# goodmattg/ndivplanning

Measured on AMD Instinct MI355X. Metric: gan_train_steps_per_sec_traj8_batch64, higher is better.
Workload: dtype f32; 1 GPU; BASELINE configs[1]: train_gan.py step (D update + G update), codes mode, batch=64 trajectories per GPU, traj_len=8, num_sample=6, noise_dim=2; rows_per_gpu=2688, global_batch=64, parallelism=dp1, hip_graph=True, steps_per_graph_launch=16, repeats=1, gradient_exchange=none

## Files before the change

include/ndp.h:

```cpp
#ifndef NDP_H_
#define NDP_H_

#include <stddef.h>
#include <stdint.h>

#ifdef __cplusplus
extern "C" {
#endif

#define NDP_VERSION 135

#define NDP_OK            0
#define NDP_E_ARG         1
#define NDP_E_LAUNCH      2
#define NDP_E_UNSUPPORTED 3

#define NDP_CODE_DIM      256
#define NDP_ACTION_DIM    4
#define NDP_MAX_NOISE_DIM 16
#define NDP_MAX_SAMPLES   256
#define NDP_ROW_PAD       32

int         ndp_version(void);
const char *ndp_last_error(void);

int64_t ndp_g_param_count(int noise_dim);
int64_t ndp_d_param_count(void);

int64_t ndp_pad_rows(int64_t rows);

int64_t ndp_ndiv_partials(int64_t n, int k);
int ndp_ndiv_fwd_bwd(const float *x, int cx, const float *z, int cz, int64_t n, int k,
                     float grad_scale, float *loss_out, float *grad_x, float *partials,
                     void *stream);

int64_t ndp_g_acts_floats(int64_t m);
int ndp_g_forward(const float *g_params, int noise_dim,
                  const float *code, int64_t ld_code, int code_rep,
                  const float *noise, int64_t ld_noise, int64_t m,
                  float *acts, float *action_hat, void *stream);

int64_t ndp_g_bwd_ws_floats(int64_t m, int noise_dim);
int ndp_g_backward(const float *g_params, int noise_dim,
                   const float *code, int64_t ld_code, int code_rep,
                   const float *noise, int64_t ld_noise, int64_t m,
                   const float *acts, const float *d_action,
                   float *grad, float *ws, void *stream);

int ndp_d_forward(const float *d_params,
                  const float *action, int action_rep,
                  const float *code, int64_t ld_code, int code_rep, int64_t m,
                  float *logits, void *stream);

int64_t ndp_d_bwd_ws_floats(int64_t m);
int ndp_d_backward(const float *d_params,
                   const float *action, int action_rep,
                   const float *code, int64_t ld_code, int code_rep, int64_t m,
                   const float *d_logits, float *grad, float *d_action,
                   float *ws, void *stream);

int ndp_adam_step(float *params, const float *grad, float *exp_avg, float *exp_avg_sq,
                  int64_t n, int32_t *step_count, float lr, float beta1, float beta2,
                  float eps, void *stream);

struct ndp_p2p;
typedef struct ndp_step_config {
  int32_t noise_dim;
  int32_t num_sample;
  int64_t flat;
  float   inv_m_global;
  float   pairwise_div_factor;
  float   lr, beta1, beta2, eps;
  int32_t fuse_adam;
  int32_t device_noise;
  uint64_t noise_seed;
  const struct ndp_p2p *p2p;
} ndp_step_config;

typedef struct ndp_step_buffers {
  float   *g_params, *g_grad, *g_exp_avg, *g_exp_avg_sq;
  float   *d_params, *d_grad, *d_exp_avg, *d_exp_avg_sq;
  int32_t *g_step, *d_step;
  float   *losses;
  float   *loss_sums;
  float   *action_hat;
  float   *workspace;
} ndp_step_buffers;

int64_t ndp_step_workspace_floats(const ndp_step_config *cfg);

int ndp_step_d_grads(const ndp_step_config *cfg, const ndp_step_buffers *buf,
                     const float *codes, const float *actions, float *noise,
                     int run_g_forward, void *stream);
int ndp_step_g_grads(const ndp_step_config *cfg, const ndp_step_buffers *buf,
                     const float *codes, const float *actions, const float *noise,
                     void *stream);

int ndp_step_pack_params(const ndp_step_config *cfg, const ndp_step_buffers *buf, void *stream);

int ndp_step_apply_adam(const ndp_step_config *cfg, const ndp_step_buffers *buf, int which,
                        void *stream);

int ndp_uniform_noise(float *out, int64_t n, uint64_t seed, const int32_t *offset_dev,
                      void *stream);

#define NDP_P2P_MAX_RANKS    8
#define NDP_P2P_HANDLE_BYTES 64

typedef struct ndp_p2p {
  int32_t world, rank;
  int32_t timeout_ms;
  int32_t reserved;
  void   *region[NDP_P2P_MAX_RANKS];
} ndp_p2p;

int64_t ndp_p2p_region_bytes(void);
int ndp_p2p_region_alloc(void **region);
int ndp_p2p_region_free(void *region);
int ndp_p2p_region_reset(void *region);
int ndp_p2p_export(void *region, void *handle_out);
int ndp_p2p_open(const void *handle, void **mapped_out);
int ndp_p2p_close(void *mapped);
int ndp_p2p_status(const ndp_p2p *p2p, int32_t *status_out);
#define NDP_P2P_DIAG_WORDS 8
int ndp_p2p_diagnostics(const ndp_p2p *p2p, int32_t *words_out);
int ndp_p2p_status_async(const ndp_p2p *p2p, int32_t *pinned_host_out, void *stream);
int ndp_device_pci_bus_id(char *out, int len);
int ndp_p2p_all_reduce(const ndp_p2p *p2p, int net, const float *in, float *out, int64_t n,
                       const int32_t *step_word, void *stream);

int64_t ndp_encoder_param_floats(void);
int64_t ndp_encoder_workspace_floats(int64_t n_images);
int ndp_encoder_forward(const float *packed_params, const float *images, int64_t n_images,
                        float *codes, float *workspace, void *stream);
int ndp_encoder_forward_u8(const float *packed_params, const uint8_t *frames_hwc, int64_t n_images,
                           float *codes, float *workspace, void *stream);

int64_t ndp_fm_param_floats(void);
int64_t ndp_fm_stat_floats(void);
int64_t ndp_fm_workspace_floats(int64_t n_images);
int64_t ndp_fm_workspace_offset(int64_t n_images, int tensor);
int ndp_fm_layout(int what, int index, int64_t *offset, int64_t *dims );
int ndp_fm_pack_params(const float *params, float *workspace, void *stream);
int ndp_fm_forward(const float *params, float *running_stats, const float *state_cur,
                   const float *actions, int64_t n_images, int training, float *out,
                   float *workspace, void *stream);
int ndp_fm_train_grads(const float *params, float *running_stats, const float *state_cur,
                       const float *state_fut, const float *actions, int64_t n_images,
                       float *grad, float *loss, float *loss_sum, float *resid_out,
                       float *workspace, void *stream);
int ndp_fm_forward_u8(const float *params, float *running_stats, const uint8_t *frames_cur,
                      const float *actions, int64_t n_images, int training, float *out,
                      float *workspace, void *stream);
int ndp_fm_train_grads_u8(const float *params, float *running_stats, const uint8_t *frames_cur,
                          const uint8_t *frames_fut, const float *actions, int64_t n_images,
                          float *grad, float *loss, float *loss_sum, float *resid_out,
                          float *workspace, void *stream);
int ndp_fm_side_stream(int on);
typedef void (*ndp_fm_stat_sync_fn)(void *acc, int64_t words, void *stream, void *ctx);
int ndp_fm_set_stat_sync(ndp_fm_stat_sync_fn fn, void *ctx, int world);

int ndp_fm_grad_buckets(int64_t *offsets, int64_t *counts, int capacity);
int ndp_fm_bucket_wait(int bucket, void *stream);
int ndp_fm_backward(const float *params, const float *d_resid, int64_t n_images, float *grad,
                    float *workspace, void *stream);
int ndp_fm_apply_adam(float *params, const float *grad, float *exp_avg, float *exp_avg_sq,
                      int32_t *step_count, float lr, float beta1, float beta2, float eps,
                      float *workspace, void *stream);

int64_t ndp_ae_param_floats(void);
int64_t ndp_ae_stat_floats(void);
int64_t ndp_ae_workspace_floats(int64_t n_images);
int64_t ndp_ae_workspace_offset(int64_t n_images, int tensor);
int ndp_ae_layout(int what, int index, int64_t *offset, int64_t *dims );
int ndp_ae_pack_params(const float *params, float *workspace, void *stream);
int ndp_ae_train_grads(const float *params, float *running_stats, const float *images, int64_t n_images,
                       float *grad, float *loss, float *loss_sum, float *recon_out, float *workspace,
                       void *stream);
int ndp_ae_apply_adam(float *params, const float *grad, float *exp_avg, float *exp_avg_sq,
                      int32_t *step_count, float lr, float beta1, float beta2, float eps,
                      float *workspace, void *stream);
int ndp_ae_train_grads_dp(const float *params, float *running_stats, const float *images, int64_t n_images,
                          float *grad, float *loss, float *loss_sum, float *recon_out, float *workspace,
                          void *stream, ndp_fm_stat_sync_fn stat_sync, void *stat_ctx, int world);
int ndp_ae_grad_buckets(int64_t *offsets, int64_t *counts, int capacity, int *n_buckets);
int ndp_ae_bucket_wait(int bucket, void *stream);

int ndp_eval_score_select(const float *pred, int64_t n_traj, int rollouts, const float *target, int64_t n_target,
                          const int32_t *target_idx, int64_t values, const float *actions0, const float *pred0,
                          const int32_t *forced, float *err, int32_t *choice, float *action_out, float *pred_out,
                          void *stream);
int64_t ndp_eval_mse_ws_floats(int64_t n_pairs);
int ndp_eval_mse(const float *a, int64_t n_a, const float *b, int64_t n_b, const int32_t *a_idx, const int32_t *b_idx,
                 int64_t n_pairs, int64_t values, int64_t group, float *mse, float *acc, float *ws, void *stream);
int ndp_eval_g_input(const float *state_code, int64_t n_state, int state_rep, const float *goal_code, int64_t n_goal,
                     int goal_rep, int64_t rows, float *out, void *stream);
int ndp_eval_frames_u8(const uint8_t *frames_hwc, int64_t n_images, float *images, void *stream);

#define NDP_JPEG_OK          0
#define NDP_JPEG_UNSUPPORTED 1
#define NDP_JPEG_SIZE        2
#define NDP_JPEG_CORRUPT     3
#define NDP_JPEG_WORKSPACE   4
int64_t ndp_jpeg_workspace_bytes(int64_t n_images, int64_t stream_bytes);
int ndp_jpeg_decode_u8(const uint8_t *streams, const int64_t *offsets , int64_t n_images,
                       uint8_t *frames_hwc , int32_t *status , void *workspace,
                       int64_t workspace_bytes, void *stream);

int ndp_timing_enable(int on);
int ndp_timing_collect(char *names, int names_len, float *total_ms, int32_t *counts,
                       int max_kernels);

#ifdef __cplusplus
}
#endif
#endif
```

ndivplanning_amd/_capi.py:

```python
import ctypes
import os
from ctypes import POINTER, Structure, c_char_p, c_float, c_int, c_int32, c_int64, c_uint64, c_void_p

import torch

from . import _build

CODE_DIM = 256
ACTION_DIM = 4
MAX_NOISE_DIM = 16
MAX_SAMPLES = 256
ROW_PAD = 32
EXPECTED_VERSION = 135

_lib = None


class NdpError(RuntimeError):
    pass


P2P_MAX_RANKS = 8
P2P_HANDLE_BYTES = 64
P2P_DIAG_WORDS = 8


class P2P(Structure):
    _fields_ = [("world", c_int32), ("rank", c_int32), ("timeout_ms", c_int32), ("reserved", c_int32),
                ("region", c_void_p * P2P_MAX_RANKS)]


class StepConfig(Structure):
    _fields_ = [("noise_dim", c_int32), ("num_sample", c_int32), ("flat", c_int64),
                ("inv_m_global", c_float), ("pairwise_div_factor", c_float),
                ("lr", c_float), ("beta1", c_float), ("beta2", c_float), ("eps", c_float),
                ("fuse_adam", c_int32), ("device_noise", c_int32), ("noise_seed", c_uint64),
                ("p2p", POINTER(P2P))]


class StepBuffers(Structure):
    _fields_ = [(n, c_void_p) for n in (
        "g_params", "g_grad", "g_exp_avg", "g_exp_avg_sq",
        "d_params", "d_grad", "d_exp_avg", "d_exp_avg_sq",
        "g_step", "d_step", "losses", "loss_sums", "action_hat", "workspace")]


SIGNATURES = {
    "ndp_version": (c_int, []),
    "ndp_last_error": (c_char_p, []),
    "ndp_g_param_count": (c_int64, [c_int]),
    "ndp_d_param_count": (c_int64, []),
    "ndp_pad_rows": (c_int64, [c_int64]),
    "ndp_ndiv_partials": (c_int64, [c_int64, c_int]),
    "ndp_ndiv_fwd_bwd": (c_int, [c_void_p, c_int, c_void_p, c_int, c_int64, c_int, c_float,
                                 c_void_p, c_void_p, c_void_p, c_void_p]),
    "ndp_g_acts_floats": (c_int64, [c_int64]),
    "ndp_g_forward": (c_int, [c_void_p, c_int, c_void_p, c_int64, c_int, c_void_p, c_int64, c_int64,
                              c_void_p, c_void_p, c_void_p]),
    "ndp_g_bwd_ws_floats": (c_int64, [c_int64, c_int]),
    "ndp_g_backward": (c_int, [c_void_p, c_int, c_void_p, c_int64, c_int, c_void_p, c_int64, c_int64,
                               c_void_p, c_void_p, c_void_p, c_void_p, c_void_p]),
    "ndp_d_forward": (c_int, [c_void_p, c_void_p, c_int, c_void_p, c_int64, c_int, c_int64, c_void_p, c_void_p]),
    "ndp_d_bwd_ws_floats": (c_int64, [c_int64]),
    "ndp_d_backward": (c_int, [c_void_p, c_void_p, c_int, c_void_p, c_int64, c_int, c_int64, c_void_p,
                               c_void_p, c_void_p, c_void_p, c_void_p]),
    "ndp_adam_step": (c_int, [c_void_p, c_void_p, c_void_p, c_void_p, c_int64, c_void_p,
                              c_float, c_float, c_float, c_float, c_void_p]),
    "ndp_step_workspace_floats": (c_int64, [POINTER(StepConfig)]),
    "ndp_step_d_grads": (c_int, [POINTER(StepConfig), POINTER(StepBuffers), c_void_p, c_void_p, c_void_p,
                                 c_int, c_void_p]),
    "ndp_step_g_grads": (c_int, [POINTER(StepConfig), POINTER(StepBuffers), c_void_p, c_void_p, c_void_p,
                                 c_void_p]),
    "ndp_step_pack_params": (c_int, [POINTER(StepConfig), POINTER(StepBuffers), c_void_p]),
    "ndp_step_apply_adam": (c_int, [POINTER(StepConfig), POINTER(StepBuffers), c_int, c_void_p]),
    "ndp_uniform_noise": (c_int, [c_void_p, c_int64, c_uint64, c_void_p, c_void_p]),
    "ndp_p2p_region_bytes": (c_int64, []),
    "ndp_p2p_region_alloc": (c_int, [POINTER(c_void_p)]),
    "ndp_p2p_region_free": (c_int, [c_void_p]),
    "ndp_p2p_region_reset": (c_int, [c_void_p]),
    "ndp_p2p_export": (c_int, [c_void_p, c_void_p]),
    "ndp_p2p_open": (c_int, [c_void_p, POINTER(c_void_p)]),
    "ndp_p2p_close": (c_int, [c_void_p]),
    "ndp_p2p_status": (c_int, [POINTER(P2P), POINTER(c_int32)]),
    "ndp_p2p_diagnostics": (c_int, [POINTER(P2P), POINTER(c_int32)]),
    "ndp_p2p_status_async": (c_int, [POINTER(P2P), c_void_p, c_void_p]),
    "ndp_device_pci_bus_id": (c_int, [ctypes.c_char_p, c_int]),
    "ndp_p2p_all_reduce": (c_int, [POINTER(P2P), c_int, c_void_p, c_void_p, c_int64, c_void_p, c_void_p]),
    "ndp_encoder_param_floats": (c_int64, []),
    "ndp_encoder_workspace_floats": (c_int64, [c_int64]),
    "ndp_encoder_forward": (c_int, [c_void_p, c_void_p, c_int64, c_void_p, c_void_p, c_void_p]),
    "ndp_encoder_forward_u8": (c_int, [c_void_p, c_void_p, c_int64, c_void_p, c_void_p, c_void_p]),
    "ndp_fm_param_floats": (c_int64, []),
    "ndp_fm_stat_floats": (c_int64, []),
    "ndp_fm_workspace_floats": (c_int64, [c_int64]),
    "ndp_fm_workspace_offset": (c_int64, [c_int64, c_int]),
    "ndp_fm_layout": (c_int, [c_int, c_int, POINTER(c_int64), POINTER(c_int64)]),
    "ndp_fm_pack_params": (c_int, [c_void_p, c_void_p, c_void_p]),
    "ndp_fm_forward": (c_int, [c_void_p, c_void_p, c_void_p, c_void_p, c_int64, c_int, c_void_p, c_void_p, c_void_p]),
    "ndp_fm_train_grads": (c_int, [c_void_p, c_void_p, c_void_p, c_void_p, c_void_p, c_int64, c_void_p, c_void_p, c_void_p,
                                   c_void_p, c_void_p, c_void_p]),
    "ndp_fm_forward_u8": (c_int, [c_void_p, c_void_p, c_void_p, c_void_p, c_int64, c_int, c_void_p, c_void_p, c_void_p]),
    "ndp_fm_train_grads_u8": (c_int, [c_void_p, c_void_p, c_void_p, c_void_p, c_void_p, c_int64, c_void_p, c_void_p, c_void_p,
                                      c_void_p, c_void_p, c_void_p]),
    "ndp_fm_side_stream": (c_int, [c_int]),
    "ndp_fm_grad_buckets": (c_int, [POINTER(c_int64), POINTER(c_int64), c_int]),
    "ndp_fm_set_stat_sync": (c_int, [c_void_p, c_void_p, c_int]),
    "ndp_fm_bucket_wait": (c_int, [c_int, c_void_p]),
    "ndp_fm_backward": (c_int, [c_void_p, c_void_p, c_int64, c_void_p, c_void_p, c_void_p]),
    "ndp_fm_apply_adam": (c_int, [c_void_p, c_void_p, c_void_p, c_void_p, c_void_p, c_float, c_float, c_float, c_float,
                                  c_void_p, c_void_p]),
    "ndp_ae_param_floats": (c_int64, []),
    "ndp_ae_stat_floats": (c_int64, []),
    "ndp_ae_workspace_floats": (c_int64, [c_int64]),
    "ndp_ae_workspace_offset": (c_int64, [c_int64, c_int]),
    "ndp_ae_layout": (c_int, [c_int, c_int, POINTER(c_int64), POINTER(c_int64)]),
    "ndp_ae_pack_params": (c_int, [c_void_p, c_void_p, c_void_p]),
    "ndp_ae_train_grads": (c_int, [c_void_p, c_void_p, c_void_p, c_int64, c_void_p, c_void_p, c_void_p, c_void_p, c_void_p,
                                   c_void_p]),
    "ndp_ae_apply_adam": (c_int, [c_void_p, c_void_p, c_void_p, c_void_p, c_void_p, c_float, c_float, c_float, c_float,
                                  c_void_p, c_void_p]),
    "ndp_ae_train_grads_dp": (c_int, [c_void_p, c_void_p, c_void_p, c_int64, c_void_p, c_void_p, c_void_p, c_void_p,
                                      c_void_p, c_void_p, c_void_p, c_void_p, c_int]),
    "ndp_ae_grad_buckets": (c_int, [POINTER(c_int64), POINTER(c_int64), c_int, POINTER(c_int)]),
    "ndp_ae_bucket_wait": (c_int, [c_int, c_void_p]),
    "ndp_eval_score_select": (c_int, [c_void_p, c_int64, c_int, c_void_p, c_int64, c_void_p, c_int64, c_void_p, c_void_p,
                                      c_void_p, c_void_p, c_void_p, c_void_p, c_void_p, c_void_p]),
    "ndp_eval_mse_ws_floats": (c_int64, [c_int64]),
    "ndp_eval_mse": (c_int, [c_void_p, c_int64, c_void_p, c_int64, c_void_p, c_void_p, c_int64, c_int64, c_int64, c_void_p,
                             c_void_p, c_void_p, c_void_p]),
    "ndp_eval_g_input": (c_int, [c_void_p, c_int64, c_int, c_void_p, c_int64, c_int, c_int64, c_void_p, c_void_p]),
    "ndp_eval_frames_u8": (c_int, [c_void_p, c_int64, c_void_p, c_void_p]),
    "ndp_jpeg_workspace_bytes": (c_int64, [c_int64, c_int64]),
    "ndp_jpeg_decode_u8": (c_int, [c_void_p, c_void_p, c_int64, c_void_p, c_void_p, c_void_p, c_int64, c_void_p]),
    "ndp_timing_enable": (c_int, [c_int]),
    "ndp_timing_collect": (c_int, [ctypes.c_char_p, c_int, POINTER(c_float), POINTER(c_int32), c_int]),
}


def lib_path():
    return _build.LIB_PATH


def load():
    global _lib
    if _lib is not None:
        return _lib
    path = lib_path()
    if not os.path.exists(path):
        raise NdpError(
            "ndivplanning_amd: %s is missing -- build it with `python -m ndivplanning_amd._build` "
            "(or __graft_entry__.build()); there is no fallback path." % path)
    lib = ctypes.CDLL(path)
    for name, (res, args) in SIGNATURES.items():
        fn = getattr(lib, name)
        fn.restype = res
        fn.argtypes = args
    if lib.ndp_version() != EXPECTED_VERSION:
        raise NdpError("%s is version %d, this package needs %d: rebuild with `python -m ndivplanning_amd._build`"
                       % (path, lib.ndp_version(), EXPECTED_VERSION))
    _lib = lib
    return lib


def check(rc, what):
    if rc != 0:
        msg = load().ndp_last_error()
        raise NdpError("%s failed (code %d): %s" % (what, rc, msg.decode() if msg else "?"))


def stream_ptr(device=None):
    return c_void_p(torch.cuda.current_stream(device).cuda_stream)


def on_device(t):
    dev = t.device if isinstance(t, torch.Tensor) else torch.device(t)
    return torch.cuda.device(dev)


def ptr(t):
    return c_void_p(t.data_ptr()) if t is not None else c_void_p(0)


def require_gpu_f32(t, name):
    if not isinstance(t, torch.Tensor):
        raise TypeError("%s must be a torch.Tensor" % name)
    if not t.is_cuda:
        raise NdpError("%s is on %s: ndivplanning_amd computes only on a ROCm GPU (no CPU fallback)"
                       % (name, t.device))
    if t.dtype != torch.float32:
        raise NdpError("%s must be float32, got %s" % (name, t.dtype))
    return t


def empty(n, like):
    return torch.empty(int(n), dtype=torch.float32, device=like.device)


def timing_enable(on):
    load().ndp_timing_enable(1 if on else 0)


def timing_collect():
    lib = load()
    names = ctypes.create_string_buffer(4096)
    ms = (c_float * 64)()
    counts = (c_int32 * 64)()
    n = lib.ndp_timing_collect(names, 4096, ms, counts, 64)
    keys = [k for k in names.value.decode().split(";") if k]
    return {keys[i]: (float(ms[i]), int(counts[i])) for i in range(min(n, len(keys)))}


def g_param_count(noise_dim):
    return int(load().ndp_g_param_count(int(noise_dim)))


def d_param_count():
    return int(load().ndp_d_param_count())


def pad_rows(m):
    return (int(m) + ROW_PAD - 1) // ROW_PAD * ROW_PAD


def fm_grad_buckets():
    lib = load()
    off = (ctypes.c_int64 * 16)()
    cnt = (ctypes.c_int64 * 16)()
    n = lib.ndp_fm_grad_buckets(off, cnt, 16)
    if n <= 0:
        msg = lib.ndp_last_error()
        raise NdpError("ndp_fm_grad_buckets failed: %s" % (msg.decode() if msg else "?"))
    return [(int(off[i]), int(cnt[i])) for i in range(n)]


def ae_grad_buckets():
    lib = load()
    off = (ctypes.c_int64 * 16)()
    cnt = (ctypes.c_int64 * 16)()
    n = ctypes.c_int(0)
    check(lib.ndp_ae_grad_buckets(off, cnt, 16, ctypes.byref(n)), "ndp_ae_grad_buckets")
    return [(int(off[i]), int(cnt[i])) for i in range(n.value)]


STAT_SYNC_FN = ctypes.CFUNCTYPE(None, c_void_p, c_int64, c_void_p, c_void_p)
```

ndivplanning_amd/csrc/ndp_capi.inc:

```
#include <stdarg.h>
#include <stdio.h>
#include <stdlib.h>
#include <string.h>

#include <dlfcn.h>
#include <mutex>

#include "../../include/ndp.h"

namespace ndp {

static thread_local char g_err[512] = "";

static int fail(int code, const char* fmt, ...) {
  va_list ap;
  va_start(ap, fmt);
  vsnprintf(g_err, sizeof(g_err), fmt, ap);
  va_end(ap);
  return code;
}

#define NDP_CHECK_ARG(cond, ...) \
  do { if (!(cond)) return ndp::fail(NDP_E_ARG, __VA_ARGS__); } while (0)

static int check_launch(const char* what) {
  hipError_t e = hipGetLastError();
  if (e != hipSuccess) return fail(NDP_E_LAUNCH, "%s: %s", what, hipGetErrorString(e));
  return NDP_OK;
}

struct TimedLaunch { const char* name; hipEvent_t t0, t1; };
struct TimingState {
  bool on = false;
  TimedLaunch ev[4096];
  int n = 0;
};
static thread_local TimingState g_timing;

struct Roctx { int (*push)(const char*); int (*pop)(); bool on; };
static Roctx& roctx() {
  static Roctx r = [] {
    Roctx x = {nullptr, nullptr, false};
    const char* e = getenv("NDP_ROCTX");
    if (e && e[0] == '1') {
      void* h = dlopen("libroctx64.so", RTLD_NOW | RTLD_GLOBAL);
      if (!h) h = dlopen("libroctx64.so.4", RTLD_NOW | RTLD_GLOBAL);
      if (h) {
        x.push = reinterpret_cast<int (*)(const char*)>(dlsym(h, "roctxRangePushA"));
        x.pop = reinterpret_cast<int (*)()>(dlsym(h, "roctxRangePop"));
        x.on = x.push && x.pop;
      }
    }
    return x;
  }();
  return r;
}

struct KTimer {
  hipStream_t st; int idx; bool range;
  KTimer(const char* name, hipStream_t s) : st(s), idx(-1), range(false) {
    if (roctx().on) { roctx().push(name); range = true; }
    TimingState& t = g_timing;
    if (!t.on || t.n >= 4096) return;
    idx = t.n++;
    t.ev[idx].name = name;
    hipEventCreate(&t.ev[idx].t0);
    hipEventCreate(&t.ev[idx].t1);
    hipEventRecord(t.ev[idx].t0, st);
  }
  ~KTimer() {
    if (idx >= 0) hipEventRecord(g_timing.ev[idx].t1, st);
    if (range) roctx().pop();
  }
};

static inline bool aligned16(const void* p) { return (reinterpret_cast<uintptr_t>(p) & 15) == 0; }
static inline int64_t pad_rows(int64_t rows) { return (rows + NDP_ROW_PAD - 1) / NDP_ROW_PAD * NDP_ROW_PAD; }

template <typename K>
static void allow_lds(K kernel, int bytes) {
  hipFuncSetAttribute(reinterpret_cast<const void*>(kernel), hipFuncAttributeMaxDynamicSharedMemorySize, bytes);
}

constexpr int kMaxDevices = 64;
static std::once_flag g_attr_once[kMaxDevices];
static std::once_flag& device_once(std::once_flag (&flags)[kMaxDevices]) {
  int dev = 0;
  if (hipGetDevice(&dev) != hipSuccess || dev < 0 || dev >= kMaxDevices) dev = 0;
  return flags[dev];
}
static_assert(phase_a_lds_floats() * 4 * 3 <= 160 * 1024, "phase A: three workgroups per CU at large M");

static void set_attrs() {
  std::call_once(device_once(g_attr_once), [] {
#define NDP_ATTR_GFWD(WA) \
    allow_lds(k_g_fwd<WA, false>, g_fwd_lds_floats() * 4); \
    allow_lds(k_g_fwd<WA, true>, g_fwd_lds_floats() * 4);
    NDP_ATTR_GFWD(1) NDP_ATTR_GFWD(2) NDP_ATTR_GFWD(4)
#undef NDP_ATTR_GFWD
#define NDP_ATTR_D(NP) \
    allow_lds(k_d<NP, false>, (d_lds_floats<NP>() * 4)); \
    allow_lds(k_d<NP, true>, (d_lds_floats<NP>() * 4));
    NDP_ATTR_D(1) NDP_ATTR_D(2)
#undef NDP_ATTR_D
    allow_lds(k_g_bwd<false>, g_bwd_lds_floats() * 4);
    allow_lds(k_g_bwd<true>, g_bwd_lds_floats() * 4);
    allow_lds(k_wgrad, wgrad_lds_floats() * 4);
    allow_lds(k_wgrad_wide, wgrad_wide_launch_lds_floats() * 4);
#define NDP_ALLOW_A(RG, NR) allow_lds((k_phase_a<true, RG, NR>), phase_a_lds_floats() * 4)
#define NDP_ALLOW_B(RG, PRE, NR) allow_lds((k_phase_b<true, RG, PRE, NR>), phase_b_lds_floats(PRE) * 4)
    NDP_ALLOW_A(96, 0);
    NDP_ALLOW_A(kPhaseASmallRing, 0); NDP_ALLOW_A(kPhaseASmallRing, 1); NDP_ALLOW_A(kPhaseASmallRing, 4);
    NDP_ALLOW_B(96, true, 0);
    NDP_ALLOW_B(32, false, 0); NDP_ALLOW_B(32, false, 1); NDP_ALLOW_B(32, false, 4);
#undef NDP_ALLOW_A
#undef NDP_ALLOW_B
    allow_lds(k_ndiv<4, 2>, 64 * 1024);
    allow_lds(k_ndiv<16, 16>, 64 * 1024);
  });
}

struct GLayout { int64_t w1, b1, w2, b2, w3, b3, w4, b4, w5, b5, total; int in1; };
static GLayout g_layout(int nz) {
  GLayout L;
  L.in1 = CODE + nz;
  int64_t o = 0;
  L.w1 = o; o += 128 * (int64_t)L.in1;
  L.b1 = o; o += 128;
  L.w2 = o; o += 64 * 128;
  L.b2 = o; o += 64;
  L.w3 = o; o += 128 * 64;
  L.b3 = o; o += 128;
  L.w4 = o; o += 256 * 128;
  L.b4 = o; o += 256;
  L.w5 = o; o += 4 * 256;
  L.b5 = o; o += 4;
  L.total = o;
  return L;
}
struct DLayout { int64_t w1, b1, w2, b2, w3, b3, w4, b4, total; };
static DLayout d_layout() {
  DLayout L;
  int64_t o = 0;
  L.w1 = o; o += 64 * 260;
  L.b1 = o; o += 64;
  L.w2 = o; o += 128 * 64;
  L.b2 = o; o += 128;
  L.w3 = o; o += 256 * 128;
  L.b3 = o; o += 256;
  L.w4 = o; o += 256;
  L.b4 = o; o += 1;
  L.total = o;
  return L;
}
constexpr int kGPackF1 = 0, kGPackF2 = 32768, kGPackF3 = 40960, kGPackF4 = 49152,
              kGPackG2 = 81920, kGPackG3 = 90112, kGPackG4 = 98304, kGPackFloats = 131072;
constexpr int kDPackF1 = 0, kDPackF2 = 16384, kDPackF3 = 24576, kDPackG2 = 57344, kDPackG3 = 65536,
              kDPackFloats = 98304;

static GNet g_net(const float* p, int nz, const float* packed = nullptr) {
  const GLayout L = g_layout(nz);
  GNet n;
  n.w1 = p + L.w1; n.b1 = p + L.b1; n.w2 = p + L.w2; n.b2 = p + L.b2; n.w3 = p + L.w3; n.b3 = p + L.b3;
  n.w4 = p + L.w4; n.b4 = p + L.b4; n.w5 = p + L.w5; n.b5 = p + L.b5;
  n.ld1 = L.in1; n.nz = nz;
  n.pf1 = n.pf2 = n.pf3 = n.pf4 = n.pg2 = n.pg3 = n.pg4 = nullptr;
  if (packed) {
    n.pf1 = packed + kGPackF1; n.pf2 = packed + kGPackF2; n.pf3 = packed + kGPackF3; n.pf4 = packed + kGPackF4;
    n.pg2 = packed + kGPackG2; n.pg3 = packed + kGPackG3; n.pg4 = packed + kGPackG4;
  }
  return n;
}
static DNet d_net(const float* p, const float* packed = nullptr) {
  const DLayout L = d_layout();
  DNet n;
  n.w1 = p + L.w1; n.b1 = p + L.b1; n.w2 = p + L.w2; n.b2 = p + L.b2; n.w3 = p + L.w3; n.b3 = p + L.b3;
  n.w4 = p + L.w4; n.b4 = p + L.b4;
  n.pf1 = n.pf2 = n.pf3 = n.pg2 = n.pg3 = nullptr;
  if (packed) {
    n.pf1 = packed + kDPackF1; n.pf2 = packed + kDPackF2; n.pf3 = packed + kDPackF3;
    n.pg2 = packed + kDPackG2; n.pg3 = packed + kDPackG3;
  }
  return n;
}
static PackLayer pack_layer(int64_t w_off, int ld, int out, int main0, int main_in, int fwd_off, int dg_off) {
  PackLayer l;
  l.w_off = (int)w_off; l.ld = ld; l.out = out; l.main0 = main0; l.main_in = main_in; l.fwd_off = fwd_off; l.dg_off = dg_off;
  return l;
}
static PackSpec g_pack_spec(int nz, float* packed) {
  const GLayout L = g_layout(nz);
  PackSpec ps;
  memset(&ps, 0, sizeof(ps));
  ps.L[0] = pack_layer(L.w1, L.in1, 128, 0, CODE, kGPackF1, -1);
  ps.L[1] = pack_layer(L.w2, 128, 64, 0, 128, kGPackF2, kGPackG2);
  ps.L[2] = pack_layer(L.w3, 64, 128, 0, 64, kGPackF3, kGPackG3);
  ps.L[3] = pack_layer(L.w4, 128, 256, 0, 128, kGPackF4, kGPackG4);
  ps.nl = 4; ps.packed = packed;
  return ps;
}
static PackSpec d_pack_spec(float* packed) {
  const DLayout L = d_layout();
  PackSpec ps;
  memset(&ps, 0, sizeof(ps));
  ps.L[0] = pack_layer(L.w1, 260, 64, ADIM, CODE, kDPackF1, -1);
  ps.L[1] = pack_layer(L.w2, 64, 128, 0, 64, kDPackF2, kDPackG2);
  ps.L[2] = pack_layer(L.w3, 128, 256, 0, 128, kDPackF3, kDPackG3);
  ps.nl = 3; ps.packed = packed;
  return ps;
}
static int launch_pack(const float* params, int64_t n, const PackSpec& ps, hipStream_t st) {
  KTimer kt("k_pack", st);
  PackArgs a;
  a.params = params; a.n = (int)n; a.ps = ps;
  hipLaunchKernelGGL(k_pack, dim3((unsigned)((n + kThreads - 1) / kThreads)), dim3(kThreads), 0, st, a);
  return check_launch("k_pack");
}
static inline int64_t pad4(int64_t n) { return (n + 3) / 4 * 4; }

struct GActs { float *h1, *h2, *h3, *h4; };
static int64_t g_acts_floats(int64_t mpad) { return mpad * (128 + 64 + 128 + 256); }
static GActs g_acts(float* base, int64_t mpad) {
  GActs a;
  a.h1 = base; a.h2 = a.h1 + mpad * 128; a.h3 = a.h2 + mpad * 64; a.h4 = a.h3 + mpad * 128;
  return a;
}
static int wgrad_chunks(int njobs, int64_t rows) {
  int64_t want = 512 / njobs;
  if (want >= 8) want = want / 8 * 8;
  if (rows >= 16384 && want < 32) want = 32;
  int64_t maxc = rows / 64;
  if (maxc < 1) maxc = 1;
  if (want > maxc) want = maxc;
  if (want > 64) want = 64;
  return (int)want;
}
constexpr int kGJobs = 26, kDJobs = 19;
static void wgrad_plan(bool is_g, int64_t rows, int* heavy, int* light) {
  const int h = is_g ? 24 : (rows <= 4096 ? 8 : 32), l = is_g ? 12 : 8;
  if (rows >= 16384 || rows / 64 < h) { *heavy = *light = wgrad_chunks(is_g ? kGJobs : kDJobs, rows); return; }
  *heavy = h; *light = l;
}
static int wgrad_wide_chunks(int64_t rows) {
  if (rows < 28000) return 0;
  const int64_t want = (rows / 480 + 16) / 32 * 32;
  return (int)(want < 64 ? 64 : want);
}
static int wgrad_slabs(bool is_g, int64_t rows) {
  int h, l;
  wgrad_plan(is_g, rows, &h, &l);
  const int w = wgrad_wide_chunks(rows);
  return h > w ? h : w;
}
struct GBwdWs { float *dy1, *dy2, *dy3, *dy4, *dy5, *slabs; int nchunks, light; int64_t slab_stride; };
static int64_t g_bwd_floats(int64_t mpad, int nz) {
  return mpad * (128 + 64 + 128 + 256 + 4) + (int64_t)wgrad_slabs(true, mpad) * pad4(g_layout(nz).total);
}
static GBwdWs g_bwd_ws(float* base, int64_t mpad, int nz) {
  GBwdWs w;
  w.dy1 = base; w.dy2 = w.dy1 + mpad * 128; w.dy3 = w.dy2 + mpad * 64; w.dy4 = w.dy3 + mpad * 128;
  w.dy5 = w.dy4 + mpad * 256; w.slabs = w.dy5 + mpad * 4;
  wgrad_plan(true, mpad, &w.nchunks, &w.light);
  w.slab_stride = pad4(g_layout(nz).total);
  return w;
}
struct DBwdWs { float *xa, *h1, *h2, *h3, *dy1, *dy2, *dy3, *dl, *slabs, *lossp; int nchunks, light; int64_t slab_stride; };
static int64_t d_bwd_floats_rows(int64_t rows) {
  return rows * (4 + 2 * (64 + 128 + 256) + 1) + (int64_t)wgrad_slabs(false, rows) * pad4(d_layout().total) +
         pad4(rows / 16);
}
static int64_t d_bwd_floats(int64_t mpad, int npass) { return d_bwd_floats_rows(mpad * npass); }
static DBwdWs d_bwd_ws_rows(float* base, int64_t rows) {
  DBwdWs w;
  w.xa = base; w.h1 = w.xa + rows * 4; w.h2 = w.h1 + rows * 64; w.h3 = w.h2 + rows * 128;
  w.dy1 = w.h3 + rows * 256; w.dy2 = w.dy1 + rows * 64; w.dy3 = w.dy2 + rows * 128; w.dl = w.dy3 + rows * 256;
  w.slabs = w.dl + rows;
  wgrad_plan(false, rows, &w.nchunks, &w.light);
  w.slab_stride = pad4(d_layout().total);
  w.lossp = w.slabs + (int64_t)wgrad_slabs(false, rows) * w.slab_stride;
  return w;
}
static DBwdWs d_bwd_ws(float* base, int64_t mpad, int npass) { return d_bwd_ws_rows(base, mpad * npass); }
static int64_t step_real_pad(const ndp_step_config* c) { return pad_rows(c->flat); }
static int64_t step_d_rows(const ndp_step_config* c) { return step_real_pad(c) + pad_rows(c->flat * c->num_sample); }

struct NoiseGen { float* out; uint64_t seed; const int32_t* step; };

static int launch_g_fwd(const GNet& net, const float* code, int64_t ld_code, int code_rep,
                        const float* noise, int64_t ld_noise, int64_t m, const GActs* acts,
                        float* action_hat, const NoiseGen* gen, hipStream_t st) {
  set_attrs();
  GFwdArgs a;
  a.net = net;
  a.code = code; a.ld_code = ld_code; a.code_rep = code_rep;
  a.code_vec4 = (ld_code % 4 == 0) && aligned16(code);
  a.noise = noise; a.ld_noise = ld_noise; a.m = m;
  a.h1 = acts ? acts->h1 : nullptr; a.h2 = acts ? acts->h2 : nullptr;
  a.h3 = acts ? acts->h3 : nullptr; a.h4 = acts ? acts->h4 : nullptr;
  a.action_hat = action_hat;
  a.noise_out = gen ? gen->out : nullptr; a.noise_seed = gen ? gen->seed : 0; a.noise_step = gen ? gen->step : nullptr;
  const int walign = (net.ld1 % 4 == 0) ? 4 : (net.ld1 % 2 == 0 ? 2 : 1);
  const dim3 grid((unsigned)(pad_rows(m) / 16));
  const bool pk = net.pf1 != nullptr;
#define NDP_LAUNCH_GFWD(WA) \
  do { \
    if (pk) hipLaunchKernelGGL((k_g_fwd<WA, true>), grid, dim3(kThreads), g_fwd_lds_floats() * 4, st, a); \
    else hipLaunchKernelGGL((k_g_fwd<WA, false>), grid, dim3(kThreads), g_fwd_lds_floats() * 4, st, a); \
  } while (0)
  KTimer kt("k_g_fwd", st);
  if (walign == 4) NDP_LAUNCH_GFWD(4); else if (walign == 2) NDP_LAUNCH_GFWD(2); else NDP_LAUNCH_GFWD(1);
#undef NDP_LAUNCH_GFWD
  return check_launch("k_g_fwd");
}

static int launch_d(DArgs& a, int npass, int nd_blocks, hipStream_t st) {
  set_attrs();
  a.ntiles = (int)(a.mpad / 16);
  if (nd_blocks == 0) a.nd.n = 0;
  const dim3 grid((unsigned)(a.ntiles + nd_blocks));
  KTimer kt(a.do_backward ? (npass == 2 ? "k_d[2 pass fwd+bwd]" : "k_d[fwd+bwd]") : "k_d[fwd]", st);
  const bool pk = a.net.pf1 != nullptr;
#define NDP_LAUNCH_D(NP) \
  do { \
    if (pk) hipLaunchKernelGGL((k_d<NP, true>), grid, dim3(kThreads), (d_lds_floats<NP>() * 4), st, a); \
    else hipLaunchKernelGGL((k_d<NP, false>), grid, dim3(kThreads), (d_lds_floats<NP>() * 4), st, a); \
  } while (0)
  if (npass == 2) NDP_LAUNCH_D(2);
  else NDP_LAUNCH_D(1);
#undef NDP_LAUNCH_D
  return check_launch("k_d");
}

static int launch_g_bwd(GBwdArgs& a, hipStream_t st) {
  set_attrs();
  const dim3 grid((unsigned)(pad_rows(a.m) / 16));
  KTimer kt("k_g_bwd", st);
  if (a.net.pg2 != nullptr) hipLaunchKernelGGL((k_g_bwd<true>), grid, dim3(kThreads), g_bwd_lds_floats() * 4, st, a);
  else hipLaunchKernelGGL((k_g_bwd<false>), grid, dim3(kThreads), g_bwd_lds_floats() * 4, st, a);
  return check_launch("k_g_bwd");
}

static WgradJob make_job(const float* A, int lda, int a_cols, const float* B, int ldb, int b_cols,
                         int64_t dst_off, int dst_ld, int64_t bias_off, int kind) {
  WgradJob j;
  j.A = A; j.lda = lda; j.a_cols = a_cols;
  j.B = B; j.ldb = ldb; j.b_cols = b_cols;
  j.b_rowmod = 0x7fffffff; j.b_rowdiv = 1; j.b_rowmax = 0x7fffffff;
  j.b_vec = (ldb % 4 == 0) && aligned16(B);
  j.dst_off = (int)dst_off; j.dst_ld = dst_ld; j.bias_off = (int)bias_off; j.kind = kind;
  j.rows = 0; j.seg = 0; j.seg_s = 1; j.seg_k = 1; j.seg_wrap = 0;
  j.nchunks = kind == WG_FULL ? 1 : 0;
  return j;
}

static int seg_per_tile(int K) { int s = 15 / K + 2; return s < 16 ? s : 16; }
static int64_t seg_entries(int64_t mpad, int K) { return (mpad / 16 * seg_per_tile(K) + 15) / 16 * 16; }

static void build_g_jobs(WgradArgs& w, int nz, const GBwdWs& ws, const GActs& acts,
                         const float* code, int64_t ld_code, int code_rep,
                         const float* noise, int64_t ld_noise, int64_t m, const float* dy1seg = nullptr) {
  const GLayout L = g_layout(nz);
  int n = 0;
  const int code_rowmax = (int)((m - 1) / code_rep);
  for (int jb = 0; jb < 2; ++jb) {
    for (int kb = 0; kb < 4; ++kb) {
      WgradJob j = make_job((dy1seg ? dy1seg : ws.dy1) + jb * 64, 128, 64, code + kb * 64, (int)ld_code, 64,
                            L.w1 + (int64_t)jb * 64 * L.in1 + kb * 64, L.in1,
                            kb == 0 ? L.b1 + jb * 64 : -1, WG_FULL);
      j.b_rowdiv = code_rep; j.b_rowmax = code_rowmax;
      if (dy1seg) { j.rows = (int)seg_entries(pad_rows(m), code_rep); j.seg = 1; j.seg_s = seg_per_tile(code_rep); j.seg_k = code_rep; }
      j.nchunks = 0;
      w.job[n++] = j;
    }
    WgradJob t = make_job(ws.dy1 + jb * 64, 128, 64, noise, (int)ld_noise, nz,
                          L.w1 + (int64_t)jb * 64 * L.in1 + CODE, L.in1, -1, WG_SKINNY_B);
    t.b_rowmax = (int)(m - 1);
    w.job[n++] = t;
  }
  for (int kb = 0; kb < 2; ++kb)
    w.job[n++] = make_job(ws.dy2, 64, 64, acts.h1 + kb * 64, 128, 64, L.w2 + kb * 64, 128,
                          kb == 0 ? L.b2 : -1, WG_FULL);
  for (int jb = 0; jb < 2; ++jb)
    w.job[n++] = make_job(ws.dy3 + jb * 64, 128, 64, acts.h2, 64, 64, L.w3 + (int64_t)jb * 64 * 64, 64,
                          L.b3 + jb * 64, WG_FULL);
  const int wide = wgrad_wide_chunks(pad_rows(m));
  if (!wide)
    for (int jb = 0; jb < 4; ++jb)
      for (int kb = 0; kb < 2; ++kb)
        w.job[n++] = make_job(ws.dy4 + jb * 64, 256, 64, acts.h3 + kb * 64, 128, 64,
                              L.w4 + (int64_t)jb * 64 * 128 + kb * 64, 128, kb == 0 ? L.b4 + jb * 64 : -1, WG_FULL);
  for (int kb = 0; kb < 4; ++kb)
    w.job[n++] = make_job(ws.dy5, 4, 4, acts.h4 + kb * 64, 256, 64, L.w5 + kb * 64, 256,
                          kb == 0 ? L.b5 : -1, WG_SKINNY_A);
  w.njobs = n; w.net_is_g = 1;
  w.nwide = 0; w.wide_chunks = 0;
  w.wide_begin = w.wide_end = 0;
  if (wide) {
    w.nwide = 2;
    for (int h = 0; h < 2; ++h)
      w.job[n + h] = make_job(ws.dy4 + h * 128, 256, 128, acts.h3, 128, 128, L.w4 + (int64_t)h * 128 * 128, 128, L.b4 + h * 128, WG_WIDE);
    w.wide_chunks = wide;
    w.wide_begin = (int)L.w4; w.wide_end = (int)L.b4 + 256;
  }
  w.nreg = 2;
  w.reg_begin[0] = (int)L.w1; w.reg_end[0] = (int)L.b1 + 128;
  w.reg_begin[1] = (int)L.w5; w.reg_end[1] = (int)L.b5 + 4;
}

static void build_d_jobs(WgradArgs& w, const DBwdWs& ws, const float* code, int64_t ld_code, int code_rep,
                         int64_t m, int64_t mpad, const float* dy1seg = nullptr, int64_t rpad = 0, int64_t wide_rows = 0) {
  const DLayout L = d_layout();
  int n = 0;
  for (int kb = 0; kb < 4; ++kb) {
    WgradJob j = make_job(dy1seg ? dy1seg : ws.dy1, 64, 64, code + kb * 64, (int)ld_code, 64, L.w1 + ADIM + kb * 64, 260,
                          kb == 0 ? L.b1 : -1, WG_FULL);
    j.b_rowmod = (int)mpad; j.b_rowdiv = code_rep; j.b_rowmax = (int)((m - 1) / code_rep);
    if (dy1seg) {
      const int e = (int)seg_entries(mpad, code_rep);
      j.rows = e + (int)rpad; j.seg = 1; j.seg_wrap = e;
      j.seg_s = seg_per_tile(code_rep); j.seg_k = code_rep;
    }
    j.nchunks = 0;
    w.job[n++] = j;
  }
  w.job[n++] = make_job(ws.dy1, 64, 64, ws.xa, 4, ADIM, L.w1, 260, -1, WG_SKINNY_B);
  for (int jb = 0; jb < 2; ++jb)
    w.job[n++] = make_job(ws.dy2 + jb * 64, 128, 64, ws.h1, 64, 64, L.w2 + (int64_t)jb * 64 * 64, 64,
                          L.b2 + jb * 64, WG_FULL);
  const int wide = wgrad_wide_chunks(wide_rows);
  if (!wide)
    for (int jb = 0; jb < 4; ++jb)
      for (int kb = 0; kb < 2; ++kb)
        w.job[n++] = make_job(ws.dy3 + jb * 64, 256, 64, ws.h2 + kb * 64, 128, 64,
                              L.w3 + (int64_t)jb * 64 * 128 + kb * 64, 128, kb == 0 ? L.b3 + jb * 64 : -1, WG_FULL);
  for (int kb = 0; kb < 4; ++kb)
    w.job[n++] = make_job(ws.dl, 1, 1, ws.h3 + kb * 64, 256, 64, L.w4 + kb * 64, 256,
                          kb == 0 ? L.b4 : -1, WG_SKINNY_A);
  w.njobs = n; w.net_is_g = 0;
  w.nwide = 0; w.wide_chunks = 0;
  w.wide_begin = w.wide_end = 0;
  if (wide) {
    w.nwide = 2;
    for (int h = 0; h < 2; ++h)
      w.job[n + h] = make_job(ws.dy3 + h * 128, 256, 128, ws.h2, 128, 128, L.w3 + (int64_t)h * 128 * 128, 128, L.b3 + h * 128, WG_WIDE);
    w.wide_chunks = wide;
    w.wide_begin = (int)L.w3; w.wide_end = (int)L.b3 + 256;
  }
  w.nreg = 2;
  w.reg_begin[0] = (int)L.w1; w.reg_end[0] = (int)L.b1 + 64;
  w.reg_begin[1] = (int)L.w4; w.reg_end[1] = (int)L.b4 + 1;
}

struct AdamHyper { float lr, beta1, beta2; };

static int launch_wgrad(WgradArgs& w, int64_t rows, int nchunks, int light, float* slabs, int64_t slab_stride,
                        int32_t* bump, const AdamHyper& hp, const NdivArgs* nd, int nd_blocks, hipStream_t st) {
  set_attrs();
  w.rows = (int)rows;
  for (int i = 0; i < w.njobs; ++i) w.job[i].nchunks = w.job[i].nchunks ? nchunks : light;
  for (int i = 0; i < w.nwide; ++i) w.job[w.njobs + i].nchunks = w.wide_chunks;
  w.slabs = slabs; w.slab_stride = slab_stride; w.bump = bump;
  w.lr = hp.lr; w.beta1 = hp.beta1; w.beta2 = hp.beta2;
  w.nchunks = nchunks;
  if (nd != nullptr && nd_blocks > 0) w.nd = *nd; else { memset(&w.nd, 0, sizeof(w.nd)); nd_blocks = 0; }
  const dim3 grid((unsigned)(w.nwide * w.wide_chunks + 8 * ((nchunks + 7) / 8) * w.njobs + nd_blocks));
  KTimer kt(w.net_is_g ? "k_wgrad[G]" : "k_wgrad[D]", st);
  if (w.nwide) hipLaunchKernelGGL(k_wgrad_wide, grid, dim3(kThreads), wgrad_wide_launch_lds_floats() * 4, st, w);
  else hipLaunchKernelGGL(k_wgrad, grid, dim3(kThreads), wgrad_lds_floats() * 4, st, w);
  return check_launch("k_wgrad");
}

static void set_red_regions(ReduceArgs& r, const WgradArgs& w, int light) {
  r.nregions = light != r.nchunks ? w.nreg : 0;
  for (int i = 0; i < r.nregions; ++i) { r.reg_begin[i] = w.reg_begin[i]; r.reg_end[i] = w.reg_end[i]; r.reg_slabs[i] = light; }
  if (w.nwide) {
    const int i = r.nregions++;
    r.reg_begin[i] = w.wide_begin; r.reg_end[i] = w.wide_end; r.reg_slabs[i] = w.wide_chunks;
  }
}

static int launch_reduce(ReduceArgs& r, hipStream_t st) {
  const dim3 grid((unsigned)((r.n + kThreads - 1) / kThreads + 1));
  KTimer kt("k_reduce_adam", st);
  if (r.p2p.world > 1)
    hipLaunchKernelGGL(k_reduce_adam<true>, grid, dim3(kThreads), 0, st, r);
  else
    hipLaunchKernelGGL(k_reduce_adam<false>, grid, dim3(kThreads), 0, st, r);
  return check_launch("k_reduce_adam");
}

static int ndiv_block_threads(int k) { return k <= 64 ? 64 : kThreads; }
static int ndiv_rows_per_block(int k, int threads) { return threads / k; }
static size_t ndiv_lds_bytes(int G, int k, int cx, int cz) { return ((size_t)G * k * (cx + cz + 2) + 8) * 4; }

static NdivArgs ndiv_args(const float* x, int cx, const float* z, int cz, int64_t n, int k, float grad_scale,
                          float* grad, float* partials, int threads) {
  NdivArgs a;
  a.x = x; a.cx = cx; a.z = z; a.cz = cz; a.n = n; a.k = k;
  a.rows_per_block = ndiv_rows_per_block(k, threads);
  a.grad_scale = grad_scale; a.grad = grad; a.partials = partials;
  return a;
}

static int launch_ndiv(const float* x, int cx, const float* z, int cz, int64_t n, int k, float grad_scale,
                       float* grad, float* partials, hipStream_t st) {
  set_attrs();
  const int threads = ndiv_block_threads(k);
  NdivArgs a = ndiv_args(x, cx, z, cz, n, k, grad_scale, grad, partials, threads);
  const int G = a.rows_per_block;
  const size_t lds = ndiv_lds_bytes(G, k, cx, cz);
  const dim3 grid((unsigned)((n + G - 1) / G));
  KTimer kt("k_ndiv", st);
  if (cx <= 4 && cz <= 2) hipLaunchKernelGGL((k_ndiv<4, 2>), grid, dim3(threads), lds, st, a);
  else hipLaunchKernelGGL((k_ndiv<16, 16>), grid, dim3(threads), lds, st, a);
  return check_launch("k_ndiv");
}

}

using namespace ndp;

extern "C" {

int ndp_version(void) { return NDP_VERSION; }
const char* ndp_last_error(void) { return g_err; }
int64_t ndp_g_param_count(int noise_dim) { return g_layout(noise_dim).total; }
int64_t ndp_d_param_count(void) { return d_layout().total; }
int64_t ndp_pad_rows(int64_t rows) { return pad_rows(rows); }

int64_t ndp_ndiv_partials(int64_t n, int k) {
  if (k < 1 || k > NDP_MAX_SAMPLES || n < 0) return 0;
  const int G = ndiv_rows_per_block(k, ndiv_block_threads(k));
  return (n + G - 1) / G + 1;
}

int ndp_ndiv_fwd_bwd(const float* x, int cx, const float* z, int cz, int64_t n, int k, float grad_scale,
                     float* loss_out, float* grad_x, float* partials, void* stream) {
  NDP_CHECK_ARG(x && z && loss_out && partials, "ndp_ndiv_fwd_bwd: null pointer");
  NDP_CHECK_ARG(k >= 1 && k <= NDP_MAX_SAMPLES, "ndp_ndiv_fwd_bwd: k=%d outside 1..%d", k, NDP_MAX_SAMPLES);
  NDP_CHECK_ARG(cx >= 1 && cx <= kNdivMaxC && cz >= 1 && cz <= kNdivMaxC, "ndp_ndiv_fwd_bwd: channel count outside 1..16");
  NDP_CHECK_ARG(n >= 1 && n * k < (1ll << 31), "ndp_ndiv_fwd_bwd: bad row count %lld", (long long)n);
  hipStream_t st = (hipStream_t)stream;
  int rc = launch_ndiv(x, cx, z, cz, n, k, grad_scale, grad_x, partials, st);
  if (rc) return rc;
  const int G = ndiv_rows_per_block(k, ndiv_block_threads(k));
  hipLaunchKernelGGL(k_sum_partials, dim3(1), dim3(kThreads), 0, st, (const float*)partials,
                     (int)((n + G - 1) / G), 1.0f, loss_out);
  return check_launch("k_sum_partials");
}

int64_t ndp_g_acts_floats(int64_t m) { return g_acts_floats(pad_rows(m)); }

static int check_g_common(const char* fn, const float* g_params, int noise_dim, const float* code,
                          int64_t ld_code, int code_rep, const float* noise, int64_t ld_noise, int64_t m) {
  NDP_CHECK_ARG(g_params && code && noise, "%s: null pointer", fn);
  NDP_CHECK_ARG(aligned16(g_params), "%s: g_params must be 16-byte aligned", fn);
  NDP_CHECK_ARG(noise_dim >= 1 && noise_dim <= NDP_MAX_NOISE_DIM, "%s: noise_dim=%d outside 1..%d", fn, noise_dim, NDP_MAX_NOISE_DIM);
  NDP_CHECK_ARG(m >= 1 && m < (1ll << 30), "%s: bad row count %lld", fn, (long long)m);
  NDP_CHECK_ARG(code_rep >= 1 && ld_code >= NDP_CODE_DIM && ld_noise >= noise_dim, "%s: bad strides", fn);
  return NDP_OK;
}

int ndp_g_forward(const float* g_params, int noise_dim, const float* code, int64_t ld_code, int code_rep,
                  const float* noise, int64_t ld_noise, int64_t m, float* acts, float* action_hat, void* stream) {
  int rc = check_g_common("ndp_g_forward", g_params, noise_dim, code, ld_code, code_rep, noise, ld_noise, m);
  if (rc) return rc;
  NDP_CHECK_ARG(action_hat && aligned16(action_hat), "ndp_g_forward: action_hat null or not 16-byte aligned");
  NDP_CHECK_ARG(!acts || aligned16(acts), "ndp_g_forward: acts not 16-byte aligned");
  const int64_t mpad = pad_rows(m);
  GActs a;
  if (acts) a = g_acts(acts, mpad);
  return launch_g_fwd(g_net(g_params, noise_dim), code, ld_code, code_rep, noise, ld_noise, m,
                      acts ? &a : nullptr, action_hat, nullptr, (hipStream_t)stream);
}

int64_t ndp_g_bwd_ws_floats(int64_t m, int noise_dim) { return g_bwd_floats(pad_rows(m), noise_dim); }

static int g_backward_impl(const GNet& gnet, int nz, const float* code, int64_t ld_code, int code_rep,
                           const float* noise, int64_t ld_noise, int64_t m, const GActs& acts,
                           const float* d_action, const float* d_action2, float* ws_base,
                           ReduceArgs& red, int32_t* bump, const AdamHyper& hp, hipStream_t st,
                           const float* dy1seg = nullptr) {
  const int64_t mpad = pad_rows(m);
  GBwdWs ws = g_bwd_ws(ws_base, mpad, nz);
  GBwdArgs b;
  b.net = gnet;
  b.m = m;
  b.h1 = acts.h1; b.h2 = acts.h2; b.h3 = acts.h3; b.h4 = acts.h4;
  b.d_action = d_action; b.d_action2 = d_action2;
  b.dy1 = ws.dy1; b.dy2 = ws.dy2; b.dy3 = ws.dy3; b.dy4 = ws.dy4; b.dy5 = ws.dy5;
  int rc = NDP_OK;
  if (d_action != nullptr) {
    rc = launch_g_bwd(b, st);
    if (rc) return rc;
  }
  WgradArgs w;
  build_g_jobs(w, nz, ws, acts, code, ld_code, code_rep, noise, ld_noise, m, dy1seg);
  rc = launch_wgrad(w, mpad, ws.nchunks, ws.light, ws.slabs, ws.slab_stride, bump, hp, nullptr, 0, st);
  if (rc) return rc;
  red.slabs = ws.slabs; red.nchunks = ws.nchunks; red.slab_stride = ws.slab_stride;
  set_red_regions(red, w, ws.light);
  red.n = g_layout(nz).total;
  return launch_reduce(red, st);
}

int ndp_g_backward(const float* g_params, int noise_dim, const float* code, int64_t ld_code, int code_rep,
                   const float* noise, int64_t ld_noise, int64_t m, const float* acts, const float* d_action,
                   float* grad, float* ws, void* stream) {
  int rc = check_g_common("ndp_g_backward", g_params, noise_dim, code, ld_code, code_rep, noise, ld_noise, m);
  if (rc) return rc;
  NDP_CHECK_ARG(acts && d_action && grad && ws, "ndp_g_backward: null pointer");
  NDP_CHECK_ARG(aligned16(acts) && aligned16(d_action) && aligned16(ws), "ndp_g_backward: buffers must be 16-byte aligned");
  ReduceArgs red;
  memset(&red, 0, sizeof(red));
  red.grad = grad;
  GActs a = g_acts(const_cast<float*>(acts), pad_rows(m));
  return g_backward_impl(g_net(g_params, noise_dim), noise_dim, code, ld_code, code_rep, noise, ld_noise, m, a, d_action,
                         nullptr, ws, red, nullptr, AdamHyper{0.f, 0.f, 0.f}, (hipStream_t)stream);
}

static int check_d_common(const char* fn, const float* d_params, const float* action, int action_rep,
                          const float* code, int64_t ld_code, int code_rep, int64_t m) {
  NDP_CHECK_ARG(d_params && action && code, "%s: null pointer", fn);
  NDP_CHECK_ARG(aligned16(d_params), "%s: d_params must be 16-byte aligned", fn);
  NDP_CHECK_ARG(m >= 1 && m < (1ll << 29), "%s: bad row count %lld", fn, (long long)m);
  NDP_CHECK_ARG(action_rep >= 1 && code_rep >= 1 && ld_code >= NDP_CODE_DIM, "%s: bad strides", fn);
  return NDP_OK;
}

static void d_args_init(DArgs& a, const float* d_params, const float* code, int64_t ld_code, int code_rep, int64_t m) {
  memset(&a, 0, sizeof(a));
  a.net = d_net(d_params);
  a.code = code; a.ld_code = ld_code; a.code_rep = code_rep;
  a.code_vec4 = (ld_code % 4 == 0) && aligned16(code);
  a.m = m; a.mpad = pad_rows(m);
  a.inv_m = 1.f / (float)m;
}

int ndp_d_forward(const float* d_params, const float* action, int action_rep, const float* code, int64_t ld_code,
                  int code_rep, int64_t m, float* logits, void* stream) {
  int rc = check_d_common("ndp_d_forward", d_params, action, action_rep, code, ld_code, code_rep, m);
  if (rc) return rc;
  NDP_CHECK_ARG(logits, "ndp_d_forward: null logits");
  DArgs a;
  d_args_init(a, d_params, code, ld_code, code_rep, m);
  a.pass[0].action = action; a.pass[0].action_rep = action_rep; a.pass[0].target = 0.f;
  a.logits = logits;
  return launch_d(a, 1, 0, (hipStream_t)stream);
}

int64_t ndp_d_bwd_ws_floats(int64_t m) { return d_bwd_floats(pad_rows(m), 1); }

int ndp_d_backward(const float* d_params, const float* action, int action_rep, const float* code, int64_t ld_code,
                   int code_rep, int64_t m, const float* d_logits, float* grad, float* d_action, float* ws,
                   void* stream) {
  int rc = check_d_common("ndp_d_backward", d_params, action, action_rep, code, ld_code, code_rep, m);
  if (rc) return rc;
  NDP_CHECK_ARG(d_logits, "ndp_d_backward: null d_logits");
  NDP_CHECK_ARG(!grad || (ws && aligned16(ws)), "ndp_d_backward: grad needs a 16-byte aligned workspace");
  NDP_CHECK_ARG(!d_action || action_rep == 1, "ndp_d_backward: d_action needs action_rep == 1");
  hipStream_t st = (hipStream_t)stream;
  DArgs a;
  d_args_init(a, d_params, code, ld_code, code_rep, m);
  a.pass[0].action = action; a.pass[0].action_rep = action_rep; a.pass[0].target = 0.f;
  a.ext_dlogit = d_logits;
  a.do_backward = 1;
  a.d_action = d_action;
  DBwdWs w;
  if (grad) {
    w = d_bwd_ws(ws, a.mpad, 1);
    a.h1 = w.h1; a.h2 = w.h2; a.h3 = w.h3; a.dy1 = w.dy1; a.dy2 = w.dy2; a.dy3 = w.dy3; a.dl = w.dl; a.xa = w.xa;
  }
  rc = launch_d(a, 1, 0, st);
  if (rc || !grad) return rc;
  WgradArgs wa;
  build_d_jobs(wa, w, code, ld_code, code_rep, m, a.mpad, nullptr, 0, a.mpad);
  rc = launch_wgrad(wa, a.mpad, w.nchunks, w.light, w.slabs, w.slab_stride, nullptr, AdamHyper{0.f, 0.f, 0.f}, nullptr, 0, st);
  if (rc) return rc;
  ReduceArgs red;
  memset(&red, 0, sizeof(red));
  red.slabs = w.slabs; red.nchunks = w.nchunks; red.slab_stride = w.slab_stride; red.n = d_layout().total;
  set_red_regions(red, wa, w.light);
  red.grad = grad;
  return launch_reduce(red, st);
}

int ndp_adam_step(float* params, const float* grad, float* exp_avg, float* exp_avg_sq, int64_t n,
                  int32_t* step_count, float lr, float beta1, float beta2, float eps, void* stream) {
  NDP_CHECK_ARG(params && grad && exp_avg && exp_avg_sq && step_count, "ndp_adam_step: null pointer");
  NDP_CHECK_ARG(n >= 1, "ndp_adam_step: n < 1");
  hipStream_t st = (hipStream_t)stream;
  hipLaunchKernelGGL(k_adam_advance, dim3(1), dim3(1), 0, st, step_count, lr, beta1, beta2);
  AdamArgs a;
  a.params = params; a.exp_avg = exp_avg; a.exp_avg_sq = exp_avg_sq; a.grad = grad; a.n = n;
  a.step = step_count; a.lr = lr; a.beta1 = beta1; a.beta2 = beta2; a.eps = eps;
  memset(&a.pack, 0, sizeof(a.pack));
  KTimer kt("k_adam", st);
  hipLaunchKernelGGL(k_adam, dim3((unsigned)((n + kThreads - 1) / kThreads)), dim3(kThreads), 0, st, a);
  return check_launch("k_adam");
}

struct StepWs {
  GActs acts; float* gb; float* db; float* d_action; float* nd_grad; float* nd_part; int64_t nd_count;
  float* g_packed; float* d_packed;
  float* d_seg; float* g_seg;
};
static bool several_per_cu(int64_t workgroups) { return workgroups > 256; }

static int step_code_rows(int K, bool several_per_cu) {
  if (!several_per_cu) return 0;
  return K % 16 == 0 ? 1 : (K >= 6 ? 4 : 0);
}

static bool step_ndiv_fused(const ndp_step_config* c) { return c->noise_dim <= 2; }
static int step_ndiv_threads(const ndp_step_config* c) {
  return step_ndiv_fused(c) ? kThreads : ndiv_block_threads(c->num_sample);
}

static int64_t step_floats(const ndp_step_config* c, StepWs* out, float* base) {
  const int64_t m = c->flat * c->num_sample, mpad = pad_rows(m);
  int64_t o = 0;
  const int64_t o_acts = o; o += g_acts_floats(mpad);
  const int64_t o_gb = o; o += g_bwd_floats(mpad, c->noise_dim);
  const int64_t o_db = o;
  { const int64_t a_ = d_bwd_floats(mpad, 2), b_ = d_bwd_floats_rows(step_d_rows(c)); o += a_ > b_ ? a_ : b_; }
  const int64_t o_da = o; o += mpad * 4;
  const int64_t o_ng = o; o += mpad * 4;
  const int64_t o_np = o;
  const int G = ndiv_rows_per_block(c->num_sample, step_ndiv_threads(c));
  const int64_t npart = (c->flat + G - 1) / G;
  o += pad4(npart);
  const int64_t o_gp = o; o += kGPackFloats;
  const int64_t o_dp = o; o += kDPackFloats;
  const int64_t o_ds = o;
  o += (seg_entries(mpad, c->num_sample) + step_real_pad(c)) * 64;
  const int64_t o_gs = o; o += seg_entries(mpad, c->num_sample) * 128;
  if (out) {
    out->g_packed = base + o_gp; out->d_packed = base + o_dp;
    out->d_seg = base + o_ds; out->g_seg = base + o_gs;
    out->acts = g_acts(base + o_acts, mpad);
    out->gb = base + o_gb; out->db = base + o_db; out->d_action = base + o_da; out->nd_grad = base + o_ng;
    out->nd_part = base + o_np; out->nd_count = npart;
  }
  return o;
}

static int check_step(const char* fn, const ndp_step_config* c, const ndp_step_buffers* b, const float* codes,
                      const float* actions, const float* noise) {
  NDP_CHECK_ARG(c && b && codes && actions && noise, "%s: null pointer", fn);
  NDP_CHECK_ARG(c->noise_dim >= 1 && c->noise_dim <= NDP_MAX_NOISE_DIM, "%s: noise_dim=%d outside 1..%d", fn, c->noise_dim, NDP_MAX_NOISE_DIM);
  NDP_CHECK_ARG(c->num_sample >= 1 && c->num_sample <= NDP_MAX_SAMPLES, "%s: num_sample=%d outside 1..%d", fn, c->num_sample, NDP_MAX_SAMPLES);
  NDP_CHECK_ARG(c->flat >= 1 && c->flat * c->num_sample < (1ll << 28), "%s: bad flat=%lld", fn, (long long)c->flat);
  NDP_CHECK_ARG(b->g_params && b->d_params && b->losses && b->action_hat && b->workspace && b->g_step && b->d_step,
                "%s: null buffer", fn);
  NDP_CHECK_ARG(c->fuse_adam ? (b->g_exp_avg && b->g_exp_avg_sq && b->d_exp_avg && b->d_exp_avg_sq)
                             : (b->g_grad && b->d_grad), "%s: missing Adam state / gradient buffers", fn);
  NDP_CHECK_ARG(aligned16(b->g_params) && aligned16(b->d_params) && aligned16(b->workspace) && aligned16(b->action_hat) &&
                aligned16(codes) && aligned16(actions), "%s: buffers must be 16-byte aligned", fn);
  return NDP_OK;
}

static int fill_p2p(const char* fn, P2PArgs& x, const ndp_p2p* c, int net, int64_t n) {
  memset(&x, 0, sizeof(x));
  if (c == nullptr || c->world <= 1) return NDP_OK;
  NDP_CHECK_ARG(c->world <= NDP_P2P_MAX_RANKS && c->rank >= 0 && c->rank < c->world, "%s: p2p world=%d rank=%d", fn, c->world, c->rank);
  NDP_CHECK_ARG(n <= (net == 0 ? kP2PCapD : kP2PCapG), "%s: %lld values exceed the p2p inbox of net %d", fn, (long long)n, net);
  for (int r = 0; r < c->world; ++r) NDP_CHECK_ARG(c->region[r] != nullptr, "%s: p2p region of rank %d is null", fn, r);
  x.world = c->world; x.rank = c->rank; x.net = net;
  x.timeout_ticks = 100000ll * (c->timeout_ms > 0 ? c->timeout_ms : 10000);
  for (int r = 0; r < c->world; ++r) x.region[r] = static_cast<uint32_t*>(c->region[r]);
  return NDP_OK;
}

#define NDP_HIP(call, what) do { hipError_t e_ = (call); if (e_ != hipSuccess) \
  return ndp::fail(NDP_E_LAUNCH, "%s: %s", what, hipGetErrorString(e_)); } while (0)

int64_t ndp_p2p_region_bytes(void) { return kP2PWords * 4; }

int ndp_p2p_region_alloc(void** region) {
  NDP_CHECK_ARG(region != nullptr, "ndp_p2p_region_alloc: null pointer");
  static_assert(sizeof(hipIpcMemHandle_t) == NDP_P2P_HANDLE_BYTES, "handle size");
  void* p = nullptr;
  NDP_HIP(hipExtMallocWithFlags(&p, (size_t)kP2PWords * 4, hipDeviceMallocUncached), "ndp_p2p_region_alloc");
  hipError_t e = hipMemset(p, 0, (size_t)kP2PWords * 4);
  if (e == hipSuccess) e = hipDeviceSynchronize();
  if (e != hipSuccess) { hipFree(p); return ndp::fail(NDP_E_LAUNCH, "ndp_p2p_region_alloc: %s", hipGetErrorString(e)); }
  *region = p;
  return NDP_OK;
}

int ndp_p2p_region_free(void* region) {
  if (region == nullptr) return NDP_OK;
  NDP_HIP(hipFree(region), "ndp_p2p_region_free");
  return NDP_OK;
}

int ndp_p2p_region_reset(void* region) {
  NDP_CHECK_ARG(region != nullptr, "ndp_p2p_region_reset: null pointer");
  NDP_HIP(hipDeviceSynchronize(), "ndp_p2p_region_reset");
  NDP_HIP(hipMemset(region, 0, (size_t)kP2PInboxD * 4), "ndp_p2p_region_reset");
  NDP_HIP(hipDeviceSynchronize(), "ndp_p2p_region_reset");
  return NDP_OK;
}

int ndp_p2p_export(void* region, void* handle_out) {
  NDP_CHECK_ARG(region && handle_out, "ndp_p2p_export: null pointer");
  hipIpcMemHandle_t h;
  NDP_HIP(hipIpcGetMemHandle(&h, region), "ndp_p2p_export");
  memcpy(handle_out, &h, sizeof(h));
  return NDP_OK;
}

int ndp_p2p_open(const void* handle, void** mapped_out) {
  NDP_CHECK_ARG(handle && mapped_out, "ndp_p2p_open: null pointer");
  hipIpcMemHandle_t h;
  memcpy(&h, handle, sizeof(h));
  void* p = nullptr;
  NDP_HIP(hipIpcOpenMemHandle(&p, h, hipIpcMemLazyEnablePeerAccess), "ndp_p2p_open");
  *mapped_out = p;
  return NDP_OK;
}

int ndp_p2p_close(void* mapped) {
  if (mapped == nullptr) return NDP_OK;
  NDP_HIP(hipIpcCloseMemHandle(mapped), "ndp_p2p_close");
  return NDP_OK;
}

int ndp_p2p_status(const ndp_p2p* c, int32_t* status_out) {
  NDP_CHECK_ARG(c && status_out && c->rank >= 0 && c->rank < NDP_P2P_MAX_RANKS && c->region[c->rank], "ndp_p2p_status: bad arguments");
  NDP_HIP(hipMemcpy(status_out, c->region[c->rank], 4, hipMemcpyDeviceToHost), "ndp_p2p_status");
  return NDP_OK;
}

int ndp_p2p_diagnostics(const ndp_p2p* c, int32_t* words_out) {
  NDP_CHECK_ARG(c && words_out && c->rank >= 0 && c->rank < NDP_P2P_MAX_RANKS && c->region[c->rank], "ndp_p2p_diagnostics: bad arguments");
  NDP_HIP(hipMemcpy(words_out, c->region[c->rank], 4 * NDP_P2P_DIAG_WORDS, hipMemcpyDeviceToHost), "ndp_p2p_diagnostics");
  return NDP_OK;
}

int ndp_p2p_status_async(const ndp_p2p* c, int32_t* pinned_host_out, void* stream) {
  NDP_CHECK_ARG(c && pinned_host_out && c->rank >= 0 && c->rank < NDP_P2P_MAX_RANKS && c->region[c->rank], "ndp_p2p_status_async: bad arguments");
  NDP_HIP(hipMemcpyAsync(pinned_host_out, c->region[c->rank], 4, hipMemcpyDeviceToHost, (hipStream_t)stream), "ndp_p2p_status_async");
  return NDP_OK;
}

int ndp_device_pci_bus_id(char* out, int len) {
  NDP_CHECK_ARG(out && len >= 16, "ndp_device_pci_bus_id: need a buffer of >= 16 bytes");
  int dev = 0;
  NDP_HIP(hipGetDevice(&dev), "ndp_device_pci_bus_id");
  NDP_HIP(hipDeviceGetPCIBusId(out, len, dev), "ndp_device_pci_bus_id");
  return NDP_OK;
}

int ndp_p2p_all_reduce(const ndp_p2p* c, int net, const float* in, float* out, int64_t n, const int32_t* step_word,
                       void* stream) {
  NDP_CHECK_ARG(c && in && out && step_word && n >= 1 && (net == 0 || net == 1), "ndp_p2p_all_reduce: bad arguments");
  ReduceArgs red;
  memset(&red, 0, sizeof(red));
  int rc = fill_p2p("ndp_p2p_all_reduce", red.p2p, c, net, n);
  if (rc) return rc;
  red.slabs = in; red.nchunks = 1; red.slab_stride = 0; red.n = n;
  red.grad = out; red.step = step_word;
  return launch_reduce(red, (hipStream_t)stream);
}

int64_t ndp_step_workspace_floats(const ndp_step_config* cfg) {
  if (!cfg || cfg->flat < 1 || cfg->num_sample < 1 || cfg->num_sample > NDP_MAX_SAMPLES) return 0;
  return step_floats(cfg, nullptr, nullptr);
}

int ndp_step_d_grads(const ndp_step_config* c, const ndp_step_buffers* b, const float* codes, const float* actions,
                     float* noise, int run_g_forward, void* stream) {
  int rc = check_step("ndp_step_d_grads", c, b, codes, actions, noise);
  if (rc) return rc;
  hipStream_t st = (hipStream_t)stream;
  const int K = c->num_sample, nz = c->noise_dim;
  const int64_t m = c->flat * K, mpad = pad_rows(m);
  StepWs ws;
  step_floats(c, &ws, b->workspace);
  const int64_t rpad = step_real_pad(c);
  DBwdWs dw = run_g_forward ? d_bwd_ws_rows(ws.db, step_d_rows(c)) : d_bwd_ws(ws.db, mpad, 2);
  const bool fused_ndiv = step_ndiv_fused(c);
  NdivArgs nd;
  if (fused_ndiv)
    nd = ndiv_args(b->action_hat, ADIM, noise, nz, c->flat, K, c->pairwise_div_factor, ws.nd_grad, ws.nd_part, kThreads);
  int loss_count = (int)(mpad / 16);
  if (run_g_forward) {
    set_attrs();
    PhaseAArgs pa;
    memset(&pa, 0, sizeof(pa));
    pa.g = g_net(b->g_params, nz, ws.g_packed);
    pa.d = d_net(b->d_params, ws.d_packed);
    pa.code = codes; pa.code_rep = K;
    pa.noise = c->device_noise ? nullptr : noise;
    pa.noise_out = c->device_noise ? noise : nullptr; pa.noise_seed = c->noise_seed; pa.noise_step = b->g_step;
    pa.actions = actions;
    pa.m = m; pa.mpad = mpad; pa.flat = c->flat; pa.rpad = rpad;
    pa.inv_m = c->inv_m_global; pa.real_scale = (float)K;
    pa.gh1 = ws.acts.h1; pa.gh2 = ws.acts.h2; pa.gh3 = ws.acts.h3; pa.gh4 = ws.acts.h4;
    pa.action_hat = b->action_hat;
    pa.h1 = dw.h1; pa.h2 = dw.h2; pa.h3 = dw.h3; pa.dy1 = dw.dy1; pa.dy2 = dw.dy2; pa.dy3 = dw.dy3; pa.dl = dw.dl; pa.xa = dw.xa;
    pa.loss_partials = dw.lossp;
    pa.dy1seg = ws.d_seg; pa.seg_s = seg_per_tile(K); pa.seg_entries = (int)seg_entries(mpad, K);
    KTimer kt("k_phase_a", st);
    loss_count = (int)(mpad / 16 + rpad / 16);
    const bool small = several_per_cu(loss_count);
    const int nr = step_code_rows(K, small);
#define NDP_LAUNCH_A(RG, NR) hipLaunchKernelGGL((k_phase_a<true, RG, NR>), dim3((unsigned)loss_count), dim3(kThreads), phase_a_lds_floats() * 4, st, pa)
    if (small) {
      if (nr == 1) NDP_LAUNCH_A(kPhaseASmallRing, 1);
      else if (nr == 4) NDP_LAUNCH_A(kPhaseASmallRing, 4);
      else NDP_LAUNCH_A(kPhaseASmallRing, 0);
    } else {
      NDP_LAUNCH_A(96, 0);
    }
#undef NDP_LAUNCH_A
    rc = check_launch("k_phase_a");
    if (rc) return rc;
  } else {
    DArgs a;
    d_args_init(a, b->d_params, codes, CODE, K, m);
    a.net = d_net(b->d_params, ws.d_packed);
    a.inv_m = c->inv_m_global;
    a.pass[0].action = actions; a.pass[0].action_rep = K; a.pass[0].target = 1.f;
    a.pass[1].action = b->action_hat; a.pass[1].action_rep = 1; a.pass[1].target = 0.f;
    a.do_backward = 1;
    a.h1 = dw.h1; a.h2 = dw.h2; a.h3 = dw.h3; a.dy1 = dw.dy1; a.dy2 = dw.dy2; a.dy3 = dw.dy3; a.dl = dw.dl; a.xa = dw.xa;
    a.loss_partials = dw.lossp;
    rc = launch_d(a, 2, 0, st);
    if (rc) return rc;
  }
  WgradArgs wa;
  build_d_jobs(wa, dw, codes, CODE, K, m, mpad, run_g_forward ? ws.d_seg : nullptr, rpad, run_g_forward ? step_d_rows(c) : 2 * mpad);
  rc = launch_wgrad(wa, run_g_forward ? step_d_rows(c) : 2 * mpad, dw.nchunks, dw.light, dw.slabs, dw.slab_stride, b->d_step,
                    AdamHyper{c->lr, c->beta1, c->beta2}, fused_ndiv ? &nd : nullptr, (int)ws.nd_count, st);
  if (rc) return rc;
  ReduceArgs red;
  memset(&red, 0, sizeof(red));
  red.slabs = dw.slabs; red.nchunks = dw.nchunks; red.slab_stride = dw.slab_stride; red.n = d_layout().total;
  set_red_regions(red, wa, dw.light);
  red.grad = b->d_grad;
  if (c->fuse_adam) {
    red.params = b->d_params; red.exp_avg = b->d_exp_avg; red.exp_avg_sq = b->d_exp_avg_sq; red.step = b->d_step;
    red.lr = c->lr; red.beta1 = c->beta1; red.beta2 = c->beta2; red.eps = c->eps;
    red.pack = d_pack_spec(ws.d_packed);
  }
  red.step = b->d_step;
  rc = fill_p2p("ndp_step_d_grads", red.p2p, c->p2p, 0, red.n);
  if (rc) return rc;
  red.loss[0].partials = dw.lossp; red.loss[0].count = loss_count; red.loss[0].scale = c->inv_m_global;
  red.loss[0].slot = 0;
  red.nloss = 1; red.losses = b->losses; red.loss_sums = b->loss_sums;
  return launch_reduce(red, st);
}

int ndp_step_g_grads(const ndp_step_config* c, const ndp_step_buffers* b, const float* codes, const float* actions,
                     const float* noise, void* stream) {
  int rc = check_step("ndp_step_g_grads", c, b, codes, actions, noise);
  if (rc) return rc;
  hipStream_t st = (hipStream_t)stream;
  const int K = c->num_sample, nz = c->noise_dim;
  const int64_t m = c->flat * K, mpad = pad_rows(m);
  StepWs ws;
  step_floats(c, &ws, b->workspace);
  DBwdWs dw = d_bwd_ws_rows(ws.db, step_d_rows(c));
  if (!step_ndiv_fused(c)) {
    rc = launch_ndiv(b->action_hat, ADIM, noise, nz, c->flat, K, c->pairwise_div_factor, ws.nd_grad, ws.nd_part, st);
    if (rc) return rc;
  }
  set_attrs();
  GBwdWs gw = g_bwd_ws(ws.gb, mpad, nz);
  PhaseBArgs pb;
  memset(&pb, 0, sizeof(pb));
  pb.g = g_net(b->g_params, nz, ws.g_packed);
  pb.d = d_net(b->d_params, ws.d_packed);
  pb.code = codes; pb.code_rep = K;
  pb.action_hat = b->action_hat; pb.nd_grad = ws.nd_grad;
  pb.m = m; pb.inv_m = c->inv_m_global;
  pb.gh1 = ws.acts.h1; pb.gh2 = ws.acts.h2; pb.gh3 = ws.acts.h3; pb.gh4 = ws.acts.h4;
  pb.dy1 = gw.dy1; pb.dy2 = gw.dy2; pb.dy3 = gw.dy3; pb.dy4 = gw.dy4; pb.dy5 = gw.dy5;
  pb.loss_partials = dw.lossp;
  pb.dy1seg = ws.g_seg; pb.seg_s = seg_per_tile(K); pb.seg_entries = (int)seg_entries(mpad, K);
  {
    KTimer kt("k_phase_b", st);
    const int nt = (int)(mpad / 16);
    const bool small = several_per_cu(nt);
    const int nr = step_code_rows(K, small);
#define NDP_LAUNCH_B(RG, PRE, NR) hipLaunchKernelGGL((k_phase_b<true, RG, PRE, NR>), dim3((unsigned)nt), dim3(kThreads), phase_b_lds_floats(PRE) * 4, st, pb)
    if (small) {
      if (nr == 1) NDP_LAUNCH_B(32, false, 1);
      else if (nr == 4) NDP_LAUNCH_B(32, false, 4);
      else NDP_LAUNCH_B(32, false, 0);
    } else {
      NDP_LAUNCH_B(96, true, 0);
    }
#undef NDP_LAUNCH_B
  }
  rc = check_launch("k_phase_b");
  if (rc) return rc;
  ReduceArgs red;
  memset(&red, 0, sizeof(red));
  red.grad = b->g_grad;
  if (c->fuse_adam) {
    red.params = b->g_params; red.exp_avg = b->g_exp_avg; red.exp_avg_sq = b->g_exp_avg_sq; red.step = b->g_step;
    red.lr = c->lr; red.beta1 = c->beta1; red.beta2 = c->beta2; red.eps = c->eps;
    red.pack = g_pack_spec(nz, ws.g_packed);
  }
  red.step = b->g_step;
  rc = fill_p2p("ndp_step_g_grads", red.p2p, c->p2p, 1, g_layout(nz).total);
  if (rc) return rc;
  red.loss[0].partials = dw.lossp; red.loss[0].count = (int)(mpad / 16); red.loss[0].scale = c->inv_m_global;
  red.loss[0].slot = 1;
  red.loss[1].partials = ws.nd_part; red.loss[1].count = (int)ws.nd_count; red.loss[1].scale = 1.f;
  red.loss[1].slot = 2;
  red.nloss = 2; red.losses = b->losses; red.loss_sums = b->loss_sums;
  return g_backward_impl(g_net(b->g_params, nz, ws.g_packed), nz, codes, CODE, K, noise, nz, m, ws.acts, nullptr,
                         nullptr, ws.gb, red, b->g_step, AdamHyper{c->lr, c->beta1, c->beta2}, st, ws.g_seg);
}

#ifdef NDP_STAMPS
int ndp_debug_set_stamps(void* dev_buffer, int kernel_id) {
  unsigned long long* p = (unsigned long long*)dev_buffer;
  if (hipMemcpyToSymbol(HIP_SYMBOL(g_stamp_kernel), &kernel_id, sizeof(int)) != hipSuccess) return NDP_E_LAUNCH;
  return hipMemcpyToSymbol(HIP_SYMBOL(g_stamps), &p, sizeof(p)) == hipSuccess ? 0 : NDP_E_LAUNCH;
}
#endif

int ndp_timing_enable(int on) {
  TimingState& t = g_timing;
  for (int i = 0; i < t.n; ++i) { hipEventDestroy(t.ev[i].t0); hipEventDestroy(t.ev[i].t1); }
  t.n = 0;
  t.on = on != 0;
  return NDP_OK;
}

int ndp_timing_collect(char* names, int names_len, float* total_ms, int32_t* counts, int max_kernels) {
  if (!(names && total_ms && counts && names_len > 0 && max_kernels > 0)) {
    fail(NDP_E_ARG, "ndp_timing_collect: bad arguments");
    return 0;
  }
  TimingState& t = g_timing;
  const char* seen[64];
  int nk = 0;
  names[0] = 0;
  for (int i = 0; i < t.n; ++i) {
    if (hipEventSynchronize(t.ev[i].t1) != hipSuccess) {
      fail(NDP_E_LAUNCH, "ndp_timing_collect: event sync failed");
      return 0;
    }
    float ms = 0.f;
    hipEventElapsedTime(&ms, t.ev[i].t0, t.ev[i].t1);
    int k = 0;
    while (k < nk && strcmp(seen[k], t.ev[i].name) != 0) ++k;
    if (k == nk) {
      if (nk >= max_kernels || nk >= 64) continue;
      seen[nk] = t.ev[i].name; total_ms[nk] = 0.f; counts[nk] = 0; ++nk;
      strncat(names, t.ev[i].name, names_len - strlen(names) - 2);
      strncat(names, ";", names_len - strlen(names) - 1);
    }
    total_ms[k] += ms;
    counts[k] += 1;
    hipEventDestroy(t.ev[i].t0);
    hipEventDestroy(t.ev[i].t1);
  }
  t.n = 0;
  return nk;
}

int ndp_step_pack_params(const ndp_step_config* c, const ndp_step_buffers* b, void* stream) {
  NDP_CHECK_ARG(c && b && b->g_params && b->d_params && b->workspace, "ndp_step_pack_params: null pointer");
  NDP_CHECK_ARG(c->noise_dim >= 1 && c->noise_dim <= NDP_MAX_NOISE_DIM && c->flat >= 1 && c->num_sample >= 1 &&
                c->num_sample <= NDP_MAX_SAMPLES, "ndp_step_pack_params: bad configuration");
  StepWs ws;
  step_floats(c, &ws, b->workspace);
  hipStream_t st = (hipStream_t)stream;
  int rc = launch_pack(b->g_params, g_layout(c->noise_dim).total, g_pack_spec(c->noise_dim, ws.g_packed), st);
  if (rc) return rc;
  return launch_pack(b->d_params, d_layout().total, d_pack_spec(ws.d_packed), st);
}

int ndp_step_apply_adam(const ndp_step_config* c, const ndp_step_buffers* b, int which, void* stream) {
  NDP_CHECK_ARG(c && b && b->workspace, "ndp_step_apply_adam: null pointer");
  NDP_CHECK_ARG(which == 0 || which == 1, "ndp_step_apply_adam: which must be 0 (D) or 1 (G)");
  StepWs ws;
  step_floats(c, &ws, b->workspace);
  hipStream_t st = (hipStream_t)stream;
  AdamArgs a;
  if (which == 1) {
    NDP_CHECK_ARG(b->g_params && b->g_grad && b->g_exp_avg && b->g_exp_avg_sq && b->g_step, "ndp_step_apply_adam: null G buffer");
    a.params = b->g_params; a.grad = b->g_grad; a.exp_avg = b->g_exp_avg; a.exp_avg_sq = b->g_exp_avg_sq;
    a.n = g_layout(c->noise_dim).total; a.step = b->g_step; a.pack = g_pack_spec(c->noise_dim, ws.g_packed);
  } else {
    NDP_CHECK_ARG(b->d_params && b->d_grad && b->d_exp_avg && b->d_exp_avg_sq && b->d_step, "ndp_step_apply_adam: null D buffer");
    a.params = b->d_params; a.grad = b->d_grad; a.exp_avg = b->d_exp_avg; a.exp_avg_sq = b->d_exp_avg_sq;
    a.n = d_layout().total; a.step = b->d_step; a.pack = d_pack_spec(ws.d_packed);
  }
  a.lr = c->lr; a.beta1 = c->beta1; a.beta2 = c->beta2; a.eps = c->eps;
  KTimer kt("k_adam", st);
  hipLaunchKernelGGL(k_adam, dim3((unsigned)((a.n + kThreads - 1) / kThreads)), dim3(kThreads), 0, st, a);
  return check_launch("k_adam");
}

int ndp_uniform_noise(float* out, int64_t n, uint64_t seed, const int32_t* offset_dev, void* stream) {
  NDP_CHECK_ARG(out && n >= 1, "ndp_uniform_noise: bad arguments");
  const int64_t nthreads = n;
  hipLaunchKernelGGL(k_philox, dim3((unsigned)((nthreads + kThreads - 1) / kThreads)), dim3(kThreads), 0,
                     (hipStream_t)stream, out, n, seed, offset_dev);
  return check_launch("k_philox");
}

}
```

ndivplanning_amd/csrc/ndp_device.h:

```cpp
#pragma once
#include <hip/hip_runtime.h>
#include <stdint.h>

namespace ndp {

typedef float f32x4 __attribute__((ext_vector_type(4)));
typedef float f32x2 __attribute__((ext_vector_type(2)));
typedef uint32_t u32x4 __attribute__((ext_vector_type(4)));

constexpr int kThreads = 256;
constexpr int kWaves = 4;
constexpr float kLreluSlope = 0.01f;

enum Act { ACT_NONE = 0, ACT_RELU = 1, ACT_LRELU = 2 };

__device__ __forceinline__ int lds_ld(int width) { return width + 4; }

template <int ACT>
__device__ __forceinline__ float act_fwd(float v) {
  if (ACT == ACT_RELU) return v > 0.f ? v : 0.f;
  if (ACT == ACT_LRELU) return v > 0.f ? v : v * kLreluSlope;
  return v;
}

// ... 116 lines not shown
            if (4 * q + j < tail_n_) wtail[n][j] = wt_p[(size_t)(n * 16) * ldw + j];
        }
      }
    }
#pragma unroll
    for (int p = 0; p < PF; ++p)
#pragma unroll
      for (int n = 0; n < NT; ++n)
        if ((p * NT + n) * nslices / kItems == i) ring[p][n] = frag(n, p);
  }
  __device__ __forceinline__ void preload(const float* __restrict__ Wm, int ldw_,
                                          const float* __restrict__ bias,
                                          const float* __restrict__ Wt, int tail_n) {
    bind(Wm, ldw_, bias, Wt, tail_n);
    preload_slice(0, 1);
    pin_vmem();
  }
};

struct NoPrefetch {
  __device__ __forceinline__ void preload_slice(int, int) {}
};

template <int RT, int IN, int OUT, int ACT, int WALIGN, bool PACKED, int RING, class NEXT>
__device__ __forceinline__ void layer_fwd_run(FwdW<IN, OUT, WALIGN, PACKED, RING>& w,
                                              const float* X, int ldx, float* Y, int ldy,
                                              const float* Xt, int ldt, NEXT& next) {
  constexpr int NT = OUT / 64, NIT = IN / 16;
  constexpr int PF = FwdW<IN, OUT, WALIGN, PACKED, RING>::PF;
  const int lane = threadIdx.x & 63, wave = threadIdx.x >> 6;
  const int c = lane & 15, q = lane >> 4;
  const int col0 = wave * (OUT / 4);
  const float* xp = X + c * ldx + 4 * q;

  constexpr int NA = (RT * NT == 1) ? 2 : 1;
  f32x4 acc[NA][RT][NT];
#pragma unroll
  for (int a = 0; a < NA; ++a)
#pragma unroll
    for (int r = 0; r < RT; ++r)
#pragma unroll
      for (int n = 0; n < NT; ++n) acc[a][r][n] = f32x4{0.f, 0.f, 0.f, 0.f};

  f32x4 av[2][RT];
#pragma unroll
  for (int r = 0; r < RT; ++r) av[0][r] = *reinterpret_cast<const f32x4*>(xp + r * 16 * ldx);
#pragma unroll
  for (int t = 0; t < NIT; ++t) {
    f32x4 bv[NT];
#pragma unroll
    for (int n = 0; n < NT; ++n) bv[n] = w.ring[t % PF][n];
    if (t + PF < NIT) {
#pragma unroll
      for (int n = 0; n < NT; ++n) w.ring[t % PF][n] = w.frag(n, t + PF);
    }
    next.preload_slice(t, NIT);
    if (t + 1 < NIT) {
#pragma unroll
      for (int r = 0; r < RT; ++r) av[(t + 1) & 1][r] = *reinterpret_cast<const f32x4*>(xp + r * 16 * ldx + 16 * (t + 1));
    } else if (Xt != nullptr) {
#pragma unroll
      for (int r = 0; r < RT; ++r) av[(t + 1) & 1][r] = *reinterpret_cast<const f32x4*>(Xt + (r * 16 + c) * ldt + 4 * q);
    }
    pin_vmem_lds();
#pragma unroll
    for (int s = 0; s < 4; ++s)
#pragma unroll
      for (int r = 0; r < RT; ++r)
#pragma unroll
        for (int n = 0; n < NT; ++n)
          acc[s % NA][r][n] = mfma16(av[t & 1][r][s], bv[n][s], acc[s % NA][r][n]);
  }
  if (Xt != nullptr) {
#pragma unroll
    for (int s = 0; s < 4; ++s)
#pragma unroll
      for (int r = 0; r < RT; ++r)
#pragma unroll
        for (int n = 0; n < NT; ++n)
          acc[s % NA][r][n] = mfma16(av[NIT & 1][r][s], w.wtail[n][s], acc[s % NA][r][n]);
  }
  if (NA == 2) {
#pragma unroll
    for (int r = 0; r < RT; ++r)
#pragma unroll
      for (int n = 0; n < NT; ++n) acc[0][r][n] += acc[NA - 1][r][n];
  }

#pragma unroll
  for (int n = 0; n < NT; ++n) {
    const int col = col0 + n * 16 + c;
#pragma unroll
    for (int r = 0; r < RT; ++r)
#pragma unroll
      for (int i = 0; i < 4; ++i) {
        const int row = r * 16 + 4 * q + i;
        Y[row * ldy + col] = act_fwd<ACT>(acc[0][r][n][i] + w.bias_r[n]);
      }
  }
}
template <int RT, int IN, int OUT, int ACT, int WALIGN, bool PACKED, int RING>
__device__ __forceinline__ void layer_fwd_run(FwdW<IN, OUT, WALIGN, PACKED, RING>& w,
                                              const float* X, int ldx, float* Y, int ldy,
                                              const float* Xt, int ldt) {
  NoPrefetch none;
  layer_fwd_run<RT, IN, OUT, ACT, WALIGN, PACKED, RING>(w, X, ldx, Y, ldy, Xt, ldt, none);
}

template <int IN, int OUT, bool PACKED, int RING = 96>
struct DgW {
  static constexpr int V = IN / 64;
  static constexpr int NIT = OUT / 16;
  static constexpr int PF0 = RING / (4 * V);
  static constexpr int PF = PF0 < NIT ? PF0 : NIT;
  float ring[PF][4][V];
  const float* wbase;
  int ldw;

  __device__ __forceinline__ void load_step(int t, float (&dst)[4][V]) const {
    if (PACKED) {
      const float* p = wbase + (size_t)t * 64 * (4 * V);
#pragma unroll
      for (int h = 0; h < V; ++h) {
        const f32x4 x = *reinterpret_cast<const f32x4*>(p + 4 * h);
#pragma unroll
        for (int e = 0; e < 4; ++e) dst[(4 * h + e) / V][(4 * h + e) % V] = x[e];
      }
      return;
    }
#pragma unroll
    for (int s = 0; s < 4; ++s) {
      const float* p = wbase + (size_t)(16 * t + s) * ldw;
      if (V == 2) {
        f32x2 v2 = *reinterpret_cast<const f32x2*>(p);
        dst[s][0] = v2[0];
        dst[s][V - 1] = v2[1];
      } else {
        dst[s][0] = *p;
      }
    }
  }

  __device__ __forceinline__ void bind(const float* __restrict__ W, int ldw_) {
    static_assert((IN == 64 || IN == 128) && OUT % 16 == 0, "layer_dgrad shape");
    const int lane = threadIdx.x & 63, wave = threadIdx.x >> 6;
    const int c = lane & 15, q = lane >> 4;
    ldw = ldw_;
    wbase = PACKED ? W + ((size_t)wave * NIT * 64 + lane) * (4 * V)
                   : W + (size_t)(4 * q) * ldw_ + wave * 16 * V + V * c;
  }
  __device__ __forceinline__ void preload_slice(int i, int nslices) {
#pragma unroll
    for (int p = 0; p < PF; ++p)
      if (p * nslices / PF == i) load_step(p, ring[p]);
  }
  __device__ __forceinline__ void preload(const float* __restrict__ W, int ldw_) {
    bind(W, ldw_);
    preload_slice(0, 1);
    pin_vmem();
  }
};

template <int RT, int IN, int OUT, int ACT, bool PACKED, int RING, class NEXT>
__device__ __forceinline__ void layer_dgrad_run(DgW<IN, OUT, PACKED, RING>& w, const float* dY, int ldd,
                                                float* H, int ldh, NEXT& next) {
  constexpr int V = IN / 64, NIT = OUT / 16;
  constexpr int PF = DgW<IN, OUT, PACKED, RING>::PF;
  const int lane = threadIdx.x & 63, wave = threadIdx.x >> 6;
  const int c = lane & 15, q = lane >> 4;
  const int colbase = wave * 16 * V + V * c;
  const float* dp = dY + c * ldd + 4 * q;

  constexpr int NA = (RT * V == 1) ? 2 : 1;
  f32x4 acc[NA][RT][V];
#pragma unroll
  for (int a = 0; a < NA; ++a)
#pragma unroll
    for (int r = 0; r < RT; ++r)
#pragma unroll
      for (int v = 0; v < V; ++v) acc[a][r][v] = f32x4{0.f, 0.f, 0.f, 0.f};

  f32x4 av[2][RT];
#pragma unroll
  for (int r = 0; r < RT; ++r) av[0][r] = *reinterpret_cast<const f32x4*>(dp + r * 16 * ldd);
#pragma unroll
  for (int t = 0; t < NIT; ++t) {
    float bv[4][V];
#pragma unroll
    for (int s = 0; s < 4; ++s)
#pragma unroll
      for (int v = 0; v < V; ++v) bv[s][v] = w.ring[t % PF][s][v];
    if (t + PF < NIT) w.load_step(t + PF, w.ring[t % PF]);
    next.preload_slice(t, NIT);
    if (t + 1 < NIT) {
#pragma unroll
      for (int r = 0; r < RT; ++r) av[(t + 1) & 1][r] = *reinterpret_cast<const f32x4*>(dp + r * 16 * ldd + 16 * (t + 1));
    }
    pin_vmem_lds();
#pragma unroll
    for (int s = 0; s < 4; ++s)
#pragma unroll
      for (int r = 0; r < RT; ++r)
#pragma unroll
        for (int v = 0; v < V; ++v) acc[s % NA][r][v] = mfma16(av[t & 1][r][s], bv[s][v], acc[s % NA][r][v]);
  }
  if (NA == 2) {
#pragma unroll
    for (int r = 0; r < RT; ++r)
#pragma unroll
      for (int v = 0; v < V; ++v) acc[0][r][v] += acc[NA - 1][r][v];
  }

#pragma unroll
  for (int r = 0; r < RT; ++r)
#pragma unroll
    for (int i = 0; i < 4; ++i) {
      float* hp = H + (r * 16 + 4 * q + i) * ldh + colbase;
#pragma unroll
      for (int v = 0; v < V; ++v) hp[v] = act_bwd<ACT>(hp[v], acc[0][r][v][i]);
    }
}
template <int RT, int IN, int OUT, int ACT, bool PACKED, int RING>
__device__ __forceinline__ void layer_dgrad_run(DgW<IN, OUT, PACKED, RING>& w, const float* dY, int ldd,
                                                float* H, int ldh) {
  NoPrefetch none;
  layer_dgrad_run<RT, IN, OUT, ACT, PACKED, RING>(w, dY, ldd, H, ldh, none);
}

template <int RT, int IN, int OUT>
__device__ __forceinline__ void layer_fwd_narrow(const float* X, int ldx,
                                                 const float* __restrict__ W,
                                                 const float* __restrict__ bias,
                                                 float* Y, int ldy) {
  constexpr int R = 16 * RT;
  constexpr int PARTS = kThreads / R;
  constexpr int NV = IN / 4 / PARTS;
  static_assert(IN % (4 * PARTS) == 0, "layer_fwd_narrow shape");
  const int row = threadIdx.x / PARTS, part = threadIdx.x % PARTS;
  float sum[OUT];
#pragma unroll
  for (int o = 0; o < OUT; ++o) sum[o] = 0.f;
#pragma unroll
  for (int m = 0; m < NV; ++m) {
    const int k = 4 * (part + PARTS * m);
    const f32x4 x = *reinterpret_cast<const f32x4*>(X + row * ldx + k);
#pragma unroll
    for (int o = 0; o < OUT; ++o) {
      const f32x4 w = *reinterpret_cast<const f32x4*>(W + (size_t)o * IN + k);
      sum[o] = fmaf(x[0], w[0], sum[o]);
      sum[o] = fmaf(x[1], w[1], sum[o]);
      sum[o] = fmaf(x[2], w[2], sum[o]);
      sum[o] = fmaf(x[3], w[3], sum[o]);
    }
  }
#pragma unroll
  for (int o = 0; o < OUT; ++o) {
#pragma unroll
    for (int d = PARTS / 2; d >= 1; d >>= 1) sum[o] += __shfl_xor(sum[o], d, 64);
  }
  if (part == 0) {
#pragma unroll
    for (int o = 0; o < OUT; ++o) Y[row * ldy + o] = sum[o] + bias[o];
  }
}

template <int RT, int IN, int OUT, int ACT>
__device__ __forceinline__ void layer_dgrad_narrow(const float* dY, int ldd,
                                                   const float* __restrict__ W,
                                                   float* H, int ldh) {
  constexpr int R = 16 * RT;
  constexpr int NV = R * IN / 4;
  for (int idx = threadIdx.x; idx < NV; idx += kThreads) {
    const int row = idx / (IN / 4), k = 4 * (idx % (IN / 4));
    f32x4 g = {0.f, 0.f, 0.f, 0.f};
#pragma unroll
    for (int o = 0; o < OUT; ++o) {
      const float d = dY[row * ldd + o];
      const f32x4 w = *reinterpret_cast<const f32x4*>(W + (size_t)o * IN + k);
      g[0] = fmaf(d, w[0], g[0]);
      g[1] = fmaf(d, w[1], g[1]);
      g[2] = fmaf(d, w[2], g[2]);
      g[3] = fmaf(d, w[3], g[3]);
    }
    f32x4* hp = reinterpret_cast<f32x4*>(H + row * ldh + k);
    f32x4 h = *hp;
    h[0] = act_bwd<ACT>(h[0], g[0]);
    h[1] = act_bwd<ACT>(h[1], g[1]);
    h[2] = act_bwd<ACT>(h[2], g[2]);
    h[3] = act_bwd<ACT>(h[3], g[3]);
    *hp = h;
  }
}

__device__ __forceinline__ void stg4_wt(float* base, uint32_t off, f32x4 v) {
  const uint64_t ub = reinterpret_cast<uint64_t>(base);
  const uint32_t hi = (uint32_t)__builtin_amdgcn_readfirstlane((int)(ub >> 32));
  const uint32_t lo = (uint32_t)__builtin_amdgcn_readfirstlane((int)(uint32_t)ub);
  const uint64_t sb = ((uint64_t)hi << 32) | (uint64_t)lo;
  const __amdgpu_buffer_rsrc_t rsrc =
      __builtin_amdgcn_make_buffer_rsrc(reinterpret_cast<float*>(sb), 0, 0x7fffffff, 0x00020000);
  __builtin_amdgcn_raw_buffer_store_b128(__builtin_bit_cast(u32x4, v), rsrc, (int)(off * 4u), 0, 16 );
}

template <int RT, int W, bool WT = false>
__device__ __forceinline__ void store_tile(float* __restrict__ dst, size_t gld,
                                           const float* src, int ld) {
  constexpr int R = 16 * RT;
  constexpr int NV = R * W / 4;
#ifdef NDP_EXP_NOSTORE
  if (gld == 0x7fffffff)
#endif
  for (int idx = threadIdx.x; idx < NV; idx += kThreads) {
    const int row = idx / (W / 4), k = 4 * (idx % (W / 4));
    const f32x4 v = *reinterpret_cast<const f32x4*>(src + row * ld + k);
    if constexpr (WT) stg4_wt(dst, (uint32_t)(row * (int)gld + k), v);
    else *reinterpret_cast<f32x4*>(dst + (size_t)row * gld + k) = v;
  }
}

template <int RT, int W>
struct TileRegs {
  static constexpr int NV = 16 * RT * W / 4;
  static constexpr int N = (NV + kThreads - 1) / kThreads;
  f32x4 v[N];
  __device__ __forceinline__ void load(const float* __restrict__ src, size_t gld) {
#pragma unroll
    for (int u = 0; u < N; ++u) {
      int idx = threadIdx.x + u * kThreads;
      idx = idx < NV ? idx : NV - 1;
      const int row = idx / (W / 4), k = 4 * (idx % (W / 4));
      v[u] = ldg4<4>(src + (size_t)row * gld + k);
    }
  }
  __device__ __forceinline__ void store(float* dst, int ld) const {
#pragma unroll
    for (int u = 0; u < N; ++u) {
      const int idx = threadIdx.x + u * kThreads;
      if (idx < NV) {
        const int row = idx / (W / 4), k = 4 * (idx % (W / 4));
        *reinterpret_cast<f32x4*>(dst + row * ld + k) = v[u];
      }
    }
  }
};

template <int RT, int W>
__device__ __forceinline__ void load_tile(float* dst, int ld,
                                          const float* __restrict__ src, size_t gld) {
  constexpr int R = 16 * RT;
  constexpr int NV = R * W / 4;
  for (int idx = threadIdx.x; idx < NV; idx += kThreads) {
    const int row = idx / (W / 4), k = 4 * (idx % (W / 4));
    *reinterpret_cast<f32x4*>(dst + row * ld + k) =
        *reinterpret_cast<const f32x4*>(src + (size_t)row * gld + k);
  }
}

template <int RT>
__device__ __forceinline__ void load_code_tile(float* dst, int ld,
                                               const float* __restrict__ code, int64_t ld_code,
                                               int rep, int64_t row0, int64_t m, bool vec4) {
  constexpr int R = 16 * RT;
  constexpr int NV = R * 64;
  for (int idx = threadIdx.x; idx < NV; idx += kThreads) {
    const int i = idx >> 6, k = 4 * (idx & 63);
    const int64_t row = row0 + i;
    f32x4 v = {0.f, 0.f, 0.f, 0.f};
    if (row < m) {
      const float* p = code + (row / rep) * ld_code + k;
      if (vec4) {
        v = *reinterpret_cast<const f32x4*>(p);
      } else {
        v[0] = p[0]; v[1] = p[1]; v[2] = p[2]; v[3] = p[3];
      }
    }
    *reinterpret_cast<f32x4*>(dst + i * ld + k) = v;
  }
}

__device__ __forceinline__ float wave_sum(float v) {
#pragma unroll
  for (int d = 32; d >= 1; d >>= 1) v += __shfl_xor(v, d, 64);
  return v;
}

__device__ __forceinline__ float block_sum(float v, float* red) {
  v = wave_sum(v);
  if ((threadIdx.x & 63) == 0) red[threadIdx.x >> 6] = v;
  __syncthreads();
  float r = 0.f;
  if (threadIdx.x == 0) {
    const int nw = blockDim.x >> 6;
    for (int w = 0; w < nw; ++w) r += red[w];
  }
  __syncthreads();
  return r;
}

}
```

ndivplanning_amd/csrc/ndp_kernels.hip:

```cpp
#include <hip/hip_runtime.h>
#include <math.h>
#include <stddef.h>
#include <stdint.h>

#include "ndp_device.h"

namespace ndp {

#ifdef NDP_STAMPS
__device__ unsigned long long* g_stamps = nullptr;
__device__ int g_stamp_kernel = 0;
#define NDP_STAMP_ON(id) (g_stamps != nullptr && (g_stamp_kernel == 0 || g_stamp_kernel == (id)))
#define NDP_STAMP_DECL __shared__ unsigned long long stamp_store_[64]; unsigned long long* stamp_lds_ = stamp_store_
#define NDP_STAMP_PTR stamp_lds_
#define NDP_STAMP(i)                                             \
  do {                                                           \
    if (threadIdx.x == 0) {                                      \
      stamp_lds_[2 * (i)] = clock64();                           \
      stamp_lds_[2 * (i) + 1] = wall_clock64();                  \
    }                                                            \
  } while (0)
#define NDP_STAMP_FLUSH(n, id)                                                              \
  do {                                                                                      \
    if (threadIdx.x == 0 && NDP_STAMP_ON(id))                                               \
// ... 755 lines not shown
        const int idx = threadIdx.x + u * kThreads;
        *reinterpret_cast<f32x4*>(XC + (idx >> 6) * 260 + 4 * (idx & 63)) = ct[u];
      }
    }
    NDP_STAMP(25);
    XT[threadIdx.x] = nv;
    *reinterpret_cast<f32x4*>(W5S + 4 * threadIdx.x) = w5r;
    if (threadIdx.x < 4) W5S[1024 + threadIdx.x] = b5r;
    W4S[threadIdx.x] = w4r;
    if (threadIdx.x == 0) W4S[256] = b4r;
    NDP_STAMP(26);
    __syncthreads();
    NDP_STAMP(1);
    float* CPG = XC + NRR * 260;
    float* CPD = CPG + NRR * 256;
    if (DD) {
      code_rows_dot<128, NRR>(g.pf1, XC, CPG);
      code_rows_dot<64, NRR>(d.pf1, XC, CPD);
      __syncthreads();
      fc1_from_code_rows<128, ACT_RELU, NRR>(CPG, g.b1, g.w1 + CODE, g.ld1, g.nz, XT, B1, 132,
                                             (int)(row0 % a.code_rep), a.code_rep);
    } else {
      gw2.bind(PK ? g.pf2 : g.w2, 128, g.b2, nullptr, 0);
      layer_fwd_run<1, 256, 128, ACT_RELU, 2, PK>(gw1, XC, 260, B1, 132, XT, TAILLD, gw2);
    }
    __syncthreads();
    NDP_STAMP(12);
    FwdW<64, 128, 4, PK, RG> gw3;
    gw3.bind(PK ? g.pf3 : g.w3, 64, g.b3, nullptr, 0);
    store_tile<1, 128, WT>(a.gh1 + row0 * 128, 128, B1, 132);
    layer_fwd_run<1, 128, 64, ACT_RELU, 4, PK>(gw2, B1, 132, B2, 68, nullptr, 0, gw3);
    __syncthreads();
    NDP_STAMP(13);
    FwdW<128, 256, 4, PK, RG> gw4;
    gw4.bind(PK ? g.pf4 : g.w4, 128, g.b4, nullptr, 0);
    NDP_STAMP(16);
    store_tile<1, 64, WT>(a.gh2 + row0 * 64, 64, B2, 68);
    NDP_STAMP(17);
    layer_fwd_run<1, 64, 128, ACT_RELU, 4, PK>(gw3, B2, 68, B1, 132, nullptr, 0, gw4);
    NDP_STAMP(18);
    __syncthreads();
    NDP_STAMP(14);
    if (DD) dw2.bind(PK ? d.pf2 : d.w2, 64, d.b2, nullptr, 0);
    else dw1.bind(PK ? d.pf1 : d.w1 + ADIM, 260, d.b1, d.w1, ADIM);
    NDP_STAMP(19);
    store_tile<1, 128, WT>(a.gh3 + row0 * 128, 128, B1, 132);
    NDP_STAMP(20);
    if (DD) layer_fwd_run<1, 128, 256, ACT_RELU, 4, PK>(gw4, B1, 132, B3, 260, nullptr, 0, dw2);
    else layer_fwd_run<1, 128, 256, ACT_RELU, 4, PK>(gw4, B1, 132, B3, 260, nullptr, 0, dw1);
    NDP_STAMP(21);
    __syncthreads();
    NDP_STAMP(15);
    store_tile<1, 256, WT>(a.gh4 + row0 * 256, 256, B3, 260);
    NDP_STAMP(22);
    layer_fwd_narrow<1, 256, 4>(B3, 260, W5S, W5S + 1024, A, 4);
    NDP_STAMP(23);
    __syncthreads();
    NDP_STAMP(2);
    for (int idx = threadIdx.x; idx < R * TAILLD; idx += kThreads) {
      const int i = idx / TAILLD, t = idx % TAILLD;
      const int64_t row = row0 + i;
      XT[idx] = (row < a.m && t < ADIM) ? A[i * 4 + t] : 0.f;
    }
    if (threadIdx.x < R) {
      const int64_t row = row0 + threadIdx.x;
      if (row < a.m)
        if constexpr (WT) stg4_wt(a.action_hat + row0 * 4, 4 * threadIdx.x, *reinterpret_cast<const f32x4*>(A + threadIdx.x * 4));
        else *reinterpret_cast<f32x4*>(a.action_hat + row * 4) = *reinterpret_cast<const f32x4*>(A + threadIdx.x * 4);
    }
    __syncthreads();
    NDP_STAMP(9);
    phase_a_d_part<PK, RG, NR>(a, false, tile, ntiles, dw1, dw2, CPD, XC, XT, B1, B2, L, DL, W4S, NDP_STAMP_PTR);
  } else {
    const int tile = (int)blockIdx.x - ntiles;
    const int64_t row0 = (int64_t)tile * R;
    dw1.preload(PK ? d.pf1 : d.w1 + ADIM, 260, d.b1, d.w1, ADIM);
    W4S[threadIdx.x] = d.w4[threadIdx.x];
    if (threadIdx.x == 0) W4S[256] = d.b4[0];
    for (int idx = threadIdx.x; idx < R * 64; idx += kThreads) {
      const int i = idx >> 6, k = 4 * (idx & 63);
      const int64_t row = row0 + i;
      f32x4 v = {0.f, 0.f, 0.f, 0.f};
      if (row < a.flat) v = *reinterpret_cast<const f32x4*>(a.code + row * CODE + k);
      *reinterpret_cast<f32x4*>(XC + i * 260 + k) = v;
    }
    for (int idx = threadIdx.x; idx < R * TAILLD; idx += kThreads) {
      const int i = idx / TAILLD, t = idx % TAILLD;
      const int64_t row = row0 + i;
      XT[idx] = (row < a.flat && t < ADIM) ? a.actions[row * ADIM + t] : 0.f;
    }
    __syncthreads();
    phase_a_d_part<PK, RG, 0>(a, true, tile, ntiles, dw1, dw2, nullptr, XC, XT, B1, B2, L, DL, W4S, NDP_STAMP_PTR);
  }
  (void)red;
  NDP_STAMP(8);
  NDP_STAMP_FLUSH(32, 5);
}

struct PhaseBArgs {
  GNet g; DNet d;
  const float* code; int code_rep;
  const float* action_hat;
  const float* nd_grad;
  int64_t m;
  float inv_m;
  const float *gh1, *gh2, *gh3, *gh4;
  float *dy1, *dy2, *dy3, *dy4, *dy5;
  float* loss_partials;
  float* dy1seg; int seg_s, seg_entries;
};

constexpr int phase_b_lds_floats(bool pre) {
  return 16 * (260 + TAILLD + 132 + 68 + 132 + 4 + 2) + 8 + 256 + kSW4 + kSW5 + (pre ? 16 * (260 + 132 + 68) : 0);
}

template <bool PK, int RG, bool PRE, int NR>
__global__ __launch_bounds__(kThreads, (RG >= 96 ? 2 : 3)) void k_phase_b(PhaseBArgs a_segment) {
  constexpr bool DD = NR > 0;
  constexpr int NRR = NR > 0 ? NR : 1;
  constexpr bool WT = wt_tiles(RG);
  const PhaseBArgs a = RG >= 96 ? load_kernargs<PhaseBArgs>() : a_segment;
  constexpr int R = 16;
  extern __shared__ __attribute__((aligned(16))) float smem[];
  float* XC = smem;
  float* XT = XC + R * 260;
  float* B1 = XT + R * TAILLD;
  float* B2 = B1 + R * 132;
  float* H1 = B2 + R * 68;
  float* DA = H1 + R * 132;
  float* L = DA + R * 4;
  float* DL = L + R;
  float* red = DL + R;
  float* W1A = red + 8;
  float* W4S = W1A + 256;
  float* W5S = W4S + kSW4;
  float* G4 = PRE ? W5S + kSW5 : XC;
  float* G3 = PRE ? G4 + R * 260 : B1;
  float* G2 = PRE ? G3 + R * 132 : B2;
  const int64_t row0 = (int64_t)blockIdx.x * R;
  const GNet& g = a.g;
  const DNet& d = a.d;
  NDP_STAMP_DECL;
  NDP_STAMP(0);

  FwdW<256, 64, 4, PK, RG> dw1;
  FwdW<64, 128, 4, PK, RG> dw2;
  f32x4 ct[R * 64 / kThreads];
  float av = 0.f;
  {
    if (DD) {
      load_code_rows<NRR>(XC, a.code, row0 / a.code_rep, (a.m + a.code_rep - 1) / a.code_rep);
    } else {
#pragma unroll
      for (int u = 0; u < R * 64 / kThreads; ++u) {
        const int idx = threadIdx.x + u * kThreads;
        const int i = idx >> 6, k = 4 * (idx & 63);
        const int64_t row = row0 + i;
        const bool ok = row < a.m;
        const f32x4 v = *reinterpret_cast<const f32x4*>(a.code + ((ok ? row : 0) / a.code_rep) * CODE + k);
        ct[u] = ok ? v : f32x4{0.f, 0.f, 0.f, 0.f};
      }
    }
    const int i = threadIdx.x / TAILLD, t = threadIdx.x % TAILLD;
    const int64_t row = row0 + i;
    if (row < a.m && t < ADIM) av = a.action_hat[row * ADIM + t];
  }
  const float w1a = d.w1[(threadIdx.x >> 2) * 260 + (threadIdx.x & 3)], w4r = d.w4[threadIdx.x], b4r = d.b4[0];
  const f32x4 w5r = *reinterpret_cast<const f32x4*>(g.w5 + 4 * threadIdx.x);
  pin_vmem();
  if (DD) dw2.preload(PK ? d.pf2 : d.w2, 64, d.b2, nullptr, 0);
  else dw1.preload(PK ? d.pf1 : d.w1 + ADIM, 260, d.b1, d.w1, ADIM);
  if (!DD) {
#pragma unroll
    for (int u = 0; u < R * 64 / kThreads; ++u) {
      const int idx = threadIdx.x + u * kThreads;
      *reinterpret_cast<f32x4*>(XC + (idx >> 6) * 260 + 4 * (idx & 63)) = ct[u];
    }
  }
  XT[threadIdx.x] = av;
  TileRegs<1, 128> t1;
  TileRegs<1, 256> t4;
  TileRegs<1, 128> t3;
  TileRegs<1, 64> t2;
  W1A[threadIdx.x] = w1a;
  W4S[threadIdx.x] = w4r;
  if (threadIdx.x == 0) W4S[256] = b4r;
  *reinterpret_cast<f32x4*>(W5S + 4 * threadIdx.x) = w5r;
  if (PRE) {
    t1.load(a.gh1 + row0 * 128, 128);
    t4.load(a.gh4 + row0 * 256, 256);
    t3.load(a.gh3 + row0 * 128, 128);
    t2.load(a.gh2 + row0 * 64, 64);
    pin_vmem();
  } else {
    load_tile<1, 128>(H1, 132, a.gh1 + row0 * 128, 128);
  }
  __syncthreads();
  NDP_STAMP(1);
  if (DD) {
    code_rows_dot<64, NRR>(d.pf1, XC, XC + NRR * 260);
    __syncthreads();
    fc1_from_code_rows<64, ACT_LRELU, NRR>(XC + NRR * 260, d.b1, d.w1, 260, ADIM, XT, B2, 68,
                                           (int)(row0 % a.code_rep), a.code_rep);
  } else {
    dw2.bind(PK ? d.pf2 : d.w2, 64, d.b2, nullptr, 0);
    layer_fwd_run<1, 256, 64, ACT_LRELU, 4, PK>(dw1, XC, 260, B2, 68, XT, TAILLD, dw2);
  }
  if (PRE) {
    t1.store(H1, 132);
    t4.store(G4, 260);
    t3.store(G3, 132);
    t2.store(G2, 68);
  }
  __syncthreads();
  FwdW<128, 256, 4, PK, RG> dw3;
  dw3.bind(PK ? d.pf3 : d.w3, 128, d.b3, nullptr, 0);
  layer_fwd_run<1, 64, 128, ACT_LRELU, 4, PK>(dw2, B2, 68, B1, 132, nullptr, 0, dw3);
  __syncthreads();
  DgW<128, 256, PK, RG> dg3;
  dg3.bind(PK ? d.pg3 : d.w3, 128);
  layer_fwd_run<1, 128, 256, ACT_LRELU, 4, PK>(dw3, B1, 132, XC, 260, nullptr, 0, dg3);
  __syncthreads();
  NDP_STAMP(2);
  layer_fwd_narrow<1, 256, 1>(XC, 260, W4S, W4S + 256, L, 1);
  __syncthreads();
  float lsum = 0.f;
  if (threadIdx.x < R) {
    const int64_t row = row0 + threadIdx.x;
    const float x = L[threadIdx.x];
    float dl = 0.f;
    if (row < a.m) {
      lsum = fmaxf(x, 0.f) - x + log1pf(expf(-fabsf(x)));
      dl = (1.f / (1.f + expf(-x)) - 1.f) * a.inv_m;
    }
    DL[threadIdx.x] = dl;
  }
  if (threadIdx.x < 64) {
    const float tot = wave_sum(lsum);
    if (threadIdx.x == 0) a.loss_partials[blockIdx.x] = tot;
  }
  __syncthreads();
  NDP_STAMP(3);
  layer_dgrad_narrow<1, 256, 1, ACT_LRELU>(DL, 1, W4S, XC, 260);
  __syncthreads();
  DgW<64, 128, PK, RG> dg2;
  dg2.bind(PK ? d.pg2 : d.w2, 64);
  layer_dgrad_run<1, 128, 256, ACT_LRELU, PK>(dg3, XC, 260, B1, 132, dg2);
  __syncthreads();
  DgW<128, 256, PK, RG> gg4;
  gg4.bind(PK ? g.pg4 : g.w4, 128);
  layer_dgrad_run<1, 64, 128, ACT_LRELU, PK>(dg2, B1, 132, B2, 68, gg4);
  __syncthreads();
  NDP_STAMP(4);
  {
    const int i = threadIdx.x >> 4, j = (threadIdx.x >> 2) & 3, part = threadIdx.x & 3;
    const int64_t row = row0 + i;
    const float ng = (part == 0 && row < a.m && a.nd_grad != nullptr) ? a.nd_grad[row * ADIM + j] : 0.f;
    float s = 0.f;
#pragma unroll
    for (int o = 16 * part; o < 16 * part + 16; ++o) s = fmaf(B2[i * 68 + o], W1A[o * 4 + j], s);
    s += __shfl_xor(s, 1, 64);
    s += __shfl_xor(s, 2, 64);
    if (part == 0) {
      s = row < a.m ? s + ng : 0.f;
      DA[i * ADIM + j] = s;
      a.dy5[row * ADIM + j] = s;
    }
  }
  __syncthreads();
  NDP_STAMP(5);

  if (!PRE) {
    load_tile<1, 256>(G4, 260, a.gh4 + row0 * 256, 256);
    load_tile<1, 128>(G3, 132, a.gh3 + row0 * 128, 128);
    load_tile<1, 64>(G2, 68, a.gh2 + row0 * 64, 64);
    __syncthreads();
  }
  NDP_STAMP(6);
  layer_dgrad_narrow<1, 256, 4, ACT_RELU>(DA, 4, W5S, G4, 260);
  __syncthreads();
  NDP_STAMP(7);
  DgW<64, 128, PK, RG> gg3;
  gg3.bind(PK ? g.pg3 : g.w3, 64);
  layer_dgrad_run<1, 128, 256, ACT_RELU, PK>(gg4, G4, 260, G3, 132, gg3);
  __syncthreads();
  NDP_STAMP(8);
  DgW<128, 64, PK, RG> gg2;
  gg2.bind(PK ? g.pg2 : g.w2, 128);
  store_tile<1, 256, WT>(a.dy4 + row0 * 256, 256, G4, 260);
  layer_dgrad_run<1, 64, 128, ACT_RELU, PK>(gg3, G3, 132, G2, 68, gg2);
  __syncthreads();
  NDP_STAMP(9);
  store_tile<1, 128, WT>(a.dy3 + row0 * 128, 128, G3, 132);
  layer_dgrad_run<1, 128, 64, ACT_RELU, PK>(gg2, G2, 68, H1, 132);
  __syncthreads();
  NDP_STAMP(10);
  store_tile<1, 64, WT>(a.dy2 + row0 * 64, 64, G2, 68);
  store_tile<1, 128, WT>(a.dy1 + row0 * 128, 128, H1, 132);
  store_segment_sums<128, 1>(H1, 132, a.dy1seg, row0, a.code_rep, a.seg_s, a.seg_entries, (int)blockIdx.x, (int)gridDim.x);
  NDP_STAMP(11);
  NDP_STAMP_FLUSH(12, 6);
}

__device__ __forceinline__ void adam_advance(int32_t* state, float lr, float b1, float b2) {
  const int32_t t = state[0] + 1;
  state[0] = t;
  const double bc1 = 1.0 - pow((double)b1, (double)t);
  const double bc2 = 1.0 - pow((double)b2, (double)t);
  reinterpret_cast<float*>(state)[1] = (float)((double)lr / bc1);
  reinterpret_cast<float*>(state)[2] = (float)sqrt(bc2);
}

enum { WG_FULL = 0, WG_SKINNY_B = 1, WG_SKINNY_A = 2, WG_WIDE = 3 };
constexpr int kWgradPrefetch = 8;

struct WgradJob {
  const float* A;
  const float* B;
  int lda, ldb;
  int a_cols, b_cols;
  int b_rowmod, b_rowdiv, b_rowmax;
  int b_vec;
  int dst_off, dst_ld;
  int bias_off;
  int kind;
  int rows, seg, seg_s, seg_k;
  int seg_wrap;
  int nchunks;
};
constexpr int kMaxJobs = 28;
struct WgradHead {
  int njobs;
  int nwide;
  int wide_chunks;
  int rows;
  float* slabs;
  int64_t slab_stride;
  int32_t* bump;
  float lr, beta1, beta2;
  int nchunks;
  NdivArgs nd;
};
struct WgradArgs : WgradHead {
  WgradJob job[kMaxJobs];
  int net_is_g;
  int nreg, reg_begin[4], reg_end[4];
  int wide_begin, wide_end;
};

#ifdef NDP_STAMPS
#define NDP_WSTAMP(i) do { if (threadIdx.x == 0) { wst[2 * (i)] = clock64(); wst[2 * (i) + 1] = wall_clock64(); } } while (0)
#else
#define NDP_WSTAMP(i) do { } while (0)
#endif

template <int MT, int NT, int KIND, bool WT>
__device__ __forceinline__ void wgrad_block(const WgradJob& jb, int rbeg, int rend, int row_last,
                                            float* slab, float* smem, unsigned long long* wst) {
  const int lane = threadIdx.x & 63, wave = threadIdx.x >> 6;
  const int c = lane & 15, q = lane >> 4;
  f32x4 acc[MT][NT];
  float bs[MT];
#pragma unroll
  for (int u = 0; u < MT; ++u) {
    bs[u] = 0.f;
#pragma unroll
    for (int v = 0; v < NT; ++v) acc[u][v] = f32x4{0.f, 0.f, 0.f, 0.f};
  }
  constexpr int PF = kWgradPrefetch;
  const bool seg_b = jb.seg != 0;
  const bool plain_b = !seg_b && jb.b_rowdiv == 1 && jb.b_rowmod == 0x7fffffff;
  const float b_inv = 1.0f / (float)(seg_b ? jb.seg_k : jb.b_rowdiv);
  const float s_inv = 1.0f / (float)(seg_b ? jb.seg_s : 1);
  const int nsteps = rend > rbeg ? (rend - rbeg) >> 4 : 0;
  const int row_first = rbeg + 4 * wave + q;
  const int ca = KIND == WG_SKINNY_A ? (c < jb.a_cols ? c : jb.a_cols - 1) : 4 * c;
  const int cb = KIND == WG_SKINNY_B ? (c < jb.b_cols ? c : jb.b_cols - 1) : 4 * c;
  const bool a_on = KIND != WG_SKINNY_A || c < jb.a_cols;
  const bool b_on = KIND != WG_SKINNY_B || c < jb.b_cols;
  f32x4 ra[PF], rb[PF];
  auto load_a = [&](int t) -> f32x4 {
    int row = row_first + 16 * t;
    row = row < row_last ? row : row_last;
    const float* p = jb.A + (size_t)row * jb.lda + ca;
    if (KIND == WG_SKINNY_A) {
      const float v = *p;
      return f32x4{a_on ? v : 0.f, 0.f, 0.f, 0.f};
    }
    return *reinterpret_cast<const f32x4*>(p);
  };
  auto load_b = [&](int t) -> f32x4 {
    int row = row_first + 16 * t;
    row = row < row_last ? row : row_last;
    int brow = row;
    if (seg_b) {
      const bool ident = jb.seg_wrap != 0 && row >= jb.seg_wrap;
      const int e = ident ? 0 : row;
      int tile = (int)((float)e * s_inv);
      tile = tile * jb.seg_s > e ? tile - 1 : tile;
      tile = (tile + 1) * jb.seg_s <= e ? tile + 1 : tile;
      const int x = 16 * tile;
      int f0 = (int)((float)x * b_inv);
      f0 = f0 * jb.seg_k > x ? f0 - 1 : f0;
      f0 = (f0 + 1) * jb.seg_k <= x ? f0 + 1 : f0;
      brow = ident ? row - jb.seg_wrap : f0 + (e - tile * jb.seg_s);
    } else if (!plain_b) {
      const int x = row >= jb.b_rowmod ? row - jb.b_rowmod : row;
      int qd = (int)((float)x * b_inv);
      qd = qd * jb.b_rowdiv > x ? qd - 1 : qd;
      qd = (qd + 1) * jb.b_rowdiv <= x ? qd + 1 : qd;
      brow = qd;
    }
    brow = brow < jb.b_rowmax ? brow : jb.b_rowmax;
    const float* p = jb.B + (size_t)brow * jb.ldb + cb;
    if (KIND == WG_SKINNY_B) {
      const float v = *p;
      return f32x4{b_on ? v : 0.f, 0.f, 0.f, 0.f};
    }
    if (jb.b_vec) return *reinterpret_cast<const f32x4*>(p);
    return f32x4{p[0], p[1], p[2], p[3]};
  };
  auto mma_step = [&](const f32x4& va, const f32x4& vb) {
#pragma unroll
    for (int u = 0; u < MT; ++u) {
      bs[u] += va[u];
#pragma unroll
      for (int v = 0; v < NT; ++v) acc[u][v] = mfma16(va[u], vb[v], acc[u][v]);
    }
  };
  NDP_WSTAMP(1);
#pragma unroll
  for (int p = 0; p < PF; ++p) {
    ra[p] = load_a(p);
    rb[p] = load_b(p);
  }
  pin_vmem();
  int t = 0;
  for (; t + PF <= nsteps; t += PF) {
#pragma unroll
    for (int p = 0; p < PF; ++p) {
      const f32x4 va = ra[p], vb = rb[p];
      ra[p] = load_a(t + p + PF);
      rb[p] = load_b(t + p + PF);
      pin_vmem();
      mma_step(va, vb);
    }
  }
  const int rem = nsteps - t;
#pragma unroll
  for (int p = 0; p < PF; ++p)
    if (p < rem) mma_step(ra[p], rb[p]);
  NDP_WSTAMP(2);
  constexpr int JR = KIND == WG_SKINNY_A ? 16 : 64;
  constexpr int KC = KIND == WG_SKINNY_B ? 16 : 64;
  float* mine = smem + wave * (JR * KC);
  float* bsh = smem + kWaves * (JR * KC);
#pragma unroll
  for (int u = 0; u < MT; ++u)
#pragma unroll
    for (int i = 0; i < 4; ++i) {
      const int j = KIND == WG_SKINNY_A ? (4 * q + i) : (4 * (4 * q + i) + u);
      if (KIND == WG_SKINNY_B) {
        mine[j * KC + c] = acc[u][0][i];
      } else {
        f32x4 t;
#pragma unroll
        for (int v = 0; v < NT; ++v) t[v] = acc[u][v][i];
        *reinterpret_cast<f32x4*>(mine + j * KC + 4 * c) = t;
      }
    }
#pragma unroll
  for (int u = 0; u < MT; ++u) {
    float s = bs[u];
    s += __shfl_xor(s, 16, 64);
    s += __shfl_xor(s, 32, 64);
    if (q == 0) bsh[wave * 64 + (KIND == WG_SKINNY_A ? c : 4 * c + u)] = s;
  }
  __syncthreads();
  NDP_WSTAMP(3);
  const int jn = jb.a_cols, kn = jb.b_cols;
  for (int e = threadIdx.x; e < JR * KC / 4; e += kThreads) {
    const int j = e / (KC / 4), k = 4 * (e % (KC / 4));
    f32x4 s = *reinterpret_cast<const f32x4*>(smem + j * KC + k);
#pragma unroll
    for (int w = 1; w < kWaves; ++w) s += *reinterpret_cast<const f32x4*>(smem + w * (JR * KC) + j * KC + k);
    if (j < jn) {
      float* d = slab + jb.dst_off + (size_t)j * jb.dst_ld + k;
      if (KIND != WG_SKINNY_B && ((jb.dst_ld | jb.dst_off) & 3) == 0) {
        if constexpr (WT) stg4_wt(slab + jb.dst_off, (uint32_t)(j * jb.dst_ld + k), s);
        else *reinterpret_cast<f32x4*>(d) = s;
      } else {
#pragma unroll
        for (int t = 0; t < 4; ++t)
          if (k + t < kn) d[t] = s[t];
      }
    }
  }
  if (jb.bias_off >= 0 && threadIdx.x < 64 && (int)threadIdx.x < jn) {
    const int j = threadIdx.x;
    slab[jb.bias_off + j] = bsh[j] + bsh[64 + j] + bsh[128 + j] + bsh[192 + j];
  }
}

constexpr int kWideR = 16;
constexpr int wide_slab_floats() { return kWideR * (128 + 128); }
constexpr int wgrad_wide_lds_floats() { return 3 * wide_slab_floats(); }
template <bool WT>
__device__ __forceinline__ void wgrad_wide(const WgradJob& jb, int rbeg, int rend, float* slab, float* smem) {
  typedef __attribute__((address_space(3))) void* lds_ptr_t;
  typedef const __attribute__((address_space(1))) void* glb_ptr_t;
  constexpr int AW = 128;
  constexpr int SLAB = wide_slab_floats();
  const int t = threadIdx.x, lane = t & 63, wave = t >> 6;
  const int c = lane & 15, q = lane >> 4;
  const int jt = wave >> 1, kt0 = wave & 1;
  f32x4 acc[4][4];
  float bs[4];
#pragma unroll
  for (int u = 0; u < 4; ++u) {
    bs[u] = 0.f;
#pragma unroll
    for (int v = 0; v < 4; ++v) acc[u][v] = f32x4{0.f, 0.f, 0.f, 0.f};
  }
  const int nslabs = rend > rbeg ? (rend - rbeg) / kWideR : 0;
  auto fetch = [&](int s) {
    float* buf = smem + (s % 3) * SLAB;
    const size_t r0 = (size_t)rbeg + (size_t)s * kWideR;
#pragma unroll
    for (int i = 0; i < 2; ++i) {
      const int pair = wave + 4 * i;
      __builtin_amdgcn_global_load_lds((glb_ptr_t)(jb.A + (r0 + 2 * pair + (lane >> 5)) * jb.lda + 4 * (lane & 31)),
                                       (lds_ptr_t)(buf + pair * 256), 16, 0, 0);
    }
#pragma unroll
    for (int i = 0; i < 2; ++i) {
      const int pair = wave + 4 * i;
      __builtin_amdgcn_global_load_lds((glb_ptr_t)(jb.B + (r0 + 2 * pair + (lane >> 5)) * jb.ldb + 4 * (lane & 31)),
                                       (lds_ptr_t)(buf + kWideR * AW + pair * 256), 16, 0, 0);
    }
  };
  if (nslabs > 0) fetch(0);
  if (nslabs > 1) fetch(1);
  for (int s = 0; s < nslabs; ++s) {
    if (s + 1 < nslabs) asm volatile("s_waitcnt vmcnt(4)" ::: "memory");
    else asm volatile("s_waitcnt vmcnt(0)" ::: "memory");
    __builtin_amdgcn_s_barrier();
    if (s + 2 < nslabs) fetch(s + 2);
    const float* As = smem + (s % 3) * SLAB + 64 * jt + 4 * c;
    const float* Bs = smem + (s % 3) * SLAB + kWideR * AW + 64 * kt0 + 4 * c;
#pragma unroll
    for (int st = 0; st < kWideR / 4; ++st) {
      const f32x4 va = *reinterpret_cast<const f32x4*>(As + (4 * st + q) * AW);
      const f32x4 vb = *reinterpret_cast<const f32x4*>(Bs + (4 * st + q) * 128);
#pragma unroll
      for (int u = 0; u < 4; ++u) {
        if (kt0 == 0) bs[u] += va[u];
#pragma unroll
        for (int v = 0; v < 4; ++v) acc[u][v] = mfma16(va[u], vb[v], acc[u][v]);
      }
    }
  }
#pragma unroll
  for (int u = 0; u < 4; ++u)
#pragma unroll
    for (int i = 0; i < 4; ++i) {
      const f32x4 o = {acc[u][0][i], acc[u][1][i], acc[u][2][i], acc[u][3][i]};
      if constexpr (WT) {
        stg4_wt(slab + jb.dst_off, (uint32_t)((64 * jt + 4 * (4 * q + i) + u) * jb.dst_ld + 64 * kt0 + 4 * c), o);
      } else {
        float* d = slab + jb.dst_off + (size_t)(64 * jt + 4 * (4 * q + i) + u) * jb.dst_ld + 64 * kt0 + 4 * c;
        *reinterpret_cast<f32x4*>(d) = o;
      }
    }
  if (jb.bias_off >= 0 && kt0 == 0) {
#pragma unroll
    for (int u = 0; u < 4; ++u) {
      float sum = bs[u];
      sum += __shfl_xor(sum, 16, 64);
      sum += __shfl_xor(sum, 32, 64);
      if (q == 0) slab[jb.bias_off + 64 * jt + 4 * c + u] = sum;
    }
  }
}

constexpr int wgrad_lds_floats() { return kWaves * 64 * 64 + kWaves * 64; }
constexpr int wgrad_wide_launch_lds_floats() { return wgrad_wide_lds_floats() > wgrad_lds_floats() ? wgrad_wide_lds_floats() : wgrad_lds_floats(); }

__device__ __forceinline__ void wgrad_fetch_args(WgradHead& a, WgradJob& jb, int& job_id, int& chunk) {
  typedef const __attribute__((address_space(4))) char* kbytes_t;
  static_assert(sizeof(WgradHead) <= 192 && offsetof(WgradArgs, job) % 8 == 0, "k_wgrad argument prefetch");
    kbytes_t kp = (kbytes_t)__builtin_amdgcn_kernarg_segment_ptr();
    uint32_t h0, h1, h2, hw0, hw1;
    asm volatile("s_load_dword %0, %5, 0x0\n\ts_load_dword %1, %5, 0x40\n\ts_load_dword %2, %5, 0x80\n\t"
                 "s_load_dword %3, %5, 0x4\n\ts_load_dword %4, %5, 0x8\n\ts_waitcnt lgkmcnt(0)"
                 : "=&s"(h0), "=&s"(h1), "=&s"(h2), "=&s"(hw0), "=&s"(hw1) : "s"(kp) : "memory");
    const int njobs = (int)h0;
    const int wide_blocks = (int)hw0 * (int)hw1;
    if ((int)blockIdx.x < wide_blocks) {
      job_id = njobs + (int)blockIdx.x / (int)hw1;
      chunk = (int)blockIdx.x % (int)hw1;
    } else {
      const int b = (int)blockIdx.x - wide_blocks;
      const int idx = b >> 3;
      job_id = idx % njobs;
      chunk = (b & 7) + 8 * (idx / njobs);
    }
    const uint32_t joff = (uint32_t)(offsetof(WgradArgs, job) + (size_t)job_id * sizeof(WgradJob));
    uint32_t j0, j1;
    asm volatile("s_load_dword %0, %2, %3\n\ts_load_dword %1, %2, %4\n\ts_waitcnt lgkmcnt(0)"
                 : "=&s"(j0), "=&s"(j1) : "s"(kp), "s"(joff), "s"(joff + (uint32_t)sizeof(WgradJob) - 4u) : "memory");
    uint64_t v = (uint64_t)kp;
    asm volatile("" : "+s"(v) : "s"(h0 | h1 | h2 | j0 | j1));
    __builtin_memcpy(&a, (kbytes_t)v, sizeof(WgradHead));
    __builtin_memcpy(&jb, (kbytes_t)v + joff, sizeof(WgradJob));
}

template <bool WIDE>
__device__ __forceinline__ void wgrad_body(float* smem) {
  WgradHead a;
  WgradJob jb;
  int job_id, chunk;
  wgrad_fetch_args(a, jb, job_id, chunk);
  const int slots = a.nwide * a.wide_chunks + 8 * ((a.nchunks + 7) / 8) * a.njobs;
  if ((int)blockIdx.x >= slots) {
    ndiv_block<4, 2>(a.nd, (int)blockIdx.x - slots, smem);
    return;
  }
  if (chunk >= jb.nchunks) return;
  const int jrows = jb.rows != 0 ? jb.rows : a.rows;
  const int jrpc = ((jrows + jb.nchunks - 1) / jb.nchunks + 15) & ~15;
  const int rbeg = chunk * jrpc;
  int rend = rbeg + jrpc;
  rend = rend < jrows ? rend : jrows;
  float* slab = a.slabs + (size_t)chunk * a.slab_stride;
  if (a.bump != nullptr && blockIdx.x == 0 && threadIdx.x == 0)
    adam_advance(a.bump, a.lr, a.beta1, a.beta2);
  const int kind = jb.kind;
#ifdef NDP_STAMPS
  __shared__ unsigned long long wst[32];
  NDP_WSTAMP(0);
#else
  unsigned long long* wst = nullptr;
#endif
  constexpr bool WT = WIDE ? kWtSlabsWide : kWtSlabs;
  if (WIDE && kind == WG_WIDE) wgrad_wide<WT>(jb, rbeg, rend, slab, smem);
  else if (kind == WG_FULL) wgrad_block<4, 4, WG_FULL, WT>(jb, rbeg, rend, jrows - 1, slab, smem, wst);
  else if (kind == WG_SKINNY_B) wgrad_block<4, 1, WG_SKINNY_B, WT>(jb, rbeg, rend, jrows - 1, slab, smem, wst);
  else wgrad_block<1, 4, WG_SKINNY_A, WT>(jb, rbeg, rend, jrows - 1, slab, smem, wst);
#ifdef NDP_STAMPS
  NDP_WSTAMP(4);
  if (threadIdx.x == 0 && NDP_STAMP_ON(4))
    for (int i_ = 0; i_ < 10; ++i_) g_stamps[(size_t)blockIdx.x * 64 + i_] = wst[i_];
#endif
}

__global__ __launch_bounds__(kThreads) void k_wgrad(WgradArgs a_segment) {
  extern __shared__ __attribute__((aligned(16))) float smem[];
  (void)a_segment;
  wgrad_body<false>(smem);
}
__global__ __launch_bounds__(kThreads, 2) void k_wgrad_wide(WgradArgs a_segment) {
  extern __shared__ __attribute__((aligned(16))) float smem[];
  (void)a_segment;
  wgrad_body<true>(smem);
}

struct LossTerm {
  const float* partials; int count; float scale; int slot;
};
constexpr int kP2PRanks = 8;
constexpr int kP2PCapD = 58368;
constexpr int kP2PCapG = 86016;
constexpr int kP2PBlocks = kP2PCapG / kThreads;
constexpr int64_t kP2PFlagOff = 64;
constexpr int64_t kP2PInboxD = kP2PFlagOff + 2ll * kP2PRanks * kP2PBlocks;
constexpr int64_t kP2PInboxG = kP2PInboxD + (int64_t)kP2PRanks * 2 * kP2PCapD;
constexpr int64_t kP2PWords = kP2PInboxG + (int64_t)kP2PRanks * 2 * kP2PCapG;

struct P2PArgs {
  int world, rank, net;
  long long timeout_ticks;
  uint32_t* region[kP2PRanks];
};

__device__ __forceinline__ float p2p_sum(const P2PArgs& x, float g, int64_t p, bool valid, uint32_t step) {
  const int W = x.world, me = x.rank;
  const int64_t cap = x.net == 0 ? kP2PCapD : kP2PCapG;
  const int64_t inbox = x.net == 0 ? kP2PInboxD : kP2PInboxG;
  const int64_t par = (int64_t)(step & 1u) * cap;
  if (valid) {
    const int64_t at = inbox + (int64_t)me * 2 * cap + par + p;
#pragma unroll
    for (int r = 0; r < kP2PRanks; ++r)
      if (r < W && r != me)
        __hip_atomic_store(reinterpret_cast<float*>(x.region[r]) + at, g, __ATOMIC_RELAXED, __HIP_MEMORY_SCOPE_SYSTEM);
  }
  __builtin_amdgcn_fence(__ATOMIC_RELEASE, "workgroup");
  asm volatile("s_waitcnt vmcnt(0)" ::: "memory");
  __syncthreads();
  const int t = threadIdx.x;
  if (t < W && t != me) {
    const int64_t fbase = kP2PFlagOff + (int64_t)x.net * kP2PRanks * kP2PBlocks + blockIdx.x;
    __hip_atomic_store(x.region[t] + fbase + (int64_t)me * kP2PBlocks, step, __ATOMIC_RELAXED, __HIP_MEMORY_SCOPE_SYSTEM);
    uint32_t* status = x.region[me];
    const uint32_t* flag = x.region[me] + fbase + (int64_t)t * kP2PBlocks;
    if (__hip_atomic_load(status, __ATOMIC_RELAXED, __HIP_MEMORY_SCOPE_SYSTEM) == 0u) {
      const long long t0 = wall_clock64();
      while ((int32_t)(__hip_atomic_load(flag, __ATOMIC_RELAXED, __HIP_MEMORY_SCOPE_SYSTEM) - step) < 0) {
        if (wall_clock64() - t0 > x.timeout_ticks) {
          const uint32_t seen = __hip_atomic_load(flag, __ATOMIC_RELAXED, __HIP_MEMORY_SCOPE_SYSTEM);
          uint32_t expected = 0u;
          if (__hip_atomic_compare_exchange_strong(status, &expected, (uint32_t)(1 + t), __ATOMIC_RELAXED,
                                                   __ATOMIC_RELAXED, __HIP_MEMORY_SCOPE_SYSTEM)) {
            __hip_atomic_store(status + 1, (uint32_t)blockIdx.x, __ATOMIC_RELAXED, __HIP_MEMORY_SCOPE_SYSTEM);
            __hip_atomic_store(status + 2, (uint32_t)x.net, __ATOMIC_RELAXED, __HIP_MEMORY_SCOPE_SYSTEM);
            __hip_atomic_store(status + 3, step, __ATOMIC_RELAXED, __HIP_MEMORY_SCOPE_SYSTEM);
            __hip_atomic_store(status + 4, seen, __ATOMIC_RELAXED, __HIP_MEMORY_SCOPE_SYSTEM);
            __hip_atomic_store(status + 5, (uint32_t)t, __ATOMIC_RELAXED, __HIP_MEMORY_SCOPE_SYSTEM);
            __hip_atomic_store(status + 6, (uint32_t)(wall_clock64() - t0), __ATOMIC_RELAXED, __HIP_MEMORY_SCOPE_SYSTEM);
          }
          break;
        }
        __builtin_amdgcn_s_sleep(2);
      }
    }
  }
  __syncthreads();
  float v[kP2PRanks];
  const float* own = reinterpret_cast<const float*>(x.region[me]) + inbox + par + p;
#pragma unroll
  for (int r = 0; r < kP2PRanks; ++r)
    v[r] = __hip_atomic_load(own + (int64_t)(r < W ? r : me) * 2 * cap, __ATOMIC_RELAXED, __HIP_MEMORY_SCOPE_SYSTEM);
  float s = 0.f;
#pragma unroll
  for (int r = 0; r < kP2PRanks; ++r)
    if (r < W) s += (r == me) ? g : v[r];
  (void)valid;
  return s;
}

struct ReduceArgs {
  const float* slabs; int nchunks; int64_t slab_stride; int64_t n;
  int nregions; int reg_begin[4], reg_end[4], reg_slabs[4];
  P2PArgs p2p;
  float* grad;
  float *params, *exp_avg, *exp_avg_sq;
  const int32_t* step;
  float lr, beta1, beta2, eps;
  LossTerm loss[3]; int nloss;
  float* losses; float* loss_sums;
  PackSpec pack;
};

__device__ __forceinline__ void adam_update(float& p, float g, float& m, float& v,
                                            float step_size, float bc2_sqrt, float b1, float b2, float eps) {
  m = m + (g - m) * (1.f - b1);
  v = v * b2 + (1.f - b2) * g * g;
  const float denom = sqrtf(v) / bc2_sqrt + eps;
  p = p - step_size * (m / denom);
}

template <bool P2P>
__global__ __launch_bounds__(kThreads) void k_reduce_adam(ReduceArgs a) {
  __shared__ float sh[8];
  const int64_t p = (int64_t)blockIdx.x * kThreads + threadIdx.x;
  const bool live = p < a.n;
  const bool upd = live && a.params != nullptr;
  float g = 0.f;
  float pv = 0.f, m = 0.f, v = 0.f, step_size = 0.f, bc2_sqrt = 1.f;
  if (upd) {
    pv = a.params[p]; m = a.exp_avg[p]; v = a.exp_avg_sq[p];
    step_size = reinterpret_cast<const float*>(a.step)[1];
    bc2_sqrt = reinterpret_cast<const float*>(a.step)[2];
  }
  if (live) {
    const float* sp = a.slabs + p;
    int nch = a.nchunks;
#pragma unroll
    for (int r = 0; r < 4; ++r)
      if (r < a.nregions && p >= a.reg_begin[r] && p < a.reg_end[r]) nch = a.reg_slabs[r];
    constexpr int NB = P2P ? 16 : 32;
    for (int ch = 0; ch < nch; ch += NB) {
      float t[NB];
#pragma unroll
      for (int u = 0; u < NB; ++u) t[u] = (ch + u < nch) ? sp[(size_t)(ch + u) * a.slab_stride] : 0.f;
#pragma unroll
      for (int u = 0; u < NB; ++u) g += t[u];
    }
  }
  if constexpr (P2P) g = p2p_sum(a.p2p, g, p, live, (uint32_t)a.step[0]);
  if (live && a.grad != nullptr) a.grad[p] = g;
  if (upd) {
    adam_update(pv, g, m, v, step_size, bc2_sqrt, a.beta1, a.beta2, a.eps);
    a.params[p] = pv;
    a.exp_avg[p] = m;
    a.exp_avg_sq[p] = v;
    if (a.pack.packed != nullptr) pack_store(a.pack, (int)p, pv);
  }
  if (blockIdx.x == gridDim.x - 1) {
#pragma unroll
    for (int t = 0; t < 3; ++t) {
      if (t >= a.nloss) break;
      const LossTerm lt = a.loss[t];
      float s = 0.f;
      for (int i = threadIdx.x; i < lt.count; i += kThreads) s += lt.partials[i];
      s = block_sum(s, sh + 4);
      if (threadIdx.x == 0) {
        s *= lt.scale;
        a.losses[lt.slot] = s;
        if (a.loss_sums != nullptr) a.loss_sums[lt.slot] += s;
      }
    }
  }
}

__global__ void k_adam_advance(int32_t* state, float lr, float b1, float b2) { adam_advance(state, lr, b1, b2); }

struct AdamArgs {
  float *params, *exp_avg, *exp_avg_sq; const float* grad; int64_t n;
  const int32_t* step; float lr, beta1, beta2, eps;
  PackSpec pack;
};
__global__ __launch_bounds__(kThreads) void k_adam(AdamArgs a) {
  const float step_size = reinterpret_cast<const float*>(a.step)[1];
  const float bc2_sqrt = reinterpret_cast<const float*>(a.step)[2];
  const int64_t p = (int64_t)blockIdx.x * kThreads + threadIdx.x;
  if (p < a.n) {
    float pv = a.params[p], m = a.exp_avg[p], v = a.exp_avg_sq[p];
    adam_update(pv, a.grad[p], m, v, step_size, bc2_sqrt, a.beta1, a.beta2, a.eps);
    a.params[p] = pv;
    a.exp_avg[p] = m;
    a.exp_avg_sq[p] = v;
    if (a.pack.packed != nullptr) pack_store(a.pack, (int)p, pv);
  }
}

__global__ __launch_bounds__(kThreads) void k_sum_partials(const float* partials, int count,
                                                           float scale, float* out) {
  __shared__ float red[4];
  float s = 0.f;
  for (int i = threadIdx.x; i < count; i += kThreads) s += partials[i];
  s = block_sum(s, red);
  if (threadIdx.x == 0) *out = s * scale;
}

__global__ __launch_bounds__(kThreads) void k_philox(float* out, int64_t n, uint64_t seed,
                                                     const int32_t* offset_dev) {
  const int64_t idx = (int64_t)blockIdx.x * kThreads + threadIdx.x;
  if (idx >= n) return;
  const uint32_t off = offset_dev != nullptr ? (uint32_t)*offset_dev : 0u;
  out[idx] = philox_uniform((uint64_t)idx, seed, off);
}

}

#include "ndp_capi.inc"
#include "ndp_encoder.inc"
#include "ndp_forward_model.inc"
#include "ndp_autoencoder.inc"
#include "ndp_eval.inc"
#include "ndp_jpeg.inc"
```

ndivplanning_amd/trainer.py:

```python
import ctypes

import torch

from . import _capi, dp
from .models.gan import ACTION_DIM, CODE_DIM, Decoder, Discriminator


def _on_own_device(fn):
    import functools

    @functools.wraps(fn)
    def wrapper(self, *args, **kw):
        with torch.cuda.device(self.device):
            return fn(self, *args, **kw)
    return wrapper


class GanTrainer:
    def __init__(self, decoder: Decoder, discriminator: Discriminator, *, flat: int, num_sample: int,
                 lr: float = 2e-4, betas=(0.5, 0.999), eps: float = 1e-8, pairwise_div_factor: float = 0.1,
                 discrim_steps: int = 1, flat_global: int = None, reduce_fn=None, use_graph: bool = True,
                 noise_seed: int = 0, steps_per_launch: int = 1, p2p=None, copy_stream=None):
        self.lib = _capi.load()
        self.decoder, self.discriminator = decoder, discriminator
        self.noise_dim = decoder.noise_dim
        self.flat, self.k = int(flat), int(num_sample)
        self.flat_global = int(flat_global) if flat_global is not None else self.flat
        self.m = self.flat * self.k
        self.discrim_steps = int(discrim_steps)
        if p2p is not None and reduce_fn is not None:
            raise ValueError("give either p2p (in-kernel exchange) or reduce_fn (collective between the phases)")
        self.reduce_fn = reduce_fn
        self.p2p = p2p
        self.use_graph = bool(use_graph) and reduce_fn is None
        self.noise_seed = int(noise_seed)
        self.nslots = max(1, int(steps_per_launch))
        self.g_flat = decoder.flat_parameters()
        self.d_flat = discriminator.flat_parameters()
        dev = self.g_flat.device
        if dev.type != "cuda":
            raise _capi.NdpError("GanTrainer needs the networks on a ROCm GPU (got %s); there is no CPU path" % dev)
        self.device = dev
        f32 = dict(dtype=torch.float32, device=dev)
        self.g_grad, self.d_grad = torch.zeros_like(self.g_flat), torch.zeros_like(self.d_flat)
        self.g_m, self.g_v = torch.zeros_like(self.g_flat), torch.zeros_like(self.g_flat)
        self.d_m, self.d_v = torch.zeros_like(self.d_flat), torch.zeros_like(self.d_flat)
        self.g_step = torch.zeros(4, dtype=torch.int32, device=dev)
        self.d_step = torch.zeros(4, dtype=torch.int32, device=dev)
        self.losses_dev = torch.zeros(4, **f32)
        self.loss_sums = torch.zeros(4, **f32)
        mpad = _capi.pad_rows(self.m)
        self.action_hat = torch.zeros(mpad, ACTION_DIM, **f32)
        self.codes_slots = torch.zeros(self.nslots, self.flat, CODE_DIM, **f32)
        self.actions_slots = torch.zeros(self.nslots, self.flat, ACTION_DIM, **f32)
        self.noise_slots = torch.zeros(self.nslots, self.flat, self.k, self.noise_dim, **f32)
        self.codes, self.actions, self.noise = self.codes_slots[0], self.actions_slots[0], self.noise_slots[0]
        self.cfg = _capi.StepConfig(
            noise_dim=self.noise_dim, num_sample=self.k, flat=self.flat,
            inv_m_global=1.0 / float(self.flat_global * self.k), pairwise_div_factor=float(pairwise_div_factor),
            lr=float(lr), beta1=float(betas[0]), beta2=float(betas[1]), eps=float(eps),
            fuse_adam=0 if reduce_fn is not None else 1, device_noise=0, noise_seed=self.noise_seed,
            p2p=p2p.pointer() if p2p is not None else None)
        nws = self.lib.ndp_step_workspace_floats(ctypes.byref(self.cfg))
        if nws <= 0:
            raise _capi.NdpError("bad step configuration (flat=%d, num_sample=%d)" % (self.flat, self.k))
        self.workspace = torch.empty(nws, **f32)
        self._graphs = None
        self._copy_stream = copy_stream
        self._stage = None
        self._alt_slots = None
        self._device_noise_now = False
        self._d_calls = 0
        with torch.cuda.device(self.device):
            self._bind()

    def _versions(self):
        return (self.g_flat._version, self.d_flat._version,
                tuple(p._version for p in self.decoder._param_list()),
                tuple(p._version for p in self.discriminator._param_list()))

    def _repack(self):
        _capi.check(self.lib.ndp_step_pack_params(ctypes.byref(self.cfg), ctypes.byref(self.buf), _capi.stream_ptr(self.device)),
                    "ndp_step_pack_params")
        self._seen_versions = self._versions()

    def _bind(self):
        self.g_flat = self.decoder.flat_parameters()
        self.d_flat = self.discriminator.flat_parameters()
        p = _capi.ptr
        self.buf = _capi.StepBuffers(
            g_params=p(self.g_flat), g_grad=p(self.g_grad), g_exp_avg=p(self.g_m), g_exp_avg_sq=p(self.g_v),
            d_params=p(self.d_flat), d_grad=p(self.d_grad), d_exp_avg=p(self.d_m), d_exp_avg_sq=p(self.d_v),
            g_step=p(self.g_step), d_step=p(self.d_step), losses=p(self.losses_dev), loss_sums=p(self.loss_sums),
            action_hat=p(self.action_hat), workspace=p(self.workspace))
        self.buf_nosum = _capi.StepBuffers()
        ctypes.memmove(ctypes.byref(self.buf_nosum), ctypes.byref(self.buf), ctypes.sizeof(_capi.StepBuffers))
        self.buf_nosum.loss_sums = None
        self._repack()

    def _inputs(self, slot, sset=0):
        if sset == 0:
            return self.codes_slots[slot], self.actions_slots[slot], self.noise_slots[slot]
        if self._alt_slots is None:
            self._alt_slots = (torch.zeros_like(self.codes_slots), torch.zeros_like(self.actions_slots),
                               torch.zeros_like(self.noise_slots))
        return tuple(t[slot] for t in self._alt_slots)

    def _phase_a(self, first, device_noise=False, last=True, slot=0, sset=0):
        self.cfg.device_noise = 1 if device_noise else 0
        buf = self.buf if last else self.buf_nosum
        codes, actions, noise = self._inputs(slot, sset)
        _capi.check(self.lib.ndp_step_d_grads(ctypes.byref(self.cfg), ctypes.byref(buf), _capi.ptr(codes),
                                              _capi.ptr(actions), _capi.ptr(noise), 1 if first else 0,
                                              _capi.stream_ptr(self.device)), "ndp_step_d_grads")

    def _phase_b(self, slot=0, sset=0):
        codes, actions, noise = self._inputs(slot, sset)
        _capi.check(self.lib.ndp_step_g_grads(ctypes.byref(self.cfg), ctypes.byref(self.buf), _capi.ptr(codes),
                                              _capi.ptr(actions), _capi.ptr(noise), _capi.stream_ptr(self.device)),
                    "ndp_step_g_grads")

    def _segments(self, device_noise, slot=0, sset=0):
        segs = []

        def seg_d(first, last):
            def run():
                self._phase_a(first, device_noise, last, slot, sset)
            return run

        def seg_g():
            self._phase_b(slot, sset)

        def d_update():
            _capi.check(self.lib.ndp_step_apply_adam(ctypes.byref(self.cfg), ctypes.byref(self.buf), 0,
                                                     _capi.stream_ptr(self.device)), "ndp_step_apply_adam")

        def g_update():
            _capi.check(self.lib.ndp_step_apply_adam(ctypes.byref(self.cfg), ctypes.byref(self.buf), 1,
                                                     _capi.stream_ptr(self.device)), "ndp_step_apply_adam")

        fused = self.reduce_fn is None
        for it in range(self.discrim_steps):
            segs.append((seg_d(it == 0, it == self.discrim_steps - 1), None if fused else self.d_grad))
            if not fused:
                segs.append((d_update, None))
        segs.append((seg_g, None if fused else self.g_grad))
        if not fused:
            segs.append((g_update, None))
        return segs

    @_on_own_device
    def d_grads(self, first):
        self._d_calls = 0 if first else self._d_calls + 1
        self._phase_a(first, self._device_noise_now, self._d_calls == self.discrim_steps - 1)
        return self.d_grad

    @_on_own_device
    def apply_d(self, grad):
        _capi.check(self.lib.ndp_step_apply_adam(ctypes.byref(self.cfg), ctypes.byref(self.buf), 0,
                                                 _capi.stream_ptr(self.device)), "ndp_step_apply_adam")

    @_on_own_device
    def g_grads(self):
        self._phase_b()
        return self.g_grad

    @_on_own_device
    def apply_g(self, grad):
        _capi.check(self.lib.ndp_step_apply_adam(ctypes.byref(self.cfg), ctypes.byref(self.buf), 1,
                                                 _capi.stream_ptr(self.device)), "ndp_step_apply_adam")

    def _run_eager(self, device_noise):
        if self.reduce_fn is not None:
            self._device_noise_now = device_noise
            dp.run_step(self, self.reduce_fn, self.discrim_steps)
            return
        for fn, _ in self._segments(device_noise):
            fn()
        if self.p2p is not None:
            self.p2p.poll()

    def _build_graphs(self, device_noise, nsteps=1, sset=0):
        tmp = torch.empty(4, dtype=torch.float32, device=self.device)
        _capi.check(self.lib.ndp_uniform_noise(_capi.ptr(tmp), 4, 0, None, _capi.stream_ptr(self.device)), "warm-up")
        torch.cuda.synchronize(self.device)
        plan, run = [], []
        all_segments = [sg for slot in range(nsteps) for sg in self._segments(device_noise, slot, sset)]
        for fn, grad in all_segments:
            run.append(fn)
            if grad is not None:
                plan.append((run, grad))
                run = []
        if run:
            plan.append((run, None))
        graphs = []
        for fns, grad in plan:
            g = torch.cuda.CUDAGraph()
            with torch.cuda.graph(g):
                for fn in fns:
                    fn()
            graphs.append((g, grad))
        return graphs

    @_on_own_device
    def step(self, codes=None, actions=None, noise=None):
        self._check_bindings()
        if codes is not None:
            self.codes.copy_(codes.reshape(self.flat, CODE_DIM), non_blocking=True)
        if actions is not None:
            self.actions.copy_(actions.reshape(self.flat, ACTION_DIM), non_blocking=True)
        device_noise = noise is None
        if not device_noise:
            self.noise.copy_(noise.reshape(self.flat, self.k, self.noise_dim), non_blocking=True)
        if not self.use_graph:
            self._run_eager(device_noise)
            return
        self._replay(device_noise, 1)

    def _replay(self, device_noise, nsteps, sset=0):
        key = (bool(device_noise), nsteps, sset)
        if self._graphs is None:
            self._graphs = {}
        if key not in self._graphs:
            self._graphs[key] = self._build_graphs(device_noise, nsteps, sset)
        for g, grad in self._graphs[key]:
            g.replay()
            if grad is not None:
                self.reduce_fn(grad)
        if self.p2p is not None:
            self.p2p.poll()

    @_on_own_device
    def step_many(self, codes=None, actions=None, noise=None, count=None):
        self._check_bindings()
        n = self.nslots if count is None else int(count)
        if not 1 <= n <= self.nslots:
            raise ValueError("count=%r outside 1..%d" % (count, self.nslots))
        if codes is not None:
            self.codes_slots[:n].copy_(codes.reshape(n, self.flat, CODE_DIM), non_blocking=True)
        if actions is not None:
            self.actions_slots[:n].copy_(actions.reshape(n, self.flat, ACTION_DIM), non_blocking=True)
        device_noise = noise is None
        if not device_noise:
            self.noise_slots[:n].copy_(noise.reshape(n, self.flat, self.k, self.noise_dim), non_blocking=True)
        if self.use_graph and self.reduce_fn is None:
            self._replay(device_noise, n)
            return
        for slot in range(n):
            for fn, grad in self._segments(device_noise, slot):
                fn()
                if grad is not None:
                    self.reduce_fn(grad)

    @_on_own_device
    def step_many_from_host(self, codes_host, actions_host):
        self._check_bindings()
        n = self.nslots
        if not (codes_host.is_pinned() and actions_host.is_pinned()):
            raise ValueError("step_many_from_host needs pinned host tensors (torch.Tensor.pin_memory())")
        if self._stage is None:
            self._stage = {"stream": self._copy_stream or torch.cuda.Stream(self.device), "next": 0,
                           "uploaded": [torch.cuda.Event(), torch.cuda.Event()],
                           "read": [torch.cuda.Event(), torch.cuda.Event()]}
            self._inputs(0, 1)
            self._stage["stream"].wait_stream(torch.cuda.current_stream(self.device))
        st = self._stage
        sset = st["next"]
        st["next"] = 1 - sset
        codes = self.codes_slots if sset == 0 else self._alt_slots[0]
        actions = self.actions_slots if sset == 0 else self._alt_slots[1]
        main = torch.cuda.current_stream(self.device)
        with torch.cuda.stream(st["stream"]):
            st["stream"].wait_event(st["read"][sset])
            codes.copy_(codes_host.reshape(n, self.flat, CODE_DIM), non_blocking=True)
            actions.copy_(actions_host.reshape(n, self.flat, ACTION_DIM), non_blocking=True)
            st["uploaded"][sset].record(st["stream"])
        main.wait_event(st["uploaded"][sset])
        if self.use_graph and self.reduce_fn is None:
            self._replay(True, n, sset)
        else:
            for slot in range(n):
                for fn, grad in self._segments(True, slot, sset):
                    fn()
                    if grad is not None:
                        self.reduce_fn(grad)
        st["read"][sset].record(main)

    def _check_bindings(self):
        if self.g_flat.data_ptr() != self.decoder.flat_parameters().data_ptr() or \
                self.d_flat.data_ptr() != self.discriminator.flat_parameters().data_ptr():
            self._bind()
            self._graphs = None
        elif self._versions() != self._seen_versions:
            self._repack()

    def losses(self):
        v = self.losses_dev.tolist()
        return v[0], v[1], v[2]

    def pop_loss_sums(self):
        v = self.loss_sums.tolist()
        self.loss_sums.zero_()
        return v[0], v[1], v[2]

    @_on_own_device
    def load_adam_state(self, g_state, d_state):
        for (m, v, step), st in (((self.g_m, self.g_v, self.g_step), g_state), ((self.d_m, self.d_v, self.d_step), d_state)):
            m.copy_(st["m"])
            v.copy_(st["v"])
            step.zero_()
            step[0] = int(st["t"])
```

Before: 13190 steps/s.

## Fuse slab reduction and Adam update into the wgrad kernel via in-launch combine

When every wgrad workgroup (plus any fused ndiv blocks) can be resident at once, the weight-gradient kernel now writes its slabs with write-through stores. Per-job arrival counters then let the workgroups themselves reduce the slabs, apply Adam, pack params and sum losses. This removes the separate k_reduce_adam launch for both the D and G updates in single-GPU fused-Adam mode. The cost is a device-wide spin wait that relies on all workgroups being co-resident, guarded by an occupancy check and a timeout status word that the trainer checks on the host. Slab stores are also slower because they are write-through.

```diff
diff --git a/include/ndp.h b/include/ndp.h
--- a/include/ndp.h
+++ b/include/ndp.h
@@ -88,6 +88,10 @@
 } ndp_step_buffers;
 
 int64_t ndp_step_workspace_floats(const ndp_step_config *cfg);
+
+int64_t ndp_step_sync_offset(const ndp_step_config *cfg);
+int ndp_step_wgrad_combine(const ndp_step_config *cfg, int which, int wg_per_cu, int cus, int32_t *eligible,
+                           int64_t *live_workgroups);
 
 int ndp_step_d_grads(const ndp_step_config *cfg, const ndp_step_buffers *buf,
                      const float *codes, const float *actions, float *noise,
diff --git a/ndivplanning_amd/_capi.py b/ndivplanning_amd/_capi.py
--- a/ndivplanning_amd/_capi.py
+++ b/ndivplanning_amd/_capi.py
@@ -67,6 +67,8 @@
     "ndp_adam_step": (c_int, [c_void_p, c_void_p, c_void_p, c_void_p, c_int64, c_void_p,
                               c_float, c_float, c_float, c_float, c_void_p]),
     "ndp_step_workspace_floats": (c_int64, [POINTER(StepConfig)]),
+    "ndp_step_sync_offset": (c_int64, [POINTER(StepConfig)]),
+    "ndp_step_wgrad_combine": (c_int, [POINTER(StepConfig), c_int, c_int, c_int, POINTER(c_int32), POINTER(c_int64)]),
     "ndp_step_d_grads": (c_int, [POINTER(StepConfig), POINTER(StepBuffers), c_void_p, c_void_p, c_void_p,
                                  c_int, c_void_p]),
     "ndp_step_g_grads": (c_int, [POINTER(StepConfig), POINTER(StepBuffers), c_void_p, c_void_p, c_void_p,
diff --git a/ndivplanning_amd/csrc/ndp_capi.inc b/ndivplanning_amd/csrc/ndp_capi.inc
--- a/ndivplanning_amd/csrc/ndp_capi.inc
+++ b/ndivplanning_amd/csrc/ndp_capi.inc
@@ -90,6 +90,8 @@
   return flags[dev];
 }
 static_assert(phase_a_lds_floats() * 4 * 3 <= 160 * 1024, "phase A: three workgroups per CU at large M");
+
+static int g_wgrad_resident[kMaxDevices][2];
 
 static void set_attrs() {
   std::call_once(device_once(g_attr_once), [] {
@@ -117,6 +119,12 @@
 #undef NDP_ALLOW_B
     allow_lds(k_ndiv<4, 2>, 64 * 1024);
     allow_lds(k_ndiv<16, 16>, 64 * 1024);
+    int dev = 0, per_cu = 0, cus = 0;
+    if (hipGetDevice(&dev) == hipSuccess && dev >= 0 && dev < kMaxDevices &&
+        hipOccupancyMaxActiveBlocksPerMultiprocessor(&per_cu, k_wgrad, kThreads, wgrad_lds_floats() * 4) == hipSuccess &&
+        hipDeviceGetAttribute(&cus, hipDeviceAttributeMultiprocessorCount, dev) == hipSuccess) {
+      g_wgrad_resident[dev][0] = per_cu; g_wgrad_resident[dev][1] = cus;
+    }
   });
 }
 
@@ -453,10 +461,33 @@
 
 struct AdamHyper { float lr, beta1, beta2; };
 
+static bool wgrad_combine_fits(int njobs, const int* live_chunks, int nwide, int nd_blocks, int wg_per_cu, int cus,
+                               int64_t* live_out) {
+  int64_t live = nd_blocks;
+  for (int i = 0; i < njobs; ++i) live += live_chunks[i];
+  if (live_out) *live_out = live;
+  return nwide == 0 && njobs <= kMaxJobs && wg_per_cu > 0 && cus > 0 && live <= (int64_t)wg_per_cu * cus;
+}
+static bool wgrad_combine_fits(const WgradArgs& w, int nchunks, int light, int nd_blocks, int wg_per_cu, int cus,
+                               int64_t* live_out) {
+  int live_chunks[kMaxJobs];
+  for (int i = 0; i < w.njobs; ++i) live_chunks[i] = w.job[i].nchunks ? nchunks : light;
+  return wgrad_combine_fits(w.njobs, live_chunks, w.nwide, nd_blocks, wg_per_cu, cus, live_out);
+}
+static bool wgrad_combine_fits_device(const WgradArgs& w, int nchunks, int light, int nd_blocks) {
+  set_attrs();
+  int dev = 0;
+  if (hipGetDevice(&dev) != hipSuccess || dev < 0 || dev >= kMaxDevices) return false;
+  return wgrad_combine_fits(w, nchunks, light, nd_blocks, g_wgrad_resident[dev][0], g_wgrad_resident[dev][1], nullptr);
+}
+
 static int launch_wgrad(WgradArgs& w, int64_t rows, int nchunks, int light, float* slabs, int64_t slab_stride,
-                        int32_t* bump, const AdamHyper& hp, const NdivArgs* nd, int nd_blocks, hipStream_t st) {
+                        int32_t* bump, const AdamHyper& hp, const NdivArgs* nd, int nd_blocks, hipStream_t st,
+                        const WgradCombine* cb = nullptr) {
   set_attrs();
   w.rows = (int)rows;
+  w.combine = cb != nullptr;
+  if (cb) w.cb = *cb; else memset(&w.cb, 0, sizeof(w.cb));
   for (int i = 0; i < w.njobs; ++i) w.job[i].nchunks = w.job[i].nchunks ? nchunks : light;
   for (int i = 0; i < w.nwide; ++i) w.job[w.njobs + i].nchunks = w.wide_chunks;
   w.slabs = slabs; w.slab_stride = slab_stride; w.bump = bump;
@@ -488,6 +519,21 @@
     hipLaunchKernelGGL(k_reduce_adam<false>, grid, dim3(kThreads), 0, st, r);
   return check_launch("k_reduce_adam");
 }
+
+static WgradCombine combine_args(const ReduceArgs& r, uint32_t* sync, int net) {
+  WgradCombine cb;
+  memset(&cb, 0, sizeof(cb));
+  cb.status = sync;
+  cb.counters = sync + kSyncStatusWords + net * kMaxJobs * kSyncLineWords;
+  cb.timeout_ticks = 100000000ll;
+  cb.grad = r.grad; cb.params = r.params; cb.exp_avg = r.exp_avg; cb.exp_avg_sq = r.exp_avg_sq;
+  cb.eps = r.eps; cb.nloss = r.nloss;
+  for (int i = 0; i < 3; ++i) cb.loss[i] = r.loss[i];
+  cb.losses = r.losses; cb.loss_sums = r.loss_sums;
+  cb.pack = r.pack;
+  return cb;
+}
+static bool step_may_combine(const ndp_step_config* c) { return c->fuse_adam && (c->p2p == nullptr || c->p2p->world <= 1); }
 
 static int ndiv_block_threads(int k) { return k <= 64 ? 64 : kThreads; }
 static int ndiv_rows_per_block(int k, int threads) { return threads / k; }
@@ -580,7 +626,7 @@
                            const float* noise, int64_t ld_noise, int64_t m, const GActs& acts,
                            const float* d_action, const float* d_action2, float* ws_base,
                            ReduceArgs& red, int32_t* bump, const AdamHyper& hp, hipStream_t st,
-                           const float* dy1seg = nullptr) {
+                           const float* dy1seg = nullptr, uint32_t* combine_sync = nullptr) {
   const int64_t mpad = pad_rows(m);
   GBwdWs ws = g_bwd_ws(ws_base, mpad, nz);
   GBwdArgs b;
@@ -596,6 +642,10 @@
   }
   WgradArgs w;
   build_g_jobs(w, nz, ws, acts, code, ld_code, code_rep, noise, ld_noise, m, dy1seg);
+  if (combine_sync != nullptr && wgrad_combine_fits_device(w, ws.nchunks, ws.light, 0)) {
+    const WgradCombine cb = combine_args(red, combine_sync, 1);
+    return launch_wgrad(w, mpad, ws.nchunks, ws.light, ws.slabs, ws.slab_stride, bump, hp, nullptr, 0, st, &cb);
+  }
   rc = launch_wgrad(w, mpad, ws.nchunks, ws.light, ws.slabs, ws.slab_stride, bump, hp, nullptr, 0, st);
   if (rc) return rc;
   red.slabs = ws.slabs; red.nchunks = ws.nchunks; red.slab_stride = ws.slab_stride;
@@ -704,6 +754,8 @@
   GActs acts; float* gb; float* db; float* d_action; float* nd_grad; float* nd_part; int64_t nd_count;
   float* g_packed; float* d_packed;
   float* d_seg; float* g_seg;
+  uint32_t* sync;
+  int64_t sync_off;
 };
 static bool several_per_cu(int64_t workgroups) { return workgroups > 256; }
 
@@ -735,7 +787,10 @@
   const int64_t o_ds = o;
   o += (seg_entries(mpad, c->num_sample) + step_real_pad(c)) * 64;
   const int64_t o_gs = o; o += seg_entries(mpad, c->num_sample) * 128;
+  o = (o + 31) / 32 * 32;
+  const int64_t o_sync = o; o += kSyncWords;
   if (out) {
+    out->sync = reinterpret_cast<uint32_t*>(base + o_sync); out->sync_off = o_sync;
     out->g_packed = base + o_gp; out->d_packed = base + o_dp;
     out->d_seg = base + o_ds; out->g_seg = base + o_gs;
     out->acts = g_acts(base + o_acts, mpad);
@@ -868,6 +923,47 @@
 int64_t ndp_step_workspace_floats(const ndp_step_config* cfg) {
   if (!cfg || cfg->flat < 1 || cfg->num_sample < 1 || cfg->num_sample > NDP_MAX_SAMPLES) return 0;
   return step_floats(cfg, nullptr, nullptr);
+}
+
+int64_t ndp_step_sync_offset(const ndp_step_config* cfg) {
+  if (!cfg || cfg->flat < 1 || cfg->num_sample < 1 || cfg->num_sample > NDP_MAX_SAMPLES) return 0;
+  StepWs ws;
+  step_floats(cfg, &ws, reinterpret_cast<float*>(static_cast<uintptr_t>(4096)));
+  return ws.sync_off;
+}
+
+int ndp_step_wgrad_combine(const ndp_step_config* c, int which, int wg_per_cu, int cus, int32_t* eligible,
+                           int64_t* live_workgroups) {
+  NDP_CHECK_ARG(c && eligible && live_workgroups, "ndp_step_wgrad_combine: null pointer");
+  NDP_CHECK_ARG(which == 0 || which == 1, "ndp_step_wgrad_combine: which must be 0 (D) or 1 (G)");
+  NDP_CHECK_ARG(c->noise_dim >= 1 && c->noise_dim <= NDP_MAX_NOISE_DIM && c->num_sample >= 1 &&
+                c->num_sample <= NDP_MAX_SAMPLES && c->flat >= 1 && c->flat * c->num_sample < (1ll << 28),
+                "ndp_step_wgrad_combine: bad configuration");
+  if (wg_per_cu < 0 || cus < 0) {
+    set_attrs();
+    int dev = 0;
+    NDP_HIP(hipGetDevice(&dev), "ndp_step_wgrad_combine");
+    NDP_CHECK_ARG(dev >= 0 && dev < kMaxDevices, "ndp_step_wgrad_combine: device index %d", dev);
+    wg_per_cu = g_wgrad_resident[dev][0]; cus = g_wgrad_resident[dev][1];
+  }
+  const int K = c->num_sample, nz = c->noise_dim;
+  const int64_t m = c->flat * K, mpad = pad_rows(m);
+  float* base = reinterpret_cast<float*>(static_cast<uintptr_t>(4096));
+  StepWs ws;
+  step_floats(c, &ws, base);
+  WgradArgs w;
+  bool ok;
+  if (which == 0) {
+    const DBwdWs dw = d_bwd_ws_rows(ws.db, step_d_rows(c));
+    build_d_jobs(w, dw, base, CODE, K, m, mpad, ws.d_seg, step_real_pad(c), step_d_rows(c));
+    ok = wgrad_combine_fits(w, dw.nchunks, dw.light, step_ndiv_fused(c) ? (int)ws.nd_count : 0, wg_per_cu, cus, live_workgroups);
+  } else {
+    const GBwdWs gw = g_bwd_ws(ws.gb, mpad, nz);
+    build_g_jobs(w, nz, gw, ws.acts, base, CODE, K, base, nz, m, ws.g_seg);
+    ok = wgrad_combine_fits(w, gw.nchunks, gw.light, 0, wg_per_cu, cus, live_workgroups);
+  }
+  *eligible = ok && step_may_combine(c) ? 1 : 0;
+  return NDP_OK;
 }
 
 int ndp_step_d_grads(const ndp_step_config* c, const ndp_step_buffers* b, const float* codes, const float* actions,
@@ -933,9 +1029,6 @@
   }
   WgradArgs wa;
   build_d_jobs(wa, dw, codes, CODE, K, m, mpad, run_g_forward ? ws.d_seg : nullptr, rpad, run_g_forward ? step_d_rows(c) : 2 * mpad);
-  rc = launch_wgrad(wa, run_g_forward ? step_d_rows(c) : 2 * mpad, dw.nchunks, dw.light, dw.slabs, dw.slab_stride, b->d_step,
-                    AdamHyper{c->lr, c->beta1, c->beta2}, fused_ndiv ? &nd : nullptr, (int)ws.nd_count, st);
-  if (rc) return rc;
   ReduceArgs red;
   memset(&red, 0, sizeof(red));
   red.slabs = dw.slabs; red.nchunks = dw.nchunks; red.slab_stride = dw.slab_stride; red.n = d_layout().total;
@@ -952,6 +1045,17 @@
   red.loss[0].partials = dw.lossp; red.loss[0].count = loss_count; red.loss[0].scale = c->inv_m_global;
   red.loss[0].slot = 0;
   red.nloss = 1; red.losses = b->losses; red.loss_sums = b->loss_sums;
+  const int64_t wrows = run_g_forward ? step_d_rows(c) : 2 * mpad;
+  const int nd_blocks = fused_ndiv ? (int)ws.nd_count : 0;
+  const AdamHyper hp{c->lr, c->beta1, c->beta2};
+  if (run_g_forward && step_may_combine(c) && wgrad_combine_fits_device(wa, dw.nchunks, dw.light, nd_blocks)) {
+    const WgradCombine cb = combine_args(red, ws.sync, 0);
+    return launch_wgrad(wa, wrows, dw.nchunks, dw.light, dw.slabs, dw.slab_stride, b->d_step, hp,
+                        fused_ndiv ? &nd : nullptr, nd_blocks, st, &cb);
+  }
+  rc = launch_wgrad(wa, wrows, dw.nchunks, dw.light, dw.slabs, dw.slab_stride, b->d_step, hp,
+                    fused_ndiv ? &nd : nullptr, nd_blocks, st);
+  if (rc) return rc;
   return launch_reduce(red, st);
 }
 
@@ -1016,7 +1120,8 @@
   red.loss[1].slot = 2;
   red.nloss = 2; red.losses = b->losses; red.loss_sums = b->loss_sums;
   return g_backward_impl(g_net(b->g_params, nz, ws.g_packed), nz, codes, CODE, K, noise, nz, m, ws.acts, nullptr,
-                         nullptr, ws.gb, red, b->g_step, AdamHyper{c->lr, c->beta1, c->beta2}, st, ws.g_seg);
+                         nullptr, ws.gb, red, b->g_step, AdamHyper{c->lr, c->beta1, c->beta2}, st, ws.g_seg,
+                         step_may_combine(c) ? ws.sync : nullptr);
 }
 
 #ifdef NDP_STAMPS
@@ -1075,6 +1180,7 @@
   StepWs ws;
   step_floats(c, &ws, b->workspace);
   hipStream_t st = (hipStream_t)stream;
+  set_attrs();
   int rc = launch_pack(b->g_params, g_layout(c->noise_dim).total, g_pack_spec(c->noise_dim, ws.g_packed), st);
   if (rc) return rc;
   return launch_pack(b->d_params, d_layout().total, d_pack_spec(ws.d_packed), st);
diff --git a/ndivplanning_amd/csrc/ndp_device.h b/ndivplanning_amd/csrc/ndp_device.h
--- a/ndivplanning_amd/csrc/ndp_device.h
+++ b/ndivplanning_amd/csrc/ndp_device.h
@@ -442,6 +442,26 @@
   __builtin_amdgcn_raw_buffer_store_b128(__builtin_bit_cast(u32x4, v), rsrc, (int)(off * 4u), 0, 16 );
 }
 
+typedef __attribute__((address_space(1))) float gf32_t;
+typedef __attribute__((address_space(1))) uint32_t gu32_t;
+typedef __attribute__((address_space(1))) unsigned long long gu64_t;
+__device__ __forceinline__ void st_wt(float* p, float v) {
+  __hip_atomic_store((gf32_t*)p, v, __ATOMIC_RELAXED, __HIP_MEMORY_SCOPE_AGENT);
+}
+__device__ __forceinline__ void st_wt2(float* p, float v0, float v1) {
+  const unsigned long long x = ((unsigned long long)__builtin_bit_cast(uint32_t, v1) << 32) | __builtin_bit_cast(uint32_t, v0);
+  __hip_atomic_store((gu64_t*)p, x, __ATOMIC_RELAXED, __HIP_MEMORY_SCOPE_AGENT);
+}
+__device__ __forceinline__ float ldg_sc1(const float* base, uint32_t off) {
+  const uint64_t ub = reinterpret_cast<uint64_t>(base);
+  const uint32_t hi = (uint32_t)__builtin_amdgcn_readfirstlane((int)(ub >> 32));
+  const uint32_t lo = (uint32_t)__builtin_amdgcn_readfirstlane((int)(uint32_t)ub);
+  const uint64_t sb = ((uint64_t)hi << 32) | (uint64_t)lo;
+  const __amdgpu_buffer_rsrc_t rsrc =
+      __builtin_amdgcn_make_buffer_rsrc(reinterpret_cast<float*>(sb), 0, 0x7fffffff, 0x00020000);
+  return __builtin_bit_cast(float, __builtin_amdgcn_raw_buffer_load_b32(rsrc, (int)(off * 4u), 0, 16 ));
+}
+
 template <int RT, int W, bool WT = false>
 __device__ __forceinline__ void store_tile(float* __restrict__ dst, size_t gld,
                                            const float* src, int ld) {
diff --git a/ndivplanning_amd/csrc/ndp_kernels.hip b/ndivplanning_amd/csrc/ndp_kernels.hip
--- a/ndivplanning_amd/csrc/ndp_kernels.hip
+++ b/ndivplanning_amd/csrc/ndp_kernels.hip
@@ -1081,13 +1081,21 @@
   NDP_STAMP_FLUSH(12, 6);
 }
 
+template <bool WT = false>
 __device__ __forceinline__ void adam_advance(int32_t* state, float lr, float b1, float b2) {
   const int32_t t = state[0] + 1;
-  state[0] = t;
   const double bc1 = 1.0 - pow((double)b1, (double)t);
   const double bc2 = 1.0 - pow((double)b2, (double)t);
-  reinterpret_cast<float*>(state)[1] = (float)((double)lr / bc1);
-  reinterpret_cast<float*>(state)[2] = (float)sqrt(bc2);
+  const float step_size = (float)((double)lr / bc1), bc2_sqrt = (float)sqrt(bc2);
+  if constexpr (WT) {
+    st_wt(reinterpret_cast<float*>(state), __builtin_bit_cast(float, t));
+    st_wt(reinterpret_cast<float*>(state) + 1, step_size);
+    st_wt(reinterpret_cast<float*>(state) + 2, bc2_sqrt);
+  } else {
+    state[0] = t;
+    reinterpret_cast<float*>(state)[1] = step_size;
+    reinterpret_cast<float*>(state)[2] = bc2_sqrt;
+  }
 }
 
 enum { WG_FULL = 0, WG_SKINNY_B = 1, WG_SKINNY_A = 2, WG_WIDE = 3 };
@@ -1118,14 +1126,173 @@
   int32_t* bump;
   float lr, beta1, beta2;
   int nchunks;
+  int combine;
   NdivArgs nd;
+};
+struct LossTerm {
+  const float* partials; int count; float scale; int slot;
+};
+constexpr int kSyncStatusWords = 32, kSyncLineWords = 32;
+constexpr int kSyncWords = kSyncStatusWords + 2 * kMaxJobs * kSyncLineWords;
+struct WgradCombine {
+  uint32_t* status;
+  uint32_t* counters;
+  long long timeout_ticks;
+  float *grad, *params, *exp_avg, *exp_avg_sq;
+  float eps; int nloss;
+  LossTerm loss[3];
+  float *losses, *loss_sums;
+  PackSpec pack;
 };
 struct WgradArgs : WgradHead {
   WgradJob job[kMaxJobs];
+  WgradCombine cb;
   int net_is_g;
   int nreg, reg_begin[4], reg_end[4];
   int wide_begin, wide_end;
 };
+
+__device__ __forceinline__ void adam_update(float& p, float g, float& m, float& v,
+                                            float step_size, float bc2_sqrt, float b1, float b2, float eps) {
+  m = m + (g - m) * (1.f - b1);
+  v = v * b2 + (1.f - b2) * g * g;
+  const float denom = sqrtf(v) / bc2_sqrt + eps;
+  p = p - step_size * (m / denom);
+}
+__device__ __forceinline__ void adam_apply(int64_t p, float g, float pv, float m, float v, float step_size, float bc2_sqrt,
+                                           float b1, float b2, float eps, float* params, float* exp_avg,
+                                           float* exp_avg_sq, const PackSpec& pack) {
+  adam_update(pv, g, m, v, step_size, bc2_sqrt, b1, b2, eps);
+  params[p] = pv;
+  exp_avg[p] = m;
+  exp_avg_sq[p] = v;
+  if (pack.packed != nullptr) pack_store(pack, (int)p, pv);
+}
+__device__ __forceinline__ void loss_terms(const LossTerm* loss, int nloss, float* losses, float* loss_sums, float* red) {
+#pragma unroll
+  for (int t = 0; t < 3; ++t) {
+    if (t >= nloss) break;
+    const LossTerm lt = loss[t];
+    float s = 0.f;
+    for (int i = threadIdx.x; i < lt.count; i += kThreads) s += lt.partials[i];
+    s = block_sum(s, red);
+    if (threadIdx.x == 0) {
+      s *= lt.scale;
+      losses[lt.slot] = s;
+      if (loss_sums != nullptr) loss_sums[lt.slot] += s;
+    }
+  }
+}
+
+__device__ __forceinline__ uint32_t sync_load(uint32_t* p) {
+  return __hip_atomic_load((gu32_t*)p, __ATOMIC_RELAXED, __HIP_MEMORY_SCOPE_AGENT);
+}
+__device__ __forceinline__ uint32_t sync_add(uint32_t* p, uint32_t v) {
+  return __hip_atomic_fetch_add((gu32_t*)p, v, __ATOMIC_RELAXED, __HIP_MEMORY_SCOPE_AGENT);
+}
+__device__ __forceinline__ void sync_store(uint32_t* p, uint32_t v) {
+  __hip_atomic_store((gu32_t*)p, v, __ATOMIC_RELAXED, __HIP_MEMORY_SCOPE_AGENT);
+}
+__device__ __forceinline__ bool wgrad_wait(const WgradCombine& cb, int job_id, uint32_t target, int nch, float* smem) {
+  int* flag = reinterpret_cast<int*>(smem);
+  if (threadIdx.x == 0) {
+    uint32_t* cnt = cb.counters + job_id * kSyncLineWords;
+    int ok = 0;
+    if (sync_load(cb.status) == 0u) {
+      const long long t0 = wall_clock64();
+      for (;;) {
+        const uint32_t seen = sync_load(cnt);
+        if (seen == target) { ok = 1; break; }
+        if (wall_clock64() - t0 > cb.timeout_ticks) {
+          uint32_t expected = 0u;
+          if (__hip_atomic_compare_exchange_strong((gu32_t*)cb.status, &expected, (uint32_t)(1 + job_id), __ATOMIC_RELAXED,
+                                                   __ATOMIC_RELAXED, __HIP_MEMORY_SCOPE_AGENT)) {
+            sync_store(cb.status + 1, (uint32_t)blockIdx.x);
+            sync_store(cb.status + 2, seen);
+            sync_store(cb.status + 3, target);
+          }
+          break;
+        }
+        __builtin_amdgcn_s_sleep(2);
+      }
+    }
+    if (ok && sync_add(cnt + 1, 1u) == (uint32_t)(nch - 1)) {
+      sync_store(cnt, 0u);
+      sync_store(cnt + 1, 0u);
+    }
+    *flag = ok;
+  }
+  __syncthreads();
+  return *flag != 0;
+}
+
+template <int EB, int NB>
+__device__ __forceinline__ void wgrad_combine_run(const WgradHead& a, const WgradJob& jb, const WgradCombine& cb,
+                                                  int job_id, int chunk, float* smem) {
+  const int jn = jb.a_cols, kn = jb.b_cols, nch = jb.nchunks;
+  const int W = jn * kn, T = W + (jb.bias_off >= 0 ? jn : 0);
+  const int per = (T + nch - 1) / nch;
+  int s0 = chunk * per, iend = s0 + per;
+  iend = iend < T ? iend : T;
+  const uint32_t stride = (uint32_t)a.slab_stride;
+  float step_size = 0.f, bc2_sqrt = 1.f;
+  bool first = true;
+  do {
+    int p[EB];
+    bool on[EB];
+    float pv[EB], m[EB], v[EB], g[EB];
+#pragma unroll
+    for (int e = 0; e < EB; ++e) {
+      const int i = s0 + e * kThreads + (int)threadIdx.x;
+      on[e] = i < iend;
+      const int ii = on[e] ? i : T - 1;
+      const int j = ii / kn;
+      p[e] = ii < W ? jb.dst_off + j * jb.dst_ld + (ii - j * kn) : jb.bias_off + (ii - W);
+      pv[e] = cb.params[p[e]];
+      m[e] = cb.exp_avg[p[e]];
+      v[e] = cb.exp_avg_sq[p[e]];
+      g[e] = 0.f;
+    }
+    if (first) {
+      if (!wgrad_wait(cb, job_id, (uint32_t)(nch + 1), nch, smem)) return;
+      step_size = ldg_sc1(reinterpret_cast<const float*>(a.bump), 1);
+      bc2_sqrt = ldg_sc1(reinterpret_cast<const float*>(a.bump), 2);
+      first = false;
+    }
+    for (int ch = 0; ch < nch; ch += NB) {
+      float t[EB][NB];
+#pragma unroll
+      for (int e = 0; e < EB; ++e)
+#pragma unroll
+        for (int u = 0; u < NB; ++u) {
+          const int c2 = ch + u < nch ? ch + u : nch - 1;
+          t[e][u] = ldg_sc1(a.slabs, (uint32_t)c2 * stride + (uint32_t)p[e]);
+        }
+#pragma unroll
+      for (int e = 0; e < EB; ++e)
+#pragma unroll
+        for (int u = 0; u < NB; ++u) g[e] += ch + u < nch ? t[e][u] : 0.f;
+    }
+#pragma unroll
+    for (int e = 0; e < EB; ++e)
+      if (on[e]) {
+        if (cb.grad != nullptr) cb.grad[p[e]] = g[e];
+        adam_apply(p[e], g[e], pv[e], m[e], v[e], step_size, bc2_sqrt, a.beta1, a.beta2, cb.eps, cb.params, cb.exp_avg,
+                   cb.exp_avg_sq, cb.pack);
+      }
+    s0 += EB * kThreads;
+  } while (s0 < iend);
+}
+
+__device__ __forceinline__ void wgrad_combine(const WgradHead& a, const WgradJob& jb, const WgradCombine& cb,
+                                              int job_id, int chunk, float* smem) {
+  asm volatile("s_waitcnt vmcnt(0)" ::: "memory");
+  __syncthreads();
+  if (threadIdx.x == 0) sync_add(cb.counters + job_id * kSyncLineWords, 1u);
+  if (jb.nchunks <= 8) wgrad_combine_run<4, 8>(a, jb, cb, job_id, chunk, smem);
+  else if (jb.nchunks <= 16) wgrad_combine_run<2, 16>(a, jb, cb, job_id, chunk, smem);
+  else wgrad_combine_run<1, 32>(a, jb, cb, job_id, chunk, smem);
+}
 
 #ifdef NDP_STAMPS
 #define NDP_WSTAMP(i) do { if (threadIdx.x == 0) { wst[2 * (i)] = clock64(); wst[2 * (i) + 1] = wall_clock64(); } } while (0)
@@ -1135,7 +1302,7 @@
 
 template <int MT, int NT, int KIND, bool WT>
 __device__ __forceinline__ void wgrad_block(const WgradJob& jb, int rbeg, int rend, int row_last,
-                                            float* slab, float* smem, unsigned long long* wst) {
+                                            float* slab, float* smem, unsigned long long* wst, bool wt_all) {
   const int lane = threadIdx.x & 63, wave = threadIdx.x >> 6;
   const int c = lane & 15, q = lane >> 4;
   f32x4 acc[MT][NT];
@@ -1268,6 +1435,18 @@
       if (KIND != WG_SKINNY_B && ((jb.dst_ld | jb.dst_off) & 3) == 0) {
         if constexpr (WT) stg4_wt(slab + jb.dst_off, (uint32_t)(j * jb.dst_ld + k), s);
         else *reinterpret_cast<f32x4*>(d) = s;
+      } else if (wt_all) {
+        if (((jb.dst_ld | jb.dst_off) & 1) == 0) {
+#pragma unroll
+          for (int t = 0; t < 4; t += 2) {
+            if (k + t + 1 < kn) st_wt2(d + t, s[t], s[t + 1]);
+            else if (k + t < kn) st_wt(d + t, s[t]);
+          }
+        } else {
+#pragma unroll
+          for (int t = 0; t < 4; ++t)
+            if (k + t < kn) st_wt(d + t, s[t]);
+        }
       } else {
 #pragma unroll
         for (int t = 0; t < 4; ++t)
@@ -1277,7 +1456,9 @@
   }
   if (jb.bias_off >= 0 && threadIdx.x < 64 && (int)threadIdx.x < jn) {
     const int j = threadIdx.x;
-    slab[jb.bias_off + j] = bsh[j] + bsh[64 + j] + bsh[128 + j] + bsh[192 + j];
+    const float b = bsh[j] + bsh[64 + j] + bsh[128 + j] + bsh[192 + j];
+    if (wt_all) st_wt(slab + jb.bias_off + j, b);
+    else slab[jb.bias_off + j] = b;
   }
 }
 
@@ -1395,7 +1576,7 @@
 }
 
 template <bool WIDE>
-__device__ __forceinline__ void wgrad_body(float* smem) {
+__device__ __forceinline__ void wgrad_body(float* smem, const WgradCombine& cb) {
   WgradHead a;
   WgradJob jb;
   int job_id, chunk;
@@ -1412,8 +1593,17 @@
   int rend = rbeg + jrpc;
   rend = rend < jrows ? rend : jrows;
   float* slab = a.slabs + (size_t)chunk * a.slab_stride;
-  if (a.bump != nullptr && blockIdx.x == 0 && threadIdx.x == 0)
+  const bool combine = !WIDE && a.combine != 0;
+  if (combine) {
+    if (blockIdx.x == 0 && threadIdx.x < 64) {
+      if (threadIdx.x == 0) adam_advance<true>(a.bump, a.lr, a.beta1, a.beta2);
+      asm volatile("s_waitcnt vmcnt(0)" ::: "memory");
+      if ((int)threadIdx.x < a.njobs) sync_add(cb.counters + threadIdx.x * kSyncLineWords, 1u);
+    }
+    if (job_id == a.njobs - 1 && chunk == 0) loss_terms(cb.loss, cb.nloss, cb.losses, cb.loss_sums, smem);
+  } else if (a.bump != nullptr && blockIdx.x == 0 && threadIdx.x == 0) {
     adam_advance(a.bump, a.lr, a.beta1, a.beta2);
+  }
   const int kind = jb.kind;
 #ifdef NDP_STAMPS
   __shared__ unsigned long long wst[32];
@@ -1423,9 +1613,13 @@
 #endif
   constexpr bool WT = WIDE ? kWtSlabsWide : kWtSlabs;
   if (WIDE && kind == WG_WIDE) wgrad_wide<WT>(jb, rbeg, rend, slab, smem);
-  else if (kind == WG_FULL) wgrad_block<4, 4, WG_FULL, WT>(jb, rbeg, rend, jrows - 1, slab, smem, wst);
-  else if (kind == WG_SKINNY_B) wgrad_block<4, 1, WG_SKINNY_B, WT>(jb, rbeg, rend, jrows - 1, slab, smem, wst);
-  else wgrad_block<1, 4, WG_SKINNY_A, WT>(jb, rbeg, rend, jrows - 1, slab, smem, wst);
+  else if (kind == WG_FULL) wgrad_block<4, 4, WG_FULL, WT>(jb, rbeg, rend, jrows - 1, slab, smem, wst, combine);
+  else if (kind == WG_SKINNY_B) wgrad_block<4, 1, WG_SKINNY_B, WT>(jb, rbeg, rend, jrows - 1, slab, smem, wst, combine);
+  else wgrad_block<1, 4, WG_SKINNY_A, WT>(jb, rbeg, rend, jrows - 1, slab, smem, wst, combine);
+  if constexpr (!WIDE) {
+    static_assert(kWtSlabs, "the in-launch combine needs write-through slab stores");
+    if (combine) wgrad_combine(a, jb, cb, job_id, chunk, smem);
+  }
 #ifdef NDP_STAMPS
   NDP_WSTAMP(4);
   if (threadIdx.x == 0 && NDP_STAMP_ON(4))
@@ -1435,18 +1629,13 @@
 
 __global__ __launch_bounds__(kThreads) void k_wgrad(WgradArgs a_segment) {
   extern __shared__ __attribute__((aligned(16))) float smem[];
-  (void)a_segment;
-  wgrad_body<false>(smem);
+  wgrad_body<false>(smem, a_segment.cb);
 }
 __global__ __launch_bounds__(kThreads, 2) void k_wgrad_wide(WgradArgs a_segment) {
   extern __shared__ __attribute__((aligned(16))) float smem[];
-  (void)a_segment;
-  wgrad_body<true>(smem);
-}
-
-struct LossTerm {
-  const float* partials; int count; float scale; int slot;
-};
+  wgrad_body<true>(smem, a_segment.cb);
+}
+
 constexpr int kP2PRanks = 8;
 constexpr int kP2PCapD = 58368;
 constexpr int kP2PCapG = 86016;
@@ -1531,14 +1720,6 @@
   PackSpec pack;
 };
 
-__device__ __forceinline__ void adam_update(float& p, float g, float& m, float& v,
-                                            float step_size, float bc2_sqrt, float b1, float b2, float eps) {
-  m = m + (g - m) * (1.f - b1);
-  v = v * b2 + (1.f - b2) * g * g;
-  const float denom = sqrtf(v) / bc2_sqrt + eps;
-  p = p - step_size * (m / denom);
-}
-
 template <bool P2P>
 __global__ __launch_bounds__(kThreads) void k_reduce_adam(ReduceArgs a) {
   __shared__ float sh[8];
@@ -1569,28 +1750,8 @@
   }
   if constexpr (P2P) g = p2p_sum(a.p2p, g, p, live, (uint32_t)a.step[0]);
   if (live && a.grad != nullptr) a.grad[p] = g;
-  if (upd) {
-    adam_update(pv, g, m, v, step_size, bc2_sqrt, a.beta1, a.beta2, a.eps);
-    a.params[p] = pv;
-    a.exp_avg[p] = m;
-    a.exp_avg_sq[p] = v;
-    if (a.pack.packed != nullptr) pack_store(a.pack, (int)p, pv);
-  }
-  if (blockIdx.x == gridDim.x - 1) {
-#pragma unroll
-    for (int t = 0; t < 3; ++t) {
-      if (t >= a.nloss) break;
-      const LossTerm lt = a.loss[t];
-      float s = 0.f;
-      for (int i = threadIdx.x; i < lt.count; i += kThreads) s += lt.partials[i];
-      s = block_sum(s, sh + 4);
-      if (threadIdx.x == 0) {
-        s *= lt.scale;
-        a.losses[lt.slot] = s;
-        if (a.loss_sums != nullptr) a.loss_sums[lt.slot] += s;
-      }
-    }
-  }
+  if (upd) adam_apply(p, g, pv, m, v, step_size, bc2_sqrt, a.beta1, a.beta2, a.eps, a.params, a.exp_avg, a.exp_avg_sq, a.pack);
+  if (blockIdx.x == gridDim.x - 1) loss_terms(a.loss, a.nloss, a.losses, a.loss_sums, sh + 4);
 }
 
 __global__ void k_adam_advance(int32_t* state, float lr, float b1, float b2) { adam_advance(state, lr, b1, b2); }
diff --git a/ndivplanning_amd/trainer.py b/ndivplanning_amd/trainer.py
--- a/ndivplanning_amd/trainer.py
+++ b/ndivplanning_amd/trainer.py
@@ -64,7 +64,9 @@
         nws = self.lib.ndp_step_workspace_floats(ctypes.byref(self.cfg))
         if nws <= 0:
             raise _capi.NdpError("bad step configuration (flat=%d, num_sample=%d)" % (self.flat, self.k))
-        self.workspace = torch.empty(nws, **f32)
+        self.workspace = torch.zeros(nws, **f32)
+        sync = self.lib.ndp_step_sync_offset(ctypes.byref(self.cfg))
+        self._status = self.workspace[sync:sync + 4].view(torch.int32)
         self._graphs = None
         self._copy_stream = copy_stream
         self._stage = None
@@ -296,10 +298,18 @@
 
     def losses(self):
         v = self.losses_dev.tolist()
+        self.check_status()
         return v[0], v[1], v[2]
+
+    def check_status(self):
+        st = self._status.tolist()
+        if st[0] != 0:
+            raise _capi.NdpError("in-launch slab combine timed out: job %d, workgroup %d saw %d of %d arrivals; "
+                                 "this trainer's workspace is unusable" % (st[0] - 1, st[1], st[2], st[3]))
 
     def pop_loss_sums(self):
         v = self.loss_sums.tolist()
+        self.check_status()
         self.loss_sums.zero_()
         return v[0], v[1], v[2]
 
```

New measurement: 12390 steps/s. 6.1% lower.
